# microsoft/CryptoNets

Hardware: AMD Instinct MI355X
Metric: encrypted images/sec (CryptoNets-MNIST, N=8192) (higher is better)
Workload: dtype u64

## Files before the change

cryptonets_amd/csrc/cn_api.hip:

```cpp
#include "cn_api_shared.h"

std::vector<Slab> &slabs_of(cn_ctx *ctx) { return *reinterpret_cast<std::vector<Slab> *>(ctx->slabs); }
bool in_slab(cn_ctx *ctx, const void *p) {
    for (const Slab &s : slabs_of(ctx)) if ((const char *)p >= s.base && (const char *)p < s.base + s.bytes) return true;
    return false;
}
int use(cn_ctx *c) { HIPCHK(hipSetDevice(c->device)); return 0; }

int ensure_scratch(cn_ctx *c, size_t bytes) {
    c->soff = 0;
    if (bytes <= c->scap) return 0;
    if (c->capturing || c->graphs_alive) return fail(CN_ERR_ARG, "the scratch arena would have to grow while a graph is recorded / alive: run the sequence once before cn_graph_begin");
    HIPCHK(hipStreamSynchronize(c->stream));
    if (c->scratch) HIPCHK(hipFree(c->scratch));
    c->scratch = nullptr; c->scap = 0;
    size_t want = bytes + (bytes >> 3) + (1 << 20);
    if (hipMalloc((void **)&c->scratch, want) != hipSuccess) {
        (void)hipGetLastError();
        pool_flush(c);
        HIPCHK(hipMalloc((void **)&c->scratch, want));
    }
    c->scap = want;
    return 0;
}
// ... 250 lines not shown
        if (b.kind == 2) (void)free_gemm_plan(ctx, b);
        else if (b.kind == 3) (void)free_graph(ctx, b);
        else if (!in_slab(ctx, b.d)) (void)hipFree(b.d);
    });
    pool_flush(ctx);
    for (const Slab &sl : slabs_of(ctx)) (void)hipFree(sl.base);
    delete &slabs_of(ctx);
    if (ctx->rlk.owned) (void)hipFree(ctx->rlk.d);
    for (auto &kv : ctx->gk) if (kv.second.owned) (void)hipFree(kv.second.d);
    defer_square_release(ctx);
    (void)hipFree(ctx->sk); (void)hipFree(ctx->pk); (void)hipFree(ctx->ks_part); (void)hipFree(ctx->d_index_map); (void)hipFree(ctx->stage); if (ctx->pin) (void)hipHostFree(ctx->pin);
    (void)hipFree(ctx->scratch); (void)hipFree(ctx->tw); (void)hipFree(ctx->twd); (void)hipFree(ctx->twdh); (void)hipFree(ctx->dc);
    if (ctx->ev0) (void)hipEventDestroy(ctx->ev0);
    if (ctx->ev1) (void)hipEventDestroy(ctx->ev1);
    if (ctx->ev_order) (void)hipEventDestroy(ctx->ev_order);
    if (ctx->ev_ms) (void)hipEventDestroy(ctx->ev_ms);
    if (ctx->ev_graph) (void)hipEventDestroy(ctx->ev_graph);
    if (ctx->stream2) { (void)hipStreamSynchronize(ctx->stream2); (void)hipStreamDestroy(ctx->stream2); }
    if (ctx->ev_fork) (void)hipEventDestroy(ctx->ev_fork);
    if (ctx->ev_join) (void)hipEventDestroy(ctx->ev_join);
    if (ctx->stream) (void)hipStreamDestroy(ctx->stream);
    cn_defer_delete(ctx->dq);
    delete ctx->ring; delete ctx->ready;
    delete ctx;
}
extern "C" int cn_set_option(cn_ctx *ctx, const char *name, int value) { API_BODY
    LOCK;
    if (!name) return fail(CN_ERR_ARG, "null option name");
    if (const OptionSpec *o = find_option(name)) {
        if (!o->flag && (value < o->lo || value > o->hi)) return fail(CN_ERR_ARG, "%s: %d .. %d", name, o->lo, o->hi);
        ctx->opt.*o->member = o->flag ? value != 0 : value;
        if (o->member == &CnTunables::f64 || o->member == &CnTunables::gemm_mfma || o->member == &CnTunables::gemm_pair) defer_square_drop_plans(ctx);
        return 0;
    }
    if (!strcmp(name, "defer")) {
        if (value < 0 || value > 2) return fail(CN_ERR_ARG, "defer: 0, 1 or 2");
        ctx->defer.store(value, std::memory_order_release);
        if (value != 2) {
            while (const cn_handle h = ctx->ready->pop()) CHECK(free_body(ctx, h));
            ctx->ready->misses.store(0, std::memory_order_relaxed);
        }
        return 0;
    }
    if (!strcmp(name, "ks_xi")) {
        if (ctx->level && (value != 0) != (ctx->hc.ks_xi != 0)) return fail(CN_ERR_ARG, "ks_xi of a level context is its parent's (its keys are)");
        if (ctx->capturing || ctx->graphs_alive) return fail(CN_ERR_ARG, "ks_xi cannot change while a graph is recorded or alive (its kernels were chosen for the other convention)");
        HIPCHK(hipStreamSynchronize(ctx->stream));
        ctx->hc.ks_xi = value != 0;
        HIPCHK(hipMemcpy(ctx->dc, &ctx->hc, sizeof(DevConsts), hipMemcpyHostToDevice));
        return 0;
    }
    if (!strcmp(name, "defer_square_gemm")) { ctx->defer_square_gemm = value != 0; return 0; }
    if (!strcmp(name, "digit_mfma")) { ctx->digit_mfma = value != 0; defer_square_drop_plans(ctx); return 0; }
    if (!strcmp(name, "mul_sum")) { ctx->mul_sum = value != 0; return 0; }
    if (!strcmp(name, "record_steps")) {
        ctx->rec_steps = value != 0;
        if (!value) { ctx->rec_set.clear(); ctx->rec_cols = false; }
        return 0;
    }
    return fail(CN_ERR_ARG, "unknown option %s", name);
API_END }
extern "C" int cn_get_option(cn_ctx *ctx, const char *name, int *value) { API_BODY
    LOCK_ONLY;
    if (!name || !value) return fail(CN_ERR_ARG, "null argument");
    if (const OptionSpec *o = find_option(name)) *value = ctx->opt.*o->member;
    else if (!strcmp(name, "defer")) *value = ctx->defer.load(std::memory_order_relaxed);
    else if (!strcmp(name, "ks_xi")) *value = (int)ctx->hc.ks_xi;
    else if (!strcmp(name, "record_steps")) *value = ctx->rec_steps;
    else if (!strcmp(name, "digit_mfma")) *value = ctx->digit_mfma;
    else if (!strcmp(name, "defer_square_gemm")) *value = ctx->defer_square_gemm;
    else if (!strcmp(name, "mul_sum")) *value = ctx->mul_sum;
    else if (!strcmp(name, "pin_laps")) *value = (int)ctx->pin_laps;
    else if (!strcmp(name, "ready_handles")) *value = (int)ctx->ready->size();
    else if (!strcmp(name, "folded_zero_encryptions")) *value = (int)std::min<uint64_t>(ctx->folded_zero, 0x7fffffff);
    else if (!strcmp(name, "square_gemm_fused")) *value = (int)std::min<uint64_t>(ctx->sg_fused, 0x7fffffff);
    else if (!strcmp(name, "defer_square_gemm_fused")) *value = (int)std::min<uint64_t>(ctx->dsg_fused, 0x7fffffff);
    else if (!strcmp(name, "mul_sum_fused")) *value = (int)std::min<uint64_t>(ctx->ms_fused, 0x7fffffff);
    else if (!strcmp(name, "mul_sum_groups")) *value = (int)ctx->ms_groups;
    else if (!strcmp(name, "mul_sum_min_k")) *value = (int)MUL_SUM_MIN_K;
    else if (!strcmp(name, "defer_pending_products")) *value = (int)ctx->dq->sq->out.size();
    else if (!strcmp(name, "digit_gemm_mfma")) *value = (int)std::min<uint64_t>(ctx->dg_mfma, 0x7fffffff);
    else if (!strcmp(name, "packed_bad_residues")) *value = (int)std::min<uint64_t>(ctx->packed_bad.load(), 0x7fffffff);
    else if (!strcmp(name, "mul_relin_pipelined")) *value = (int)std::min<uint64_t>(ctx->mr_pipelined, 0x7fffffff);
    else if (!strcmp(name, "behz_small_base")) *value = ctx->hc.bsk[ctx->hc.kb - 1].q < (1ull << 49);
    else if (!strcmp(name, "behz_f64")) *value = ctx->hc.behz_f64 && ctx->opt.f64;
    else if (!strcmp(name, "mod_switch_f64")) *value = ctx->ms_f64;
    else if (!strcmp(name, "aux_primes")) *value = (int)ctx->hc.kb;
    else if (!strcmp(name, "pending_calls")) *value = (int)ctx->dq->ops.size();
    else if (!strcmp(name, "pool_arrays")) { size_t c = 0; for (auto &kv : ctx->pool) c += kv.second.size(); *value = (int)std::min<size_t>(c, 0x7fffffff); }
    else if (!strcmp(name, "stream_tries")) *value = ctx->stream_tries;
    else return fail(CN_ERR_ARG, "unknown option %s", name);
    return 0;
API_END }
extern "C" int cn_sync(cn_ctx *ctx) { API_BODY LOCK; NOT_CAPTURING("cn_sync"); HIPCHK(hipStreamSynchronize(ctx->stream)); ctx->staged.clear(); return 0; API_END }
extern "C" void *cn_stream(cn_ctx *ctx) { return (void *)ctx->stream; }
extern "C" int cn_ctx_wait_for(cn_ctx *ctx_, cn_ctx *other) {
    if (!ctx_ || !other) return fail(CN_ERR_ARG, "null argument");
    if (ctx_ == other) return 0;
    hipEvent_t ev = nullptr;
    {
        cn_ctx *ctx = other;
        const int rc = ctx->mu.run([&]() -> int {
            LOCK; NOT_CAPTURING("cn_ctx_wait_for");
            if (!ctx->ev_order) HIPCHK(hipEventCreateWithFlags(&ctx->ev_order, hipEventDisableTiming));
            HIPCHK(hipEventRecord(ctx->ev_order, ctx->stream)); ev = ctx->ev_order;
            return 0;
        });
        if (rc) return rc;
    }
    cn_ctx *ctx = ctx_;
    return ctx->mu.run([&]() -> int {
        LOCK; NOT_CAPTURING("cn_ctx_wait_for");
        HIPCHK(hipStreamWaitEvent(ctx->stream, ev, 0));
        return 0;
    });
}
extern "C" size_t cn_key_words(cn_ctx *ctx, int which) { return (size_t)(which ? ctx->hc.gk_tot : ctx->hc.rl_tot) * ctx->ctw2; }

bool keys_as_f64(const cn_ctx *ctx) { return ctx->opt.f64 && cn_mod_range(ctx->hc, 0, ctx->hc.k).f64ok && rr_kernels(ctx); }
int set_key(cn_ctx *ctx, KsKey &slot, const uint64_t *words, size_t count, size_t expect, int is_dev, bool coeff_form) {
    if (!words || count != expect) return fail(CN_ERR_ARG, "key has %zu words, expected %zu", count, expect);
    HIPCHK(hipStreamSynchronize(ctx->stream));
    if (slot.owned && slot.d) HIPCHK(hipFree(slot.d));
    slot = {nullptr, false, false};
    if (is_dev) { slot.d = (uint64_t *)words; slot.owned = false; }
    else {
        HIPCHK(hipMalloc((void **)&slot.d, count * 8));
        slot.owned = true;
        HIPCHK(hipMemcpy(slot.d, words, count * 8, hipMemcpyHostToDevice));
    }
    if (coeff_form) CHECK(cn_run_ntt(ctx, slot.d, (uint32_t)(count / ctx->hc.n), 0, ctx->hc.k, 0));
    if (keys_as_f64(ctx)) {
        hipLaunchKernelGGL(k_u64_to_f64, dim3((unsigned)((count + 255) / 256)), dim3(256), 0, ctx->stream, slot.d, count);
        HIPCHK(hipGetLastError());
// ... 429 lines not shown
```

cryptonets_amd/csrc/cn_api_shared.h:

```cpp
#pragma once
#include "cn_runtime.h"
#include "cn_rotation.h"
#include <thread>
#include "cn_k_elem.hip.h"
#include <algorithm>
#include <chrono>
#include <mutex>
#include <map>
#include <unordered_map>
#include <cstdio>
#include <cstdlib>
#include <cstring>

#define fail cn_fail
struct DOp; struct DeferQueue; struct GemmPlan; struct GemmArith; struct Tab2; struct RotJob; struct BcastNext; struct Slab;

static const RrOps *const rr_ops[3] = {&cn_rr_u64, &cn_rr_f64, &cn_rr_f64l};
static const KsOps *const ks_ops[3] = {&cn_ks_u64, &cn_ks_f64, &cn_ks_f64l};
inline bool rr_kernels(const cn_ctx *c, uint32_t max_logn = 14) { return !c->opt.legacy_ntt && cn_rr_size(c->hc.logn, max_logn); }
enum { DOP_GEMM1 = 0, DOP_ADD, DOP_SUB, DOP_ADDPLAIN, DOP_SUBPLAIN, DOP_MULRELIN, DOP_ENCRYPT,
       DOP_COPY, DOP_MULPLAIN, DOP_ROT, DOP_ROTADD, DOP_COLS, DOP_COLSADD, DOP_SUMSLOTS, DOP_TYPES };
struct DOp {
    int type; int32_t level;
    uint64_t *out;
// ... 9 lines not shown
    std::vector<uint64_t> addr, wt;
    struct Haz { int32_t w = -1, r = -1, wop = -1; uint32_t readers = 0; int32_t hd = 0; };
    struct HazMap {
        struct E { const uint64_t *key = nullptr; uint32_t epoch = 0; Haz v; };
        std::vector<E> tab = std::vector<E>(1 << 12);
        uint32_t epoch = 1; size_t used = 0;
        static size_t hash(const uint64_t *p) { uint64_t x = (uint64_t)p >> 8; x *= 0x9E3779B97F4A7C15ull; return (size_t)(x >> 20); }
        Haz *find(const uint64_t *p) {
            for (size_t i = hash(p) & (tab.size() - 1);; i = (i + 1) & (tab.size() - 1)) {
                if (tab[i].epoch != epoch) return nullptr;
                if (tab[i].key == p) return &tab[i].v;
            }
        }
        Haz &operator[](const uint64_t *p) {
            if (2 * (used + 1) > tab.size()) grow();
            for (size_t i = hash(p) & (tab.size() - 1);; i = (i + 1) & (tab.size() - 1)) {
                if (tab[i].epoch != epoch) { tab[i].key = p; tab[i].epoch = epoch; tab[i].v = Haz(); used++; return tab[i].v; }
                if (tab[i].key == p) return tab[i].v;
            }
        }
        void grow() {
            std::vector<E> old; old.swap(tab);
            tab.assign(old.size() * 2, E()); used = 0;
            for (const E &e : old) if (e.epoch == epoch) (*this)[e.key] = e.v;
        }
        void clear() { used = 0; if (++epoch == 0) { for (E &e : tab) e.epoch = 0; epoch = 1; } }
    } haz;
    int32_t maxlevel = -1;
    std::vector<std::pair<uint64_t *, size_t>> frees;
    struct Fold { int32_t enc; uint64_t w; };
    std::vector<Fold> folds;
    struct DeferSquare *sq = nullptr;
};
static const size_t SLAB_MAX_ITEM = 8u << 20, SLAB_BYTES = 64u << 20;
struct Slab { char *base; size_t bytes; };
static const uint32_t DEFER_STAGED_MAX = 4;
struct CtSpan { uint64_t *d; uint32_t count; };
struct PtSpan { const uint64_t *d; uint32_t stride; const uint8_t *zero; };
struct GaloisCall {
    const uint64_t *in; uint64_t elt; uint64_t *out, *tmp; uint32_t count;
    const uint64_t *acc = nullptr, *pre = nullptr; uint64_t next_elt = 0; uint64_t *next_out = nullptr;
};
struct BcastNext { uint64_t elt; uint64_t *out, *ctn; };
struct GemmArith { bool small, two; uint32_t lazy; int bits; };
struct GemmPlan {
    uint32_t O = 0, K = 0, Kp = 0, G = 0, M = 0, MT = 0, lazy = 0, max_in = 0;
    bool small = false, two = false, one = false, has_bias = false, mfma = false;
    uint32_t P = 0, mtiles = 0, ksteps = 0;
    cn_handle bias_pt = 0; uint32_t bias_count = 0;
    uint64_t nnz = 0;
    std::vector<char> host;
    size_t off_oidx = 0, off_bidx = 0, off_w = 0;
    char *dev = nullptr;
    bool dig = false, dig_mfma = false; uint32_t dMT = 0, dKw = 0; size_t off_dw = 0;
};
struct SgPlan {
    bool ok = false, bias = false; uint32_t O = 0, K = 0;
    std::vector<uint64_t> W; std::vector<int32_t> cidx;
    GemmPlan P; std::vector<int32_t> idx, oidx;
    uint64_t used = 0;
};
struct DeferSquare {
    uint64_t *arr = nullptr; size_t cap = 0;
    std::vector<uint64_t *> out;
    std::unordered_map<const uint64_t *, uint32_t> slot;
    std::vector<std::unique_ptr<SgPlan>> plans; uint64_t tick = 0;
};
static const size_t DEFER_SQ_PLANS = 8;
struct Tab2 { const NTT_GLOBAL uint64_t *src; NTT_GLOBAL uint64_t *dst; };
struct RotJob { const uint64_t *src; uint64_t *dst; int steps; CnRotPlan plan; };

int cn_run_ntt(cn_ctx *c, uint64_t *data, uint32_t limbs, uint32_t base_off, uint32_t nmod, int inverse);
const NoiseTab &cn_noise_table();
std::vector<Slab> &slabs_of(cn_ctx *ctx);
bool in_slab(cn_ctx *ctx, const void *p);
int use(cn_ctx *c);
int ensure_scratch(cn_ctx *c, size_t bytes);
size_t al(size_t b);
char *pin_block(cn_ctx *c, size_t bytes);
int upload_bytes(cn_ctx *c, const void *host, size_t bytes, void *dev);
int place_table(cn_ctx *c, const void *host, size_t bytes, void *fallback, const void **dev);
Buffer *getbuf(cn_ctx *c, cn_handle h, int kind);
int range_ok(const Buffer *b, uint32_t first, uint32_t count, uint32_t stride = 1);
bool streams_share_a_queue(hipStream_t a, hipStream_t b);
int pick_stream(cn_ctx *c);
int ctx_init(cn_ctx *c, uint32_t n, uint32_t k, int device, std::vector<uint64_t> &tw);
void ctx_teardown(cn_ctx *ctx);
bool keys_as_f64(const cn_ctx *ctx);
int set_key(cn_ctx *ctx, KsKey &slot, const uint64_t *words, size_t count, size_t expect, int is_dev, bool coeff_form = false);
void pool_flush(cn_ctx *ctx);
int dev_alloc(cn_ctx *ctx, size_t bytes, uint64_t **out);
int dev_release(cn_ctx *ctx, uint64_t *p, size_t bytes);
int alloc_buf(cn_ctx *ctx, int kind, uint32_t count, uint32_t size, cn_handle *out);
bool submit_async(const cn_ctx *ctx);
int free_body(cn_ctx *ctx, cn_handle h);
int free_many_body(cn_ctx *ctx, const cn_handle *h, uint32_t n);
int free_graph(cn_ctx *ctx, Buffer &b);
void end_recording(cn_ctx *root);
int ensure_index_map(cn_ctx *ctx);
int addsub(cn_ctx *ctx, cn_handle a, uint32_t ai, cn_handle b, uint32_t bi, cn_handle out, uint32_t oi, uint32_t count, int op);
int addsub_body(cn_ctx *ctx, cn_handle a, uint32_t ai, cn_handle b, uint32_t bi, cn_handle out, uint32_t oi, uint32_t count, int op);
int add_plain_body(cn_ctx *ctx, cn_handle a, uint32_t ai, cn_handle pt, uint32_t pi, int subtract, cn_handle out, uint32_t oi, uint32_t count);
bool shifted_overlap(const uint64_t *a, const uint64_t *o, size_t words);
bool mul_plain_takes_bcast(cn_ctx *ctx, uint32_t count);
int mul_plain_impl(cn_ctx *ctx, CtSpan A, bool a_bcast, PtSpan P, CtSpan O, uint32_t polys, const BcastNext *nx = nullptr);
uint64_t lift_scalar(const DevConsts &hc, uint64_t w, uint32_t j);
bool gemm_weights_small(cn_ctx *ctx, const uint64_t *W, size_t count);
// ... 247 lines not shown
```

cryptonets_amd/csrc/cn_defer.hip:

```cpp
#include "cn_api_shared.h"


static const size_t DEFER_FLUSH_MIN = 64, DEFER_MAX_OPS = 32768;
DeferQueue *cn_defer_new() { DeferQueue *q = new DeferQueue(); q->sq = new DeferSquare(); return q; }
void cn_defer_delete(DeferQueue *q) { if (q) delete q->sq; delete q; }
bool cn_defer_pending(cn_ctx *ctx) { return ctx->dq && (!ctx->dq->ops.empty() || !ctx->dq->sq->out.empty()); }

int32_t defer_level(DeferQueue *q, const uint64_t *const *ins, uint32_t nin, const uint64_t *out) {
    int32_t lv = 0;
    for (uint32_t i = 0; i < nin; i++) {
        if (!ins[i]) continue;
        const DeferQueue::Haz *h = q->haz.find(ins[i]);
        if (h) lv = std::max(lv, h->w + 1);
    }
    const DeferQueue::Haz *ho = q->haz.find(out);
    if (ho) lv = std::max(lv, std::max(ho->w, ho->r) + 1);
    return lv;
}
int defer_push(cn_ctx *ctx, DOp op, const uint64_t *const *ins, uint32_t nin) {
    DeferQueue *q = ctx->dq;
    int32_t lv = defer_level(q, ins, nin, op.out);
    const bool heavy = op.type == DOP_GEMM1 || op.type == DOP_MULRELIN;
    int32_t hd = 0;
    for (uint32_t i = 0; i < nin; i++) if (ins[i]) { const DeferQueue::Haz *h = q->haz.find(ins[i]); if (h) hd = std::max(hd, h->hd); }
// ... 199 lines not shown
    if (*rc) return true;
    sq.out.resize(n);
    for (uint32_t i = 0; i < n; i++) { sq.out[i] = ops[i]->out; sq.slot[ops[i]->out] = i; }
    if (defer_trace()) fprintf(stderr, "defer %p level %d: parks %u squarings (Multiply only, %zu MB of products)\n", (void *)ctx, level, n, need >> 20);
    return true;
}
static int pending_materialise(cn_ctx *ctx, DeferSquare &sq, const std::vector<uint8_t> &need) {
    const uint32_t n = (uint32_t)sq.out.size();
    const size_t kn = (size_t)ctx->hc.k * ctx->hc.n;
    CHECK(ensure_scratch(ctx, al((size_t)n * 8) + 4096));
    uint64_t **dout; CHECK(upload_tmp(ctx, sq.out.data(), n, &dout));
    uint32_t done = 0;
    for (uint32_t s = 0; s < n;) {
        if (!need[s]) { s++; continue; }
        uint32_t e = s; while (e < n && need[e]) e++;
        CHECK(do_keyswitch(ctx, ctx->rlk, KsCall::relin(sq.arr + (size_t)s * 3 * kn, kn, e - s).to_table(dout + s)));
        done += e - s; s = e;
    }
    if (defer_trace()) fprintf(stderr, "defer %p: materialises %u of %u pending products (one key switch each)\n", (void *)ctx, done, n);
    return 0;
}
struct SgGroup { int32_t level; SgPlan *plan; std::vector<const DOp *> rows; std::vector<int32_t> slot_of; };
static SgPlan *sg_plan(cn_ctx *ctx, DeferSquare &sq, uint32_t O, uint32_t K, std::vector<uint64_t> &W, std::vector<int32_t> &cidx, uint64_t keep) {
    for (auto &p : sq.plans)
        if (p->O == O && p->K == K && !memcmp(p->W.data(), W.data(), W.size() * 8) && !memcmp(p->cidx.data(), cidx.data(), cidx.size() * 4)) { p->used = ++sq.tick; return p.get(); }
    if (sq.plans.size() >= DEFER_SQ_PLANS) {
        size_t v = sq.plans.size();
        for (size_t i = 0; i < sq.plans.size(); i++) if (sq.plans[i]->used <= keep && (v == sq.plans.size() || sq.plans[i]->used < sq.plans[v]->used)) v = i;
        if (v < sq.plans.size()) {
            if (sq.plans[v]->P.dev) { (void)hipStreamSynchronize(ctx->stream); (void)hipFree(sq.plans[v]->P.dev); }
            sq.plans.erase(sq.plans.begin() + v);
        }
    }
    std::unique_ptr<SgPlan> p(new SgPlan());
    p->O = O; p->K = K; p->W.swap(W); p->cidx.swap(cidx); p->used = ++sq.tick;
    GemmPlan &P = p->P;
    if (build_gemm_plan(ctx, p->cidx.data(), p->W.data(), O, K, nullptr, 0, nullptr, P)) return nullptr;
    p->ok = P.dig;
    if (p->ok) {
        p->idx.assign((const int32_t *)P.host.data(), (const int32_t *)P.host.data() + (size_t)P.G * P.Kp);
        p->oidx.assign((const int32_t *)(P.host.data() + P.off_oidx), (const int32_t *)(P.host.data() + P.off_oidx) + (size_t)P.G * P.M);
        if (hipMalloc((void **)&P.dev, P.host.size()) != hipSuccess || hipMemcpy(P.dev, P.host.data(), P.host.size(), hipMemcpyHostToDevice) != hipSuccess) {
            (void)hipGetLastError();
            if (P.dev) (void)hipFree(P.dev);
            P.dev = nullptr; p->ok = false;
        }
    }
    P.host.clear(); P.host.shrink_to_fit();
    sq.plans.push_back(std::move(p));
    return sq.plans.back().get();
}
static size_t sg_scratch(cn_ctx *ctx, const GemmPlan &P) {
    const size_t kn = (size_t)ctx->hc.k * ctx->hc.n;
    return al((size_t)P.O * 2 * kn * 8) + al((size_t)P.O * ctx->hc.rl_tot * ctx->hc.n * 8) + al((size_t)P.G * P.Kp * 4) + al((size_t)P.G * P.M * 4) + al((size_t)P.O * 8) + 8192;
}
static bool sg_prepare(cn_ctx *ctx, DeferQueue *q, const std::vector<uint8_t> &dead, const std::map<const uint64_t *, size_t> &freed, std::vector<SgGroup> &groups,
                       std::vector<int32_t> &sg_of, std::vector<uint8_t> &need) {
    DeferSquare &sq = *q->sq;
    const std::vector<DOp> &ops = q->ops;
    const uint32_t n = (uint32_t)sq.out.size();
    need.assign(n, 0);
    bool ok = ctx->defer_square_gemm && square_gemm_ctx_ok(ctx) && ctx->rlk.d;
    auto slot_of = [&](const uint64_t *p) -> int32_t { if (!p) return -1; auto it = sq.slot.find(p); return it == sq.slot.end() ? -1 : (int32_t)it->second; };
    std::map<std::pair<int32_t, uint32_t>, std::vector<size_t>> cand;
    for (size_t x = 0; x < ops.size(); x++) {
        if (dead[x]) continue;
        const DOp &X = ops[x];
        if (slot_of(X.out) >= 0) ok = false;
        if (X.type == DOP_GEMM1) {
            uint32_t np = 0, other = 0;
            for (uint32_t kk = 0; kk < X.K; kk++) {
                const uint64_t *a = (const uint64_t *)q->addr[X.terms + kk];
                if (!a) continue;
                const int32_t s = slot_of(a);
                if (s >= 0) { need[s] = 1; np++; } else other++;
            }
            if (!np) continue;
            if (other || X.fold_count) ok = false;
            cand[{X.level, X.K}].push_back(x);
            continue;
        }
        if (X.type == DOP_ENCRYPT) continue;
        const bool b_plain = X.type == DOP_ADDPLAIN || X.type == DOP_SUBPLAIN || X.type == DOP_MULPLAIN;
        for (const uint64_t *p : {X.a, b_plain ? nullptr : X.b}) { const int32_t s = slot_of(p); if (s >= 0) { need[s] = 1; ok = false; } }
    }
    for (uint32_t s = 0; s < n; s++) if (!in_freed(freed, sq.out[s])) { need[s] = 1; ok = false; }
    if (!ok) return false;
    const uint64_t keep = sq.tick;
    for (auto &kv : cand) {
        const uint32_t K = kv.first.second, O = (uint32_t)kv.second.size();
        SgGroup g; g.level = kv.first.first;
        for (size_t x : kv.second) g.rows.push_back(&ops[x]);
        std::stable_sort(g.rows.begin(), g.rows.end(), [&](const DOp *x, const DOp *y) {
            return std::lexicographical_compare(&q->wt[x->terms], &q->wt[x->terms] + K, &q->wt[y->terms], &q->wt[y->terms] + K); });
        std::vector<uint64_t> W((size_t)O * K); std::vector<int32_t> cidx((size_t)O * K, -1), canon(n, -1);
        for (uint32_t o = 0; o < O; o++) {
            memcpy(&W[(size_t)o * K], &q->wt[g.rows[o]->terms], (size_t)K * 8);
            for (uint32_t kk = 0; kk < K; kk++) {
                const int32_t s = slot_of((const uint64_t *)q->addr[g.rows[o]->terms + kk]);
                if (s < 0) continue;
                if (canon[s] < 0) { canon[s] = (int32_t)g.slot_of.size(); g.slot_of.push_back(s); }
                cidx[(size_t)o * K + kk] = canon[s];
            }
        }
        g.plan = sg_plan(ctx, sq, O, K, W, cidx, keep);
        if (!g.plan || !g.plan->ok || !square_gemm_fused_ok(ctx, g.plan->P) || sg_scratch(ctx, g.plan->P) > ctx->smax) return false;
        if (sg_scratch(ctx, g.plan->P) > ctx->scap && ctx->graphs_alive) return false;
        uint64_t bbase = ~0ull;
        for (const DOp *r : g.rows) { if ((r->bias != nullptr) != (g.rows[0]->bias != nullptr)) return false; if (r->bias) bbase = std::min(bbase, (uint64_t)r->bias); }
        for (const DOp *r : g.rows) if (r->bias && ((((uint64_t)r->bias - bbase) & 255) || (((uint64_t)r->bias - bbase) >> 8) >= 0x7fffffffull)) return false;
        for (size_t x : kv.second) sg_of[x] = (int32_t)groups.size();
        groups.push_back(std::move(g));
    }
    return true;
}
static int sg_run(cn_ctx *ctx, DeferQueue *q, const SgGroup &g) {
    const SgPlan &sp = *g.plan; const GemmPlan &P = sp.P;
    const uint32_t n = ctx->hc.n, k = ctx->hc.k, tot = ctx->hc.rl_tot;
    const size_t kn = (size_t)k * n;
    std::vector<int32_t> pidx(sp.idx.size()), bidx(sp.oidx.size(), 0);
    std::vector<uint64_t *> outs(P.O);
    for (size_t x = 0; x < pidx.size(); x++) pidx[x] = sp.idx[x] >= 0 ? g.slot_of[sp.idx[x]] : -1;
    const bool bias = g.rows[0]->bias != nullptr;
    uint64_t bbase = ~0ull;
    if (bias) {
        for (const DOp *r : g.rows) bbase = std::min(bbase, (uint64_t)r->bias);
        for (size_t x = 0; x < bidx.size(); x++) if (sp.oidx[x] >= 0) bidx[x] = (int32_t)(((uint64_t)g.rows[sp.oidx[x]]->bias - bbase) >> 8);
    }
    for (uint32_t o = 0; o < P.O; o++) outs[o] = g.rows[o]->out;
    CHECK(ensure_scratch(ctx, sg_scratch(ctx, P)));
    uint64_t *T = salloc<uint64_t>(ctx, (size_t)P.O * 2 * kn);
    double *S = salloc<double>(ctx, (size_t)P.O * tot * n);
    if (!T || !S) return fail(CN_ERR_HIP, "internal: scratch exhausted in the deferred square + dense form");
    int32_t *dpidx, *dbidx; uint64_t **douts;
    CHECK(upload_tmp(ctx, pidx.data(), pidx.size(), &dpidx)); CHECK(upload_tmp(ctx, bidx.data(), bidx.size(), &dbidx)); CHECK(upload_tmp(ctx, outs.data(), outs.size(), &douts));
    const uint64_t *arr = q->sq->arr;
    CHECK(launch_gemm_plan(ctx, P, P.dev, dpidx, arr, (uint32_t)(3 * kn), 2u, bias ? (const uint64_t *)bbase : nullptr, dbidx, 32, T, 0));
    DigitGemmLaunch dg{arr + 2 * kn, 3 * kn, dpidx, P.dev + P.off_dw, P.dev + P.off_oidx, S, P.G, P.M, P.K, P.Kp, P.dKw, P.dMT};
    if (P.dig_mfma) { dg.W = P.dev + P.off_w; dg.mfma = true; dg.P = P.P; dg.mtiles = P.mtiles; dg.ksteps = P.ksteps; }
    CHECK(cn_l_digit_gemm(ctx, dg));
    CHECK(do_keyswitch(ctx, ctx->rlk, KsCall::relin_digits(S, T, kn, P.O).to_table(douts)));
    ctx->dsg_fused++;
    if (defer_trace()) fprintf(stderr, "defer %p level %d: fuses %u scalar products over %zu pending products (GEMM, digit GEMM%s, %u key switches)\n", (void *)ctx, g.level, P.O,
                               g.slot_of.size(), P.dig_mfma ? " on the matrix cores" : "", P.O);
    return 0;
}

int flush_mulrelin_group(cn_ctx *ctx, const std::vector<const DOp *> &all, const std::map<const uint64_t *, size_t> *park, int32_t level) {
    const size_t kn = (size_t)ctx->hc.k * ctx->hc.n;
    for (int sq = 1; sq >= 0; sq--) {
        std::vector<const DOp *> ops;
        for (const DOp *op : all) if ((op->a == op->b) == (sq == 1)) ops.push_back(op);
        if (ops.empty()) continue;
        if (sq && park) { int rc = 0; if (park_squarings(ctx, ctx->dq, ops, *park, level, &rc)) { CHECK(rc); continue; } }
        const size_t per = mul_scratch_per_ct(ctx, sq == 1) + al(3 * kn * 8) + 3 * 8 + 64;
        const uint32_t ch = chunk_for(ctx, per, (uint32_t)ops.size());
        for (uint32_t s0 = 0; s0 < ops.size(); s0 += ch) {
            const uint32_t c = std::min<uint32_t>(ch, (uint32_t)ops.size() - s0);
            CHECK(ensure_scratch(ctx, per * c + 3 * al((size_t)c * 8) + 8192));
            std::vector<const uint64_t *> ha(c), hb(c); std::vector<uint64_t *> ho(c);
            for (uint32_t i = 0; i < c; i++) { ha[i] = ops[s0 + i]->a; hb[i] = ops[s0 + i]->b; ho[i] = ops[s0 + i]->out; }
            const uint64_t **da, **db = nullptr; uint64_t **dout;
            CHECK(upload_tmp(ctx, ha.data(), c, &da));
            if (!sq) CHECK(upload_tmp(ctx, hb.data(), c, &db));
            CHECK(upload_tmp(ctx, ho.data(), c, &dout));
            uint64_t *t3 = salloc<uint64_t>(ctx, (size_t)c * 3 * kn);
            if (!t3) return fail(CN_ERR_HIP, "internal: scratch exhausted in deferred multiply");
            auto mul = [&](uint32_t f, uint32_t n_) { return do_multiply(ctx, nullptr, 1, nullptr, 1, t3 + (size_t)f * 3 * kn, n_, da + f, (sq ? da : db) + f); };
            auto ksw = [&](uint32_t f, uint32_t n_) { return do_keyswitch(ctx, ctx->rlk, KsCall::relin(t3 + (size_t)f * 3 * kn, kn, n_).to_table(dout + f)); };
            if (ctx->opt.sq_halves >= 2 && ctx->hc.logn <= 13 && c >= SQ_HALVES_MIN && !ctx->capturing && pipeline_fused_ks(ctx, c) && aux_stream_ready(ctx)) {
                CHECK(pipelined_halves(ctx, c, mul, ksw)); continue;
            }
            CHECK(mul(0, c));
            CHECK(ksw(0, c));
        }
    }
    return 0;
}


__global__ void k_copy_tab(const Tab2 *__restrict__ tab, uint32_t pairs_per_item) {
    const Tab2 t = tab[blockIdx.y];
    const uint32_t i = blockIdx.x * blockDim.x + threadIdx.x;
    typedef unsigned long long v2u64 __attribute__((ext_vector_type(2)));
    if (i < pairs_per_item) reinterpret_cast<NTT_GLOBAL v2u64 *>(t.dst)[i] = reinterpret_cast<const NTT_GLOBAL v2u64 *>(t.src)[i];
}
int ensure_stage(cn_ctx *ctx, size_t bytes) {
    if (bytes <= ctx->stage_cap) return 0;
    if (ctx->capturing || ctx->graphs_alive) return fail(CN_ERR_ARG, "the staging arena would have to grow while a graph is recorded / alive");
    HIPCHK(hipStreamSynchronize(ctx->stream));
    if (ctx->stage) HIPCHK(hipFree(ctx->stage));
    ctx->stage = nullptr; ctx->stage_cap = 0;
    const size_t want = bytes + (bytes >> 2) + (1 << 20);
    HIPCHK(hipMalloc((void **)&ctx->stage, want));
// ... 490 lines not shown
```

cryptonets_amd/csrc/cn_eval.hip:

```cpp
#include "cn_api_shared.h"

int addsub(cn_ctx *ctx, cn_handle a, uint32_t ai, cn_handle b, uint32_t bi, cn_handle out, uint32_t oi, uint32_t count, int op) {
    GETCT(A, a, 0); GETCT(O, out, A->size);
    Buffer *B = A;
    if (op != 2) { B = getbuf(ctx, b, 0); if (!B || B->size != A->size) return fail(CN_ERR_ARG, "operand sizes do not match"); }
    if (!range_ok(A, ai, count) || !range_ok(O, oi, count) || (op != 2 && !range_ok(B, bi, count))) return fail(CN_ERR_ARG, "index out of range");
    if (!count) return 0;
    uint32_t limbs = count * A->size * ctx->hc.k;
    hipLaunchKernelGGL(k_addsub, dim3(limbs * ctx->chunks), dim3(ctx->bs), 0, ctx->stream, A->d + ai * A->item_words,
                       B->d + (op != 2 ? bi : ai) * B->item_words, O->d + oi * O->item_words, ctx->dc, ctx->chunks, op);
    HIPCHK(hipGetLastError()); launch_count(ctx);
    return 0;
}
int addsub_body(cn_ctx *ctx, cn_handle a, uint32_t ai, cn_handle b, uint32_t bi, cn_handle out, uint32_t oi, uint32_t count, int op) {
    if (deferring(ctx)) { int rc = defer_addsub(ctx, a, ai, b, bi, out, oi, count, op); if (rc <= 0) return rc; }
    CHECK(cn_defer_flush(ctx)); CHECK(addsub(ctx, a, ai, b, bi, out, oi, count, op));
    if (op) ctx->st.Subtraction += count; else ctx->st.Addition += count;
    return 0;
}
extern "C" int cn_add(cn_ctx *ctx, cn_handle a, uint32_t ai, cn_handle b, uint32_t bi, cn_handle out, uint32_t oi, uint32_t count) {
    if (submit_async(ctx) && count <= DEFER_STAGED_MAX) return ring_push(ctx, SUB_ADD, count, a, ai, b, bi, out, oi, 0, 0);
    API_BODY LOCK_ONLY; return addsub_body(ctx, a, ai, b, bi, out, oi, count, 0); API_END
}
extern "C" int cn_sub(cn_ctx *ctx, cn_handle a, uint32_t ai, cn_handle b, uint32_t bi, cn_handle out, uint32_t oi, uint32_t count) {
// ... 228 lines not shown
    const uint64_t t = ctx->hc.t.q;
    std::vector<int32_t> gidx((size_t)O * K);
    for (uint32_t o = 0; o < O; o++) {
        bool any = false;
        for (uint32_t kk = 0; kk < K; kk++) {
            int32_t id = idx ? idx[(size_t)o * K + kk] : (int32_t)kk;
            uint64_t w = W[(size_t)o * K + kk];
            if (w >= t) return fail(CN_ERR_ARG, "weight >= plain modulus");
            if (id >= 0) P.max_in = std::max<uint32_t>(P.max_in, (uint32_t)id + 1);
            if (id >= 0 && w) { any = true; P.nnz++; }
            gidx[(size_t)o * K + kk] = id;
        }
        if (!any) return fail(CN_ERR_ARG, "output %u has no non-zero term (AddMany of nothing)", o);
        if (BP && (bias_idx[o] < 0 || (uint32_t)bias_idx[o] >= BP->count)) return fail(CN_ERR_ARG, "bias index out of range");
    }
    std::vector<uint64_t> W2;
    if (ctx->opt.gemm_pair && gemm_arith(ctx, gemm_weights_small(ctx, W, (size_t)O * K)).small && pair_gather_lists(O, K, gidx, W, W2)) W = W2.data();
    std::map<std::vector<int32_t>, std::vector<uint32_t>> groups;
    for (uint32_t o = 0; o < O; o++) groups[std::vector<int32_t>(gidx.begin() + (size_t)o * K, gidx.begin() + (size_t)(o + 1) * K)].push_back(o);
    const uint32_t NONE = 0xffffffffu;
    uint32_t G = (uint32_t)groups.size(), M = 0;
    for (auto &g : groups) M = std::max<uint32_t>(M, (uint32_t)g.second.size());
    const GemmArith ar = gemm_arith(ctx, gemm_weights_small(ctx, W, (size_t)O * K));
    const bool small = ar.small, mfma = gemm_mfma_ok(ctx, ar, M, K);
    const uint32_t Kp = mfma ? ((K + 31) / 32) * 32 : ((K + 15) & ~15u) + 16;
    std::vector<int32_t> hidx((size_t)G * Kp, -1), hoidx((size_t)G * M, -1), hbidx((size_t)G * M, 0);
    std::vector<uint32_t> member((size_t)G * M, NONE);
    {
        uint32_t g = 0;
        for (auto &kv : groups) {
            memcpy(&hidx[(size_t)g * Kp], kv.first.data(), K * 4);
            for (uint32_t m = 0; m < kv.second.size(); m++) member[(size_t)g * M + m] = kv.second[m];
            g++;
        }
    }
    for (size_t x = 0; x < member.size(); x++) if (member[x] != NONE) { hoidx[x] = (int32_t)member[x]; if (BP) hbidx[x] = bias_idx[member[x]]; }
    P.O = O; P.K = K; P.Kp = Kp; P.G = G; P.M = M; P.small = small; P.has_bias = BP != nullptr; P.bias_pt = bias_pt; P.bias_count = BP ? BP->count : 0;
    P.two = ar.two; P.lazy = ar.lazy; P.mfma = mfma;
    std::vector<char> wbytes;
    auto row = [&](uint32_t g, uint32_t m) -> const uint64_t * { return member[(size_t)g * M + m] == NONE ? nullptr : W + (size_t)member[(size_t)g * M + m] * K; };
    if (mfma) {
        P.P = gemm_weight_planes(ctx, W, (size_t)O * K); P.mtiles = (M + 31) / 32; P.ksteps = (K + 31) / 32;
        pack_gemm_mfma(ctx, G, M, K, P.P, row, [&](uint32_t g, uint32_t kk) { return hidx[(size_t)g * Kp + kk] >= 0; }, wbytes);
    } else {
        auto tap = [&](uint32_t g, uint32_t kk) { return hidx[(size_t)g * Kp + kk] >= 0; };
        pack_gemm_weights(ctx, G, M, K, small, row, tap, P.MT, wbytes);
        P.one = gemm_one_limb(ctx, ar, G, M, K, row, tap);
    }
    std::vector<double> dW;
    if (small && ctx->hc.k >= 2 && ctx->hc.dbc >= 1 && ctx->hc.dbc <= 30) {
        uint64_t qmin = ~0ull; for (uint32_t j = 0; j < ctx->hc.k; j++) qmin = std::min(qmin, ctx->hc.q[j].q);
        const uint64_t dmax = (1ull << ctx->hc.dbc) - 1, lim = std::min<uint64_t>((qmin - 1) / 2, (1ull << 52) - 1) / dmax;
        bool ok = true;
        for (uint32_t g = 0; g < G && ok; g++) for (uint32_t m = 0; m < M && ok; m++) {
            const uint64_t *wr = row(g, m);
            if (!wr) continue;
            uint64_t sum = 0;
            for (uint32_t kk = 0; kk < K; kk++) if (hidx[(size_t)g * Kp + kk] >= 0) { const uint64_t w = wr[kk]; sum += w >= ctx->hc.t_half ? t - w : w; }
            ok = sum <= lim;
        }
        if (ok) { P.dig = true; P.dig_mfma = mfma && ctx->digit_mfma && ctx->hc.dbc <= 14 && !(ctx->hc.n & 255); }
        if (ok && !P.dig_mfma) {
            P.dMT = digit_gemm_tile(M); P.dKw = digit_gemm_rows(K);
            const uint32_t mtd = (M + P.dMT - 1) / P.dMT;
            dW.assign((size_t)G * mtd * P.dKw * P.dMT, 0.0);
            for (uint32_t g = 0; g < G; g++) for (uint32_t m = 0; m < M; m++) {
                const uint64_t *wr = row(g, m);
                if (!wr) continue;
                double *dst = &dW[(((size_t)g * mtd + m / P.dMT) * P.dKw) * P.dMT + m % P.dMT];
                for (uint32_t kk = 0; kk < K; kk++) { const uint64_t w = hidx[(size_t)g * Kp + kk] >= 0 ? wr[kk] : 0; dst[(size_t)kk * P.dMT] = w >= ctx->hc.t_half ? -(double)(t - w) : (double)w; }
            }
        }
    }
    P.off_oidx = al(hidx.size() * 4); P.off_bidx = P.off_oidx + al(hoidx.size() * 4); P.off_w = P.off_bidx + al(hbidx.size() * 4);
    P.off_dw = P.off_w + al(wbytes.size());
    P.host.assign(P.off_dw + al(dW.size() * 8), 0);
    memcpy(P.host.data() + P.off_dw, dW.data(), dW.size() * 8);
    memcpy(P.host.data(), hidx.data(), hidx.size() * 4);
    memcpy(P.host.data() + P.off_oidx, hoidx.data(), hoidx.size() * 4);
    memcpy(P.host.data() + P.off_bidx, hbidx.data(), hbidx.size() * 4);
    memcpy(P.host.data() + P.off_w, wbytes.data(), wbytes.size());
    return 0;
}
int launch_gemm_plan(cn_ctx *ctx, const GemmPlan &P, const char *tables, const void *idx, const uint64_t *in, uint32_t in_unit, uint32_t polys, const uint64_t *bias, const void *bidx,
                     uint32_t bias_unit, uint64_t *out, uint32_t obase) {
    GemmLaunch gl{P.small, P.two, false, P.MT, in, idx, tables + P.off_w, tables + P.off_oidx, bias, bidx, out,
                  P.G, P.M, P.K, P.lazy, P.Kp, obase, P.P, P.mtiles, P.ksteps, polys, (uint32_t)ctx->opt.gemm_order, P.one};
    gl.in_unit = in_unit; gl.bias_unit = bias_unit;
    return P.mfma ? cn_l_gemm_mfma(ctx, gl) : cn_l_gemm(ctx, gl);
}
int run_gemm_plan(cn_ctx *ctx, const GemmPlan &P, const char *tables, Buffer *I, Buffer *OB, uint32_t oi, const uint64_t *in3) {
    if (!range_ok(OB, oi, P.O)) return fail(CN_ERR_ARG, "output index out of range");
    if (!in3) {
    if (I == OB) return fail(CN_ERR_ARG, "scalar GEMM cannot run in place");
    if (P.max_in > I->count) return fail(CN_ERR_ARG, "input index out of range");
    if (I->size != OB->size || I->size < 2 || I->size > 3) return fail(CN_ERR_ARG, "scalar GEMM: input and output ciphertext sizes must match (2 or 3)");
    } else if (OB->size != 2) return fail(CN_ERR_ARG, "scalar GEMM: output ciphertext size must be 2");
    const uint64_t *bias = nullptr;
    if (P.has_bias) {
        Buffer *BP = getbuf(ctx, P.bias_pt, 1);
        if (!BP || BP->count < P.bias_count) return fail(CN_ERR_ARG, "invalid bias plaintext handle");
        bias = BP->d;
    }
    CHECK(launch_gemm_plan(ctx, P, tables, tables, in3 ? in3 : I->d, in3 ? (uint32_t)(3 * ctx->hc.k * ctx->hc.n) : 0u, in3 ? 2u : I->size, bias, tables + P.off_bidx, 0, OB->d, oi));
    ctx->st.PlainMultiplication += P.nnz; ctx->st.Addition += P.nnz - P.O;
    if (P.has_bias) ctx->st.PlainAddition += P.O;
    return 0;
}
extern "C" int cn_scalar_gemm(cn_ctx *ctx, cn_handle in, const int32_t *idx, const uint64_t *W, uint32_t O, uint32_t K, cn_handle bias_pt,
                              const int32_t *bias_idx, cn_handle out, uint32_t oi) { API_BODY
    LOCK; GETCT(I, in, 0); GETCT(OB, out, 0);
    Buffer *BP = bias_pt ? getbuf(ctx, bias_pt, 1) : nullptr;
    GemmPlan P;
    CHECK(build_gemm_plan(ctx, idx, W, O, K, BP, bias_pt, bias_idx, P));
// ... 123 lines not shown
    return (size_t)cnt * (mode == 2 ? k : tot_dig) * ctx->ctw2 * 8 > ctx->smax ? 0 : mode;
}
int do_keyswitch(cn_ctx *ctx, const KsKey &key, const KsCall &call) {
    const uint32_t n = ctx->hc.n, k = ctx->hc.k, cnt = call.cnt, tot_dig = call.galois ? ctx->hc.gk_tot : ctx->hc.rl_tot;
    const CnModRange qr = cn_mod_range(ctx->hc, 0, k);
    const int bits = qr.bits, pol = cn_policy(qr, key.f64);
    KsArgs a{call, key.d,
             key.f64 ? (bits >= 50 ? 1u : (1u << std::min(10, 50 - bits))) : 0xffffffffu,
             ks_planned_mode(ctx, cnt, call.galois)};
    if (ctx->opt.ks_xcd == 1) a.xcd_cts = cnt & ~7u;
    else if (ctx->opt.ks_xcd == 2) a.xcd_cts = 0x80000000u;
    const bool rr = rr_kernels(ctx);
    if (a.mode) CHECK(ensure_ks_part(ctx, (size_t)cnt * (a.mode == 2 ? k : tot_dig) * ctx->ctw2 * 8));
    if (a.dig && !(rr && key.f64 && ctx->hc.logn <= 13 && !a.galois && !ctx->hc.ks_xi)) return fail(CN_ERR_ARG, "internal: ready-made digits outside the FP64 register-radix key switch");
    const bool pair = ks_pair14_ok(ctx, cnt, a.galois, key);
    if ((a.perm_elt || a.items || a.next_elt) && !a.mode && !(pair && !a.items)) return fail(CN_ERR_ARG, "internal: automorphism inside the fused key switch");
    if (pair) {
        CHECK(ensure_ks_part(ctx, (size_t)cnt * ctx->ctw2 * 8));
        a.xcd_cts = ctx->opt.ks_xcd == 1 ? (cnt & ~7u) : 0u;
        ks_ops[pol]->pair14(ctx, a);
    } else if (a.mode == 0 && rr && key.f64 && ctx->hc.logn == 14 && ctx->hc.twdh && ctx->opt.ks_split14) {
        CHECK(ensure_ks_part(ctx, (size_t)cnt * ctx->ctw2 * 8));
        ks_ops[pol]->split14(ctx, a);
        hipLaunchKernelGGL(k_ks_combine14, dim3(cnt * 2 * k * (n / 512)), dim3(256), 0, ctx->stream, (const uint64_t *)ctx->ks_part, a.add0, a.add1, a.astride, a.out, ctx->dc,
                           a.extra, a.xstride, a.out_tab);
        launch_count(ctx);
    } else {
        const bool done = rr && ks_ops[pol]->launch(ctx, a);
        if (!done && key.f64) return fail(CN_ERR_ARG, "internal: FP64 key without FP64 kernel");
        if (!done) {
            uint64_t *const out = a.out;
            if (a.extra) {
                if (a.xstride != ctx->ctw2 || a.out_tab) return fail(CN_ERR_ARG, "internal: accumulator stride");
                CHECK(ensure_ks_part(ctx, (size_t)cnt * ctx->ctw2 * 8));
                a.out = (uint64_t *)ctx->ks_part;
            }
            const uint32_t nt = std::min<uint32_t>(1024, n);
            switch (n / nt) {
                case 1: launch_ks_legacy<1>(ctx, nt, a); break;
                case 2: launch_ks_legacy<2>(ctx, nt, a); break;
                case 4: launch_ks_legacy<4>(ctx, nt, a); break;
                case 8: launch_ks_legacy<8>(ctx, nt, a); break;
                case 16: launch_ks_legacy<16>(ctx, nt, a); break;
                default: return fail(CN_ERR_ARG, "unsupported poly modulus degree for key switching");
            }
            if (a.extra) {
                hipLaunchKernelGGL(k_addsub, dim3(cnt * 2 * k * ctx->chunks), dim3(ctx->bs), 0, ctx->stream, (const uint64_t *)ctx->ks_part, a.extra, out, ctx->dc,
                                   ctx->chunks, 0);
                launch_count(ctx);
            }
        }
    }
    HIPCHK(hipGetLastError()); launch_count(ctx);
    ctx->st.ntt_forward_limbs += (uint64_t)cnt * tot_dig * k; ctx->st.ntt_inverse_limbs += (uint64_t)cnt * 2 * k;
    return 0;
}
bool ks_pair14_ok(cn_ctx *ctx, uint32_t cnt, int galois, const KsKey &key) {
    return ctx->opt.ks_pair14 && ctx->opt.ks_split14 && rr_kernels(ctx) && ctx->hc.logn == 14 && ctx->hc.twdh && key.f64 && ks_planned_mode(ctx, cnt, galois) == 0;
}
uint32_t chunk_for(cn_ctx *ctx, size_t per_ct, uint32_t count) {
    size_t c = std::max<size_t>(1, ctx->smax / per_ct);
    return (uint32_t)std::min<size_t>(c, count);
}

extern "C" int cn_multiply(cn_ctx *ctx, cn_handle a, uint32_t ai, cn_handle b, uint32_t bi, cn_handle out3, uint32_t oi, uint32_t count) { API_BODY TWO_LIMBS("cn_multiply");
    LOCK; GETCT(A, a, 2); GETCT(B, b, 2); GETCT(O, out3, 3);
    if (!range_ok(A, ai, count) || !range_ok(B, bi, count) || !range_ok(O, oi, count)) return fail(CN_ERR_ARG, "index out of range");
    if (!count) return 0;
    const uint64_t *pa = A->d + ai * A->item_words, *pb = B->d + bi * B->item_words;
    size_t per = mul_scratch_per_ct(ctx, pa == pb);
    uint32_t ch = chunk_for(ctx, per, count);
    for (uint32_t s = 0; s < count; s += ch) {
        uint32_t c = std::min(ch, count - s);
        CHECK(ensure_scratch(ctx, per * c + 4096));
        CHECK(do_multiply(ctx, pa + s * A->item_words, 1, pb + s * B->item_words, 1, O->d + (oi + s) * O->item_words, c));
    }
    return 0;
API_END }
extern "C" int cn_relinearize(cn_ctx *ctx, cn_handle in3, uint32_t ii, cn_handle out, uint32_t oi, uint32_t count) { API_BODY TWO_LIMBS("cn_relinearize");
    LOCK; GETCT(I, in3, 3); GETCT(O, out, 2);
    if (!range_ok(I, ii, count) || !range_ok(O, oi, count)) return fail(CN_ERR_ARG, "index out of range");
    if (!ctx->rlk.d) return fail(CN_ERR_NOKEY, "relinearization keys not set");
    if (!count) return 0;
    const size_t kn = (size_t)ctx->hc.k * ctx->hc.n;
    const uint64_t *p = I->d + ii * I->item_words;
    CHECK(do_keyswitch(ctx, ctx->rlk, KsCall::relin(p, kn, count).to(O->d + oi * O->item_words)));
    ctx->st.Relinarization += count;
    return 0;
API_END }
static int mul_relin_overlap(cn_handle x, uint32_t xi, uint32_t xstride, cn_handle out, uint32_t oi, uint32_t count) {
    if (x != out || !count) return 0;
    const uint64_t lo = xi, hi = (uint64_t)xi + (uint64_t)(count - 1) * xstride + 1, olo = oi, ohi = (uint64_t)oi + count;
    if ((lo == olo && hi == ohi) || hi <= olo || ohi <= lo) return 0;
    return fail(CN_ERR_ARG, "mul_relin: an operand range and the result range overlap partially (use the same range or disjoint ranges)");
}
extern "C" int cn_mul_relin(cn_ctx *ctx, cn_handle a, uint32_t ai, uint32_t astride, cn_handle b, uint32_t bi, uint32_t bstride, cn_handle out,
                            uint32_t oi, uint32_t count) {
    TWO_LIMBS("cn_mul_relin");
    CHECK(mul_relin_overlap(a, ai, astride, out, oi, count)); CHECK(mul_relin_overlap(b, bi, bstride, out, oi, count));
    if (submit_async(ctx) && count <= DEFER_STAGED_MAX) return ring_push(ctx, SUB_MUL_RELIN, count, a, ai, b, bi, out, oi, astride, bstride);
    API_BODY LOCK_ONLY; return mul_relin_body(ctx, a, ai, astride, b, bi, bstride, out, oi, count); API_END
}
int mul_relin_body(cn_ctx *ctx, cn_handle a, uint32_t ai, uint32_t astride, cn_handle b, uint32_t bi, uint32_t bstride, cn_handle out, uint32_t oi, uint32_t count) {
    CHECK(mul_relin_overlap(a, ai, astride, out, oi, count)); CHECK(mul_relin_overlap(b, bi, bstride, out, oi, count));
    if (deferring(ctx)) return defer_mul_relin(ctx, a, ai, astride, b, bi, bstride, out, oi, count);
    CHECK(cn_defer_flush(ctx));
    GETCT(A, a, 2); GETCT(B, b, 2); GETCT(O, out, 2);
    if (!range_ok(A, ai, astride ? count : 1, astride ? astride : 1) || !range_ok(B, bi, bstride ? count : 1, bstride ? bstride : 1) || !range_ok(O, oi, count))
        return fail(CN_ERR_ARG, "index out of range");
    if (!ctx->rlk.d) return fail(CN_ERR_NOKEY, "relinearization keys not set");
    if (!count) return 0;
    const size_t kn = (size_t)ctx->hc.k * ctx->hc.n;
    const uint64_t *pa = A->d + ai * A->item_words, *pb = B->d + bi * B->item_words;
    const bool square = (pa == pb && astride == bstride);
    size_t per = mul_scratch_per_ct(ctx, square) + al(3 * kn * 8);
    uint32_t ch = chunk_for(ctx, per, count);
    for (uint32_t s = 0; s < count; s += ch) {
        uint32_t c = std::min(ch, count - s);
        CHECK(ensure_scratch(ctx, per * c + 8192));
        uint64_t *t3 = salloc<uint64_t>(ctx, (size_t)c * 3 * kn);
        auto mul = [&](uint32_t f, uint32_t n_) { return do_multiply(ctx, pa + (size_t)(s + f) * astride * A->item_words, astride, pb + (size_t)(s + f) * bstride * B->item_words, bstride, t3 + (size_t)f * 3 * kn, n_); };
        auto ksw = [&](uint32_t f, uint32_t n_) { return do_keyswitch(ctx, ctx->rlk, KsCall::relin(t3 + (size_t)f * 3 * kn, kn, n_).to(O->d + (oi + s + f) * O->item_words)); };
        if (ctx->opt.sq_halves && ctx->hc.logn <= 13 && c >= SQ_HALVES_MIN && !ctx->capturing && pipeline_fused_ks(ctx, c) && aux_stream_ready(ctx)) {
            CHECK(pipelined_halves(ctx, c, mul, ksw)); continue;
        }
        CHECK(mul(0, c));
        CHECK(ksw(0, c));
    }
    ctx->st.Relinarization += count;
    return 0;
}

bool square_gemm_ctx_ok(cn_ctx *ctx) {
    return ctx->opt.f64 && rr_kernels(ctx, 13) && !ctx->hc.ks_xi && ctx->rlk.f64 && cn_mod_range(ctx->hc, 0, ctx->hc.k).f64ok;
}
bool square_gemm_fused_ok(cn_ctx *ctx, const GemmPlan &P) { return P.dig && square_gemm_ctx_ok(ctx); }
extern "C" int cn_square_gemm(cn_ctx *ctx, cn_handle plan, cn_handle in, uint32_t ii, cn_handle out, uint32_t oi) { TWO_LIMBS("cn_square_gemm"); API_BODY
    LOCK; GETCT(I, in, 2); GETCT(OB, out, 2);
    Buffer *PB = getbuf(ctx, plan, 2);
    if (!PB || !PB->plan) return fail(CN_ERR_ARG, "invalid scalar GEMM plan handle");
    const GemmPlan &P = *PB->plan;
    const uint32_t cnt = P.max_in;
    if (!range_ok(I, ii, cnt)) return fail(CN_ERR_ARG, "input index out of range");
    if (!range_ok(OB, oi, P.O)) return fail(CN_ERR_ARG, "output index out of range");
    if (I == OB) return fail(CN_ERR_ARG, "cn_square_gemm cannot run in place");
    if (!ctx->rlk.d) return fail(CN_ERR_NOKEY, "relinearization keys not set");
    const uint32_t n = ctx->hc.n, k = ctx->hc.k, tot = ctx->hc.rl_tot;
    const size_t kn = (size_t)k * n;
    const size_t per = mul_scratch_per_ct(ctx, true);
    const size_t fixed = al((size_t)cnt * 3 * kn * 8) + al((size_t)P.O * tot * n * 8) + 8192;
    if (!square_gemm_fused_ok(ctx, P) || fixed + per > ctx->smax) {
        cn_handle tmp = 0;
        CHECK(alloc_buf(ctx, 0, cnt, 2, &tmp));
        int rc = mul_relin_body(ctx, in, ii, 1, in, ii, 1, tmp, 0, cnt);
        if (!rc) rc = cn_defer_flush(ctx);
        OB = getbuf(ctx, out, 0);
        if (!rc) rc = run_gemm_plan(ctx, P, P.dev, getbuf(ctx, tmp, 0), OB, oi);
        const int rf = free_body(ctx, tmp);
        return rc ? rc : rf;
    }
    const uint32_t ch = (uint32_t)std::min<size_t>(cnt, (ctx->smax - fixed) / per);
    CHECK(ensure_scratch(ctx, fixed + per * ch + 4096));
    uint64_t *t3 = salloc<uint64_t>(ctx, (size_t)cnt * 3 * kn);
    double *S = salloc<double>(ctx, (size_t)P.O * tot * n);
    if (!t3 || !S) return fail(CN_ERR_HIP, "internal: scratch exhausted in cn_square_gemm");
    const size_t mark = ctx->soff;
    const uint64_t *pa = I->d + ii * I->item_words;
    for (uint32_t s = 0; s < cnt; s += ch) {
        const uint32_t c = std::min(ch, cnt - s);
        ctx->soff = mark;
        CHECK(do_multiply(ctx, pa + (size_t)s * I->item_words, 1, pa + (size_t)s * I->item_words, 1, t3 + (size_t)s * 3 * kn, c));
    }
    CHECK(run_gemm_plan(ctx, P, P.dev, nullptr, OB, oi, t3));
    DigitGemmLaunch dg{t3 + 2 * kn, 3 * kn, P.dev, P.dev + P.off_dw, P.dev + P.off_oidx, S, P.G, P.M, P.K, P.Kp, P.dKw, P.dMT};
    if (P.dig_mfma) { dg.W = P.dev + P.off_w; dg.mfma = true; dg.P = P.P; dg.mtiles = P.mtiles; dg.ksteps = P.ksteps; }
    CHECK(cn_l_digit_gemm(ctx, dg));
    uint64_t *o = OB->d + oi * OB->item_words;
    CHECK(do_keyswitch(ctx, ctx->rlk, KsCall::relin_digits(S, o, kn, P.O).to(o)));
    ctx->st.Relinarization += cnt; ctx->sg_fused++;
    return 0;
API_END }

static bool mul_sum_fused_ok(cn_ctx *ctx, uint32_t K) {
    if (!ctx->mul_sum || K < MUL_SUM_MIN_K || !square_gemm_ctx_ok(ctx)) return false;
    const int dbc = ctx->hc.dbc;
    if (dbc < 1 || dbc > 31) return false;
    const unsigned __int128 s = (unsigned __int128)K * ((1ull << dbc) - 1);
    if (s >= ((unsigned __int128)1 << 52)) return false;
    const uint64_t qmax = cn_mod_range(ctx->hc, 0, ctx->hc.k).qmax;
    for (uint32_t j = 0; j < ctx->hc.k; j++) {
        if (s >= ctx->hc.q[j].q / 2) return false;
        if (ctx->hc.rl_dig[j] > PRODUCT_SUM_MAX_DIGITS) return false;
    }
    return (unsigned __int128)K * (qmax - 1) < ((unsigned __int128)1 << 64) && !(ctx->hc.n & 511);
}
static int add_many_terms(cn_ctx *ctx, Buffer *T, uint32_t K, Buffer *O, uint32_t oi, uint32_t count) {
    std::vector<uint32_t> idx((size_t)count * K);
    for (uint32_t i = 0; i < count; i++) for (uint32_t kk = 0; kk < K; kk++) idx[(size_t)i * K + kk] = kk * count + i;
    CHECK(ensure_scratch(ctx, al(idx.size() * 4) + 4096));
    uint32_t *didx; CHECK(upload_tmp(ctx, idx.data(), idx.size(), &didx));
    const uint32_t limbs = T->size * ctx->hc.k;
    for (uint32_t i = 0; i < count; i++) {
        hipLaunchKernelGGL(k_add_many, dim3(limbs * ctx->chunks), dim3(ctx->bs), 0, ctx->stream, T->d, didx + (size_t)i * K, K, T->item_words,
                           O->d + (oi + i) * O->item_words, ctx->dc, ctx->chunks);
        HIPCHK(hipGetLastError()); launch_count(ctx);
    }
    return 0;
}
extern "C" int cn_mul_relin_sum(cn_ctx *ctx, const cn_handle *a, const uint32_t *a_idx, const cn_handle *b, const uint32_t *b_idx, uint32_t K, uint32_t b_stride,
                                cn_handle out, uint32_t oi, uint32_t count) { TWO_LIMBS("cn_mul_relin_sum"); API_BODY
    LOCK;
    if (!a || !b) return fail(CN_ERR_ARG, "null argument");
    if (!K || !count) return fail(CN_ERR_ARG, "cn_mul_relin_sum of an empty list");
    if (b_stride > 1) return fail(CN_ERR_ARG, "cn_mul_relin_sum: b_stride is 0 (one ciphertext for every output) or 1");
    if ((uint64_t)K * count > 0x7fffffffull) return fail(CN_ERR_ARG, "cn_mul_relin_sum: too many products");
    GETCT(O, out, 2);
    if (!range_ok(O, oi, count)) return fail(CN_ERR_ARG, "output index out of range");
    auto ai = [&](uint32_t kk) { return a_idx ? a_idx[kk] : 0u; };
    auto bi = [&](uint32_t kk) { return b_idx ? b_idx[kk] : 0u; };
    for (uint32_t kk = 0; kk < K; kk++) {
        if (a[kk] == out || b[kk] == out) return fail(CN_ERR_ARG, "cn_mul_relin_sum cannot run in place (out is an operand handle)");
        Buffer *A = getbuf(ctx, a[kk], 0), *B = getbuf(ctx, b[kk], 0);
        if (!A || !B) return fail(CN_ERR_ARG, "invalid ciphertext handle in term %u", kk);
        if (A->size != 2 || B->size != 2) return fail(CN_ERR_ARG, "ciphertext size mismatch in term %u", kk);
        if (!range_ok(A, ai(kk), count) || !range_ok(B, bi(kk), b_stride ? count : 1)) return fail(CN_ERR_ARG, "index out of range in term %u", kk);
    }
    if (!ctx->rlk.d) return fail(CN_ERR_NOKEY, "relinearization keys not set");
    ctx->ms_groups = 0;
    const uint32_t n = ctx->hc.n, k = ctx->hc.k, tot = ctx->hc.rl_tot;
    const size_t kn = (size_t)k * n;
    if (K == 1) {
        int rc = mul_relin_body(ctx, a[0], ai(0), 1, b[0], bi(0), b_stride, out, oi, count);
        if (!rc) rc = cn_defer_flush(ctx);
        if (!rc) { ctx->st.AddMany += count; ctx->st.AddManyItemCount += count; }
        return rc;
    }
    const size_t per = mul_scratch_per_ct(ctx, false);
    const size_t per_out = (size_t)K * 3 * kn * 8 + (size_t)tot * n * 8 + (size_t)K * 16, slack = 4 * 256 + 8192;
    const size_t g_fit = ctx->smax > per + slack ? (ctx->smax - per - slack) / per_out : 0;
    if (!mul_sum_fused_ok(ctx, K) || !g_fit) {
        cn_handle tmp = 0;
        CHECK(alloc_buf(ctx, 0, K * count, 2, &tmp));
        int rc = 0;
        for (uint32_t kk = 0; kk < K && !rc; kk++) rc = mul_relin_body(ctx, a[kk], ai(kk), 1, b[kk], bi(kk), b_stride, tmp, kk * count, count);
        if (!rc) rc = cn_defer_flush(ctx);
        if (!rc) rc = add_many_terms(ctx, getbuf(ctx, tmp, 0), K, getbuf(ctx, out, 0), oi, count);
        if (!rc) { ctx->st.AddMany += count; ctx->st.AddManyItemCount += (uint64_t)count * K; }
        const int rf = free_body(ctx, tmp);
        return rc ? rc : rf;
    }
    const uint32_t g = (uint32_t)std::min<size_t>(count, g_fit);
    std::vector<const uint64_t *> ha((size_t)g * K), hb((size_t)g * K);
    for (uint32_t o0 = 0; o0 < count; o0 += g) {
        const uint32_t go = std::min(g, count - o0), np = go * K;
        const size_t fixed = al((size_t)np * 3 * kn * 8) + al((size_t)go * tot * n * 8) + 2 * al((size_t)np * 8) + 8192;
        const uint32_t ch = (uint32_t)std::min<size_t>(np, std::max<size_t>(1, (ctx->smax - std::min(ctx->smax, fixed)) / per));
        CHECK(ensure_scratch(ctx, fixed + per * ch + 4096));
        uint64_t *t3 = salloc<uint64_t>(ctx, (size_t)np * 3 * kn);
        double *S = salloc<double>(ctx, (size_t)go * tot * n);
        if (!t3 || !S) return fail(CN_ERR_HIP, "internal: scratch exhausted in cn_mul_relin_sum");
        for (uint32_t i = 0; i < go; i++) for (uint32_t kk = 0; kk < K; kk++) {
            const Buffer *A = getbuf(ctx, a[kk], 0), *B = getbuf(ctx, b[kk], 0);
            ha[(size_t)i * K + kk] = A->d + (size_t)(ai(kk) + o0 + i) * A->item_words;
            hb[(size_t)i * K + kk] = B->d + (size_t)(bi(kk) + (o0 + i) * b_stride) * B->item_words;
        }
        const uint64_t **da, **db;
        CHECK(upload_tmp(ctx, ha.data(), np, &da)); CHECK(upload_tmp(ctx, hb.data(), np, &db));
        const size_t mark = ctx->soff;
        for (uint32_t s = 0; s < np; s += ch) {
            const uint32_t c = std::min(ch, np - s);
            ctx->soff = mark;
            CHECK(do_multiply(ctx, nullptr, 1, nullptr, 1, t3 + (size_t)s * 3 * kn, c, da + s, db + s));
        }
        uint64_t *o = O->d + (size_t)(oi + o0) * O->item_words;
        CHECK(cn_l_product_sum(ctx, ProductSumLaunch{t3, K, o, S, go}));
        CHECK(do_keyswitch(ctx, ctx->rlk, KsCall::relin_digits(S, o, kn, go).to(o)));
        ctx->ms_groups++;
    }
    ctx->st.Relinarization += (uint64_t)K * count; ctx->st.AddMany += count; ctx->st.AddManyItemCount += (uint64_t)count * K;
    ctx->ms_fused++;
    return 0;
API_END }

const KsKey *galois_key(cn_ctx *ctx, uint64_t elt) { auto it = ctx->gk.find(elt); return it != ctx->gk.end() && it->second.d ? &it->second : nullptr; }
static int columns_key(cn_ctx *ctx) { return galois_key(ctx, 2ull * ctx->hc.n - 1) ? 0 : fail(CN_ERR_NOKEY, "Galois key not present"); }
static int add_overlap(cn_ctx *ctx, const uint64_t *in, const uint64_t *acc, const uint64_t *out, uint32_t count) {
    if (!shifted_overlap(in, out, count * ctx->ctw2) && !shifted_overlap(acc, out, count * ctx->ctw2)) return 0;
    return fail(CN_ERR_ARG, "rotate-and-add: operand / accumulator and result ranges overlap partially (use the same range or disjoint ranges)");
}
int do_galois(cn_ctx *ctx, const GaloisCall &g) {
    const KsKey *key = galois_key(ctx, g.elt);
    if (!key) return fail(CN_ERR_NOKEY, "Galois key not present");
    const size_t kn = (size_t)ctx->hc.k * ctx->hc.n;
    const uint32_t count = g.count, limbs = count * 2 * ctx->hc.k, elt = (uint32_t)g.elt;
    const bool shifted = shifted_overlap(g.in, g.out, count * ctx->ctw2);
    CHECK(add_overlap(ctx, nullptr, g.acc, g.out, count));
    KsCall ks;
    if (!shifted && ks_pair14_ok(ctx, count, 1, *key)) {
        if (!g.pre) {
            hipLaunchKernelGGL(k_galois_limbs, dim3(count * ctx->hc.k), dim3(1024), (size_t)ctx->hc.n * 8, ctx->stream, g.in + kn, 2 * kn, g.tmp, kn, ctx->dc, g.elt);
            HIPCHK(hipGetLastError()); launch_count(ctx);
        }
        ks = KsCall::galois_of(g.pre ? g.pre : g.tmp, kn, g.in, kn, count).perm(elt).next((uint32_t)g.next_elt, g.next_out);
    } else if (g.pre || g.next_elt) return fail(CN_ERR_ARG, "internal: rotation chain outside the one-launch key switch");
    else if (!shifted && ctx->opt.ks_perm_fused && ks_planned_mode(ctx, count, 1) != 0)
        ks = KsCall::galois_of(g.in + kn, 2 * kn, g.in, kn, count).perm(elt);
    else {
        if (ctx->hc.n >= 1024) hipLaunchKernelGGL(k_galois_lds, dim3(limbs), dim3(std::min<uint32_t>(1024, ctx->hc.n / 4)), (size_t)ctx->hc.n * 8, ctx->stream, g.in, g.tmp, ctx->dc, g.elt);
        else hipLaunchKernelGGL(k_galois, dim3(limbs * ctx->chunks), dim3(ctx->bs), 0, ctx->stream, g.in, g.tmp, ctx->dc, ctx->chunks, g.elt);
        HIPCHK(hipGetLastError()); launch_count(ctx);
        ks = KsCall::galois_of(g.tmp + kn, 2 * kn, g.tmp, kn, count);
    }
    CHECK(do_keyswitch(ctx, *key, ks.to(g.out).plus(g.acc, ctx->ctw2)));
    ctx->st.Rotation += count;
    if (g.acc) ctx->st.Addition += count;
    return 0;
}
static int ct_scratch(cn_ctx *ctx, uint32_t count, uint32_t arrays, uint64_t **first) {
    CHECK(ensure_scratch(ctx, al(count * ctx->ctw2 * 8) * arrays));
    *first = salloc<uint64_t>(ctx, count * ctx->ctw2);
    return 0;
}
int galois_impl(cn_ctx *ctx, CtSpan in, uint64_t elt, CtSpan acc, CtSpan out) {
    if (acc.d) CHECK(add_overlap(ctx, in.d, acc.d, out.d, out.count));
    if (!out.count) return 0;
    uint64_t *tmp; CHECK(ct_scratch(ctx, out.count, 1, &tmp));
    return do_galois(ctx, {.in = in.d, .elt = elt, .out = out.d, .tmp = tmp, .count = out.count, .acc = acc.d});
}
extern "C" int cn_apply_galois(cn_ctx *ctx, cn_handle in, uint32_t ii, uint64_t elt, cn_handle out, uint32_t oi, uint32_t count) { API_BODY TWO_LIMBS("cn_apply_galois");
// ... 302 lines not shown
```

cryptonets_amd/csrc/cn_k_gemm.hip.h:

```cpp
#pragma once
#include "cn_dev_common.hip.h"

DEV void gemm_block_coords(uint32_t bx, uint32_t by, uint32_t chunks, uint32_t limbs, uint32_t mtiles, uint32_t G, uint32_t &chunk, uint32_t &limb, uint32_t &mt, uint32_t &g,
                           uint32_t order = 0) {
    if (order == 1) {
        const uint32_t x = bx & 7, r = bx >> 3;
        if (mtiles == 1) { mt = 0; g = r; } else { mt = r % mtiles; g = r / mtiles; }
        const uint32_t sl = by * 8 + x;
        chunk = sl & (chunks - 1); limb = sl >> (__ffs((int)chunks) - 1);
        return;
    }
    const uint32_t b = bx, D = chunks * limbs * G;
    uint32_t d;
    if ((D & 7) == 0) { const uint32_t r = b >> 3; mt = r % mtiles; d = (r / mtiles) * 8 + (b & 7); }
    else { d = b % D; mt = b / D; }
    chunk = d % chunks; limb = (d / chunks) % limbs; g = d / (chunks * limbs);
}
DEV const NTT_GLOBAL uint64_t *gmem(uint64_t a) { return (const NTT_GLOBAL uint64_t *)a; }
DEV NTT_GLOBAL uint64_t *gmem_w(uint64_t a) { return (NTT_GLOBAL uint64_t *)a; }
struct GemmUnits { uint32_t in, out, bias; };
template <bool ABS> struct GemmTab { typedef int32_t T; };
template <> struct GemmTab<true> { typedef uint64_t T; };
template <int MT, bool ABS = false>
__global__ void __launch_bounds__(256) k_scalar_gemm(const uint64_t *__restrict__ in, const void *__restrict__ idx_, const uint64_t *__restrict__ Wl,
// ... 321 lines not shown
        fb[3][lane][wave] = byte_perm(cd13, ab13, 0x07060302u);
        fb[4][lane][wave] = byte_perm(hcd, hab, 0x05040100u);
        fb[5][lane][wave] = byte_perm(hcd, hab, 0x07060302u);
        load_x(xn, nidx); load_a(afn, ks + GEMM_MFMA_DEPTH);
        load_idx(nidx, ks + GEMM_MFMA_DEPTH + 1);
        __syncthreads();
        if (active) {
            v4i_t bf[ND];
#pragma unroll
            for (int i = 0; i < ND; i++) bf[i] = *reinterpret_cast<const v4i_t *>(&fb[i][lane][0]);
#pragma unroll
            for (int p = 0; p < P; p++)
#pragma unroll
                for (int i = 0; i < ND; i++) acc[i + p] = __builtin_amdgcn_mfma_i32_32x32x32_i8(af[p], bf[i], acc[i + p], 0, 0, 0);
        }
    };
    uint32_t ks = 0;
    for (; ks + NB <= ksteps; ks += NB) {
#pragma unroll
        for (int s = 0; s < NB; s++) step(xs[s], afs[s], xs[(s + GEMM_MFMA_DEPTH) % NB], afs[(s + GEMM_MFMA_DEPTH) % NB], ks + s, frag[s]);
    }
#pragma unroll
    for (int s = 0; s < NB - 1; s++)
        if (ks + s < ksteps) step(xs[s], afs[s], xs[(s + GEMM_MFMA_DEPTH) % NB], afs[(s + GEMM_MFMA_DEPTH) % NB], ks + s, frag[s]);
    if (!active) return;
    const BzF::Mod mq = {C->qd[j], C->qinvd[j]};
    const DMod qm = C->q[j];
    const double c24 = BzF::center(16777216.0, mq), c48 = BzF::center(__dmul_rn(c24, 16777216.0), mq);
#pragma unroll
    for (int r = 0; r < 16; r++) {
        const uint32_t row = (uint32_t)(r & 3) + 8u * (uint32_t)(r >> 2) + 4u * half, o = g * M + mt * 32 + row;
        if (mt * 32 + row >= M) continue;
        auto group = [&](int d0) {
            double t = (double)acc[d0][r];
            if (d0 + 1 < D) t = __fma_rn((double)acc[d0 + 1 < D ? d0 + 1 : d0][r], 256.0, t);
            if (d0 + 2 < D) t = __fma_rn((double)acc[d0 + 2 < D ? d0 + 2 : d0][r], 65536.0, t);
            return t;
        };
        double v = __dadd_rn(group(0), BzF::mulmod(group(3), c24, mq));
        if (D > 6) v = __dadd_rn(v, BzF::mulmod(group(6), c48, mq));
        uint64_t res = BzF::to_u64(v, mq);
        if constexpr (ABS) {
            if (!out_idx[o]) continue;
            if (bias_idx && bias_idx[o] && limb < k) { const uint64_t bv = gmem(bias_idx[o])[(size_t)ctile * 32 + col]; if (bv) res = addmod(res, scale_plain(C, bv, j), qm.q); }
            gmem_w(out_idx[o])[e] = res;
        } else {
            if (out_idx[o] < 0) continue;
            if (bias && limb < k) { const uint64_t bv = bias[(size_t)bias_idx[o] * bu + (size_t)ctile * 32 + col]; if (bv) res = addmod(res, scale_plain(C, bv, j), qm.q); }
            out[(size_t)(obase + (uint32_t)out_idx[o]) * ou + e] = res;
        }
    }
}

template <int MT, int DG>
__global__ void __launch_bounds__(256) k_digit_gemm(const uint64_t *__restrict__ in, size_t in_unit, const int32_t *__restrict__ idx, const double *__restrict__ Wd,
                                                    const int32_t *__restrict__ out_idx, double *__restrict__ S, const DevConsts *__restrict__ C, uint32_t G, uint32_t M,
                                                    uint32_t K, uint32_t mtiles, uint32_t Kp, uint32_t Kw, uint32_t ndg) {
    const uint32_t n = C->n, k = C->k, chunks = n >> 8;
    uint32_t chunk, lj, mt, g;
    gemm_block_coords(blockIdx.x, 0, chunks, k * ndg, mtiles, G, chunk, lj, mt, g);
    const uint32_t l = lj % k, d0 = (lj / k) * DG, nd = C->rl_dig[l];
    if (d0 >= nd) return;
    uint32_t g0 = 0;
    for (uint32_t x = 0; x < l; x++) g0 += C->rl_dig[x];
    const uint32_t i = chunk * 256 + threadIdx.x, dbc = (uint32_t)C->dbc, mask = (1u << dbc) - 1;
    const size_t e = (size_t)l * n + i;
    uint32_t sh[DG];
#pragma unroll
    for (int d = 0; d < DG; d++) sh[d] = min(dbc * (d0 + (uint32_t)d), 63u);
    double acc[DG][MT];
#pragma unroll
    for (int d = 0; d < DG; d++)
#pragma unroll
        for (int m = 0; m < MT; m++) acc[d][m] = 0.0;
    const int32_t *gi = idx + (size_t)g * Kp;
    const double *gw = Wd + ((size_t)g * mtiles + mt) * (size_t)Kw * MT;
    constexpr int PF = 4, WB = MT > 10 ? 1 : 2;
    auto fetch = [&](uint64_t (&x)[PF], uint32_t kk) {
        const int4 ids = *reinterpret_cast<const int4 *>(__builtin_assume_aligned(gi + min(kk, Kp - PF), 16));
        const int32_t id[4] = {ids.x, ids.y, ids.z, ids.w};
#pragma unroll
        for (int p = 0; p < PF; p++) x[p] = in[(size_t)max(id[p], 0) * in_unit + e];
    };
    auto terms = [&](const uint64_t (&x)[PF], uint32_t kk) {
#pragma unroll
        for (int p0 = 0; p0 < PF; p0 += WB) {
            double w[WB * MT];
            const double *wp = gw + (size_t)(kk + p0) * MT;
#pragma unroll
            for (int q = 0; q < WB * MT; q++) w[q] = wp[q];
#pragma unroll
            for (int p = p0; p < p0 + WB; p++) {
                double dg[DG];
#pragma unroll
                for (int d = 0; d < DG; d++) dg[d] = (double)((uint32_t)(x[p] >> sh[d]) & mask);
#pragma unroll
                for (int m = 0; m < MT; m++)
#pragma unroll
                    for (int d = 0; d < DG; d++) acc[d][m] = __fma_rn(dg[d], w[(p - p0) * MT + m], acc[d][m]);
            }
        }
    };
    {
        const uint32_t sets = (K + PF - 1) / PF;
        uint32_t kk = 0;
        uint64_t xa[PF], xb[PF];
        fetch(xa, 0);
        for (uint32_t it = sets >> 1; it; it--, kk += 2 * PF) {
            fetch(xb, kk + PF);
            terms(xa, kk);
            fetch(xa, kk + 2 * PF);
            terms(xb, kk + PF);
        }
        if (sets & 1) terms(xa, kk);
    }
    const uint32_t tot = C->rl_tot;
#pragma unroll
    for (int m = 0; m < MT; m++) {
        const uint32_t mm = mt * MT + (uint32_t)m;
        if (mm >= M) break;
        const int32_t o = out_idx[g * M + mm];
        if (o < 0) continue;
#pragma unroll
        for (int d = 0; d < DG; d++)
            if (d0 + (uint32_t)d < nd) S[((size_t)o * tot + g0 + d0 + (uint32_t)d) * n + i] = acc[d][m];
    }
}

template <int P, int DG>
__global__ void __launch_bounds__(256, 2) k_digit_gemm_mfma(const uint64_t *__restrict__ in, size_t in_unit, const int32_t *__restrict__ idx, const int8_t *__restrict__ Wf,
                                                            const int32_t *__restrict__ out_idx, double *__restrict__ S, const DevConsts *__restrict__ C, uint32_t G,
                                                            uint32_t M, uint32_t mtiles, uint32_t ksteps, uint32_t ndg) {
    constexpr int NP = 2 * DG, D = P + 1, NB = GEMM_MFMA_DEPTH + 1;
    __shared__ __align__(16) uint32_t frag[NB][NP][64][4];
    const uint32_t n = C->n, k = C->k, ctiles = n >> 5;
    const uint32_t lane = threadIdx.x & 63, wave = (uint32_t)__builtin_amdgcn_readfirstlane((int)(threadIdx.x >> 6)), half = lane >> 5, col = lane & 31;
    uint32_t b = blockIdx.x;
    const uint32_t x8 = b & 7; b >>= 3;
    const uint32_t dgi = b % ndg; b /= ndg;
    const uint32_t ctile = (b % (ctiles >> 3)) * 8 + x8; b /= ctiles >> 3;
    const uint32_t l = b % k; b /= k;
    const uint32_t mgroups = (mtiles + 3) >> 2, mg = b % mgroups, g = b / mgroups;
    const uint32_t d0 = dgi * DG, nd = C->rl_dig[l];
    if (d0 >= nd) return;
    const uint32_t cnt = min((uint32_t)DG, nd - d0);
    uint32_t g0 = 0;
    for (uint32_t x = 0; x < l; x++) g0 += C->rl_dig[x];
    const uint32_t mt = mg * 4 + wave;
    const bool active = mt < mtiles;
    const uint32_t dbc = (uint32_t)C->dbc, mask = (1u << dbc) - 1;
    uint32_t sh[DG];
#pragma unroll
    for (int d = 0; d < DG; d++) sh[d] = min(dbc * (d0 + (uint32_t)d), 63u);
    const size_t e = (size_t)l * n + (size_t)ctile * 32 + col;
    const uint32_t Kp = ksteps * 32;
    const int32_t *gi = idx + (size_t)g * Kp + 4 * wave;
    const int8_t *wf = Wf + ((((size_t)g * P) * mtiles + (active ? mt : 0)) * ksteps) * 1024 + (size_t)lane * 16;
    v16i_t acc[DG][D];
#pragma unroll
    for (int d = 0; d < DG; d++)
#pragma unroll
        for (int j = 0; j < D; j++)
#pragma unroll
            for (int r = 0; r < 16; r++) acc[d][j][r] = 0;
    const uint32_t klast = ksteps - 1;
    auto load_idx = [&](int32_t (&s)[8], uint32_t ks) {
        const int32_t *t = gi + (size_t)min(ks, klast) * 32;
#pragma unroll
        for (int u = 0; u < 4; u++) { s[u] = t[u]; s[4 + u] = t[16 + u]; }
    };
    auto load_x = [&](uint64_t (&x)[4], const int32_t (&s)[8]) {
#pragma unroll
        for (int u = 0; u < 4; u++) {
            size_t o0 = (size_t)max(s[u], 0) * in_unit, o1 = (size_t)max(s[4 + u], 0) * in_unit;
            asm volatile("" : "+s"(o0), "+s"(o1));
            x[u] = in[(half ? o1 : o0) + e];
        }
    };
    auto load_a = [&](v4i_t (&af)[P], uint32_t ks) {
#pragma unroll
        for (int p = 0; p < P; p++) af[p] = *reinterpret_cast<const v4i_t *>(wf + ((size_t)p * mtiles * ksteps + min(ks, klast)) * 1024);
    };
    uint64_t xs[NB][4];
    v4i_t afs[NB][P];
    int32_t nidx[8];
    load_idx(nidx, 0);
#pragma unroll
    for (int s = 0; s < GEMM_MFMA_DEPTH; s++) { load_x(xs[s], nidx); load_a(afs[s], s); load_idx(nidx, s + 1); }
    auto step = [&](uint64_t (&x)[4], v4i_t (&af)[P], uint64_t (&xn)[4], v4i_t (&afn)[P], uint32_t ks, uint32_t (*fb)[64][4]) {
#pragma unroll
        for (int d = 0; d < DG; d++) {
            uint32_t t[4];
#pragma unroll
            for (int u = 0; u < 4; u++) t[u] = ((uint32_t)(x[u] >> sh[d]) & mask) + 128u;
            const uint32_t ab = byte_perm(t[1], t[0], 0x05010400u), cd = byte_perm(t[3], t[2], 0x05010400u);
            fb[2 * d][lane][wave] = byte_perm(cd, ab, 0x05040100u) ^ 0x80808080u;
            fb[2 * d + 1][lane][wave] = byte_perm(cd, ab, 0x07060302u);
        }
        load_x(xn, nidx); load_a(afn, ks + GEMM_MFMA_DEPTH);
        load_idx(nidx, ks + GEMM_MFMA_DEPTH + 1);
        __syncthreads();
        if (active) {
#pragma unroll
            for (int d = 0; d < DG; d++) {
                if ((uint32_t)d >= cnt) continue;
                const v4i_t blo = *reinterpret_cast<const v4i_t *>(&fb[2 * d][lane][0]), bhi = *reinterpret_cast<const v4i_t *>(&fb[2 * d + 1][lane][0]);
#pragma unroll
                for (int p = 0; p < P; p++) acc[d][p] = __builtin_amdgcn_mfma_i32_32x32x32_i8(af[p], blo, acc[d][p], 0, 0, 0);
#pragma unroll
                for (int p = 0; p < P; p++) acc[d][p + 1] = __builtin_amdgcn_mfma_i32_32x32x32_i8(af[p], bhi, acc[d][p + 1], 0, 0, 0);
            }
        }
    };
    uint32_t ks = 0;
    for (; ks + NB <= ksteps; ks += NB) {
#pragma unroll
        for (int s = 0; s < NB; s++) step(xs[s], afs[s], xs[(s + GEMM_MFMA_DEPTH) % NB], afs[(s + GEMM_MFMA_DEPTH) % NB], ks + s, frag[s]);
    }
#pragma unroll
    for (int s = 0; s < NB - 1; s++)
        if (ks + s < ksteps) step(xs[s], afs[s], xs[(s + GEMM_MFMA_DEPTH) % NB], afs[(s + GEMM_MFMA_DEPTH) % NB], ks + s, frag[s]);
    if (!active) return;
    const uint32_t tot = C->rl_tot, olast = G * M - 1;
    int32_t oo[16];
#pragma unroll
    for (int r = 0; r < 16; r++) {
        const uint32_t mm = mt * 32 + (uint32_t)(r & 3) + 8u * (uint32_t)(r >> 2) + 4u * half;
        oo[r] = out_idx[min(g * M + mm, olast)];
        if (mm >= M) oo[r] = -1;
    }
#pragma unroll
    for (int d = 0; d < DG; d++) {
        if ((uint32_t)d >= cnt) continue;
#pragma unroll
        for (int r = 0; r < 16; r++) {
            if (oo[r] < 0) continue;
            double v = (double)acc[d][0][r];
#pragma unroll
            for (int j = 1; j < D; j++) v = __fma_rn((double)acc[d][j][r], (double)(1u << (8 * j)), v);
            S[((size_t)oo[r] * tot + g0 + d0 + (uint32_t)d) * n + (size_t)ctile * 32 + col] = v;
        }
    }
}

typedef uint64_t ps_u64x2 __attribute__((ext_vector_type(2)));
typedef double ps_f64x2 __attribute__((ext_vector_type(2)));
DEV uint64_t ps_reduce(uint64_t x, const DMod &m) {
    const uint64_t r = x - __umul64hi(x, m.r1) * m.q;
    return r >= m.q ? r - m.q : r;
}
template <int ND>
__global__ void __launch_bounds__(256) k_product_sum(const uint64_t *__restrict__ prod_, uint32_t K, uint64_t *__restrict__ out_, double *__restrict__ S_,
                                                     const DevConsts *__restrict__ C) {
    typedef const NTT_GLOBAL ps_u64x2 *In;
    constexpr int PF = 4;
    const uint32_t n = C->n, k = C->k, n2 = n >> 1, tiles = n >> 9;
    uint32_t b = blockIdx.x;
    const uint32_t tile = b % tiles; b /= tiles;
    const uint32_t l = b % k, o = b / k;
    const uint32_t p = tile * 256 + threadIdx.x;
    const uint32_t dbc = (uint32_t)C->dbc, mask = (1u << dbc) - 1, nd = C->rl_dig[l];
    uint32_t g0 = 0;
    for (uint32_t x = 0; x < l; x++) g0 += C->rl_dig[x];
    uint32_t sh[ND];
#pragma unroll
    for (int d = 0; d < ND; d++) sh[d] = min(dbc * (uint32_t)d, 63u);
    const size_t comp = (size_t)k * n2, unit = 3 * comp;
    const NTT_GLOBAL char *src = (const NTT_GLOBAL char *)prod_ + (size_t)o * K * unit * 16;
    const uint32_t lane_off = (l * n2 + p) * 16;
    uint64_t c0x = 0, c0y = 0, c1x = 0, c1y = 0, dx[ND], dy[ND];
#pragma unroll
    for (int d = 0; d < ND; d++) { dx[d] = 0; dy[d] = 0; }
    auto fetch = [&](ps_u64x2 (&x)[PF][3], uint32_t kk) {
#pragma unroll
        for (int t = 0; t < PF; t++) {
            const NTT_GLOBAL char *s = src + (size_t)min(kk + (uint32_t)t, K - 1) * unit * 16;
#pragma unroll
            for (int c = 0; c < 3; c++) x[t][c] = *(In)(s + (size_t)c * comp * 16 + lane_off);
        }
    };
    auto term = [&](const ps_u64x2 (&x)[3]) {
        c0x += x[0].x; c0y += x[0].y; c1x += x[1].x; c1y += x[1].y;
#pragma unroll
        for (int d = 0; d < ND; d++) { dx[d] += (uint32_t)(x[2].x >> sh[d]) & mask; dy[d] += (uint32_t)(x[2].y >> sh[d]) & mask; }
    };
    auto terms = [&](const ps_u64x2 (&x)[PF][3]) {
#pragma unroll
        for (int t = 0; t < PF; t++) term(x[t]);
    };
    auto tail = [&](const ps_u64x2 (&x)[PF][3], uint32_t nv) {
#pragma unroll
        for (int t = 0; t < PF; t++) if ((uint32_t)t < nv) term(x[t]);
    };
    {
        uint32_t kk = 0;
        ps_u64x2 xa[PF][3], xb[PF][3];
        fetch(xa, 0);
        for (uint32_t it = K / (2 * PF); it; it--, kk += 2 * PF) {
            fetch(xb, kk + PF);
            terms(xa);
            fetch(xa, kk + 2 * PF);
            terms(xb);
        }
        const uint32_t r = K - kk;
        if (r > PF) fetch(xb, kk + PF);
        tail(xa, min(r, (uint32_t)PF));
        if (r > PF) tail(xb, r - PF);
    }
    const DMod m = C->q[l];
    typedef NTT_GLOBAL ps_u64x2 *Out;
    Out dst = (Out)out_ + (size_t)o * 2 * comp + (size_t)l * n2 + p;
    ps_u64x2 v;
    v.x = ps_reduce(c0x, m); v.y = ps_reduce(c0y, m); dst[0] = v;
    v.x = ps_reduce(c1x, m); v.y = ps_reduce(c1y, m); dst[comp] = v;
    typedef NTT_GLOBAL ps_f64x2 *OutS;
    OutS sd = (OutS)S_ + ((size_t)o * C->rl_tot + g0) * n2 + p;
#pragma unroll
    for (int d = 0; d < ND; d++)
        if ((uint32_t)d < nd) { ps_f64x2 w; w.x = (double)dx[d]; w.y = (double)dy[d]; sd[(size_t)d * n2] = w; }
}
```

cryptonets_amd/csrc/cn_k_ks.hip.h:

```cpp
#pragma once
#include "cn_dev_common.hip.h"

template <class AR, int L> struct KsFwd { typedef AR P; static constexpr bool lds = false; };
template <int RN, int L> struct KsFwd<ArF64T<RN>, L> { typedef typename std::conditional<(L <= 13), ArF64LdsT<RN>, ArF64T<RN>>::type P; static constexpr bool lds = L <= 13; };
DEV void ks_premultiply(uint64_t (&raw)[16], const DevConsts *C, uint32_t l) {
    if (C->ks_xi) {
        const DMod ql = C->q[l]; const uint64_t f = C->ks_inv_qhat_q[l];
#pragma unroll
        for (int r = 0; r < 16; r++) raw[r] = mulmod(raw[r], f, ql);
    }
}
template <class AR> struct KsMac;
template <> struct KsMac<ArU64> {
    static DEV void mac(uint64_t &acc, uint64_t x, uint64_t key, const DMod &qm, const ArCtx<ArU64> &A) { acc = addmod(acc, mulmod(canon4(x, qm.q), key, qm), qm.q); }
    static DEV void settle(uint64_t (&)[16], const ArCtx<ArU64> &) {}
    static DEV uint64_t sum(uint64_t acc, uint64_t x, const DMod &qm) { return addmod(acc, x, qm.q); }
};
template <int RN> struct KsMac<ArF64T<RN>> {
    typedef ArF64T<RN> ArF64;
    static DEV void mac(double &acc, double x, double key, const DMod &, const ArCtx<ArF64> &A) { acc = __dadd_rn(acc, ArF64::mulmod(x, key, A.m)); }
    static DEV void settle(double (&a)[16], const ArCtx<ArF64> &A) { ArF64::renorm(a, A.m); }
    static DEV double sum(double acc, double x, const DMod &) { return __dadd_rn(acc, x); }
};
#ifndef KS_SGPR_A
#define KS_SGPR_A 1
#endif
template <class FW0, bool ON> struct KsPassA { typedef FW0 P; };
template <class FW0> struct KsPassA<FW0, true> { typedef ArPassA<FW0> P; };
#ifndef KS_PRE_SYNC
#define KS_PRE_SYNC 1
#endif
#ifndef KS_SRC_AHEAD
#define KS_SRC_AHEAD 0
#endif
#ifndef KS_MAC_FENCE
#define KS_MAC_FENCE 0
#endif
template <class AR> struct KsDigits {};
template <class AR> struct KsSrc { typedef AR P; static constexpr bool dig = false; };
template <class AR> struct KsSrc<KsDigits<AR>> { typedef AR P; static constexpr bool dig = true; };
template <int L, class AR_, int MINW = 1, bool TWL = false, bool XI = false>
__global__ void __launch_bounds__(NttPlan<L>::NT, MINW) k_keyswitch_rr(const uint64_t *__restrict__ target, size_t tgt_stride, const uint64_t *__restrict__ add0,
                                                                 const uint64_t *__restrict__ add1, size_t add_stride, const void *__restrict__ key_,
                                                                 uint64_t *out, const DevConsts *__restrict__ C, int galois, uint32_t accmax,
                                                                 const uint64_t *extra, size_t ex_stride, uint64_t *const *__restrict__ out_tab,
                                                                 uint32_t xcd_cts) {
    typedef typename KsSrc<AR_>::P AR;
    constexpr bool DIG = KsSrc<AR_>::dig;
    typedef typename AR::T T;
    static_assert(!DIG || (std::is_same<T, double>::value && !XI), "ready-made digits: FP64 policies, plain decomposition");
    extern __shared__ __align__(16) unsigned char smem[];
    T *s = reinterpret_cast<T *>(smem);
    constexpr uint32_t n = 1u << L;
    constexpr int SA = NttPlan<L>::SA;
    const uint32_t k = C->k, tid = threadIdx.x;
    uint32_t ct = blockIdx.x / k, j = blockIdx.x % k;
    if (xcd_cts & 0x80000000u) { const uint32_t cnt = gridDim.x / k; j = blockIdx.x / cnt; ct = blockIdx.x % cnt; }
    else if (blockIdx.x < xcd_cts * k) { const uint32_t x = blockIdx.x & 7, sl = blockIdx.x >> 3; ct = 8 * (sl / k) + x; j = sl % k; }
    const DMod qm = C->q[j];
    const uint64_t q = qm.q;
    const ArCtx<AR> A(C, j);
    const int dbc = galois ? C->gdbc : C->dbc;
    const uint64_t mask = (1ull << dbc) - 1;
    const size_t kn = (size_t)k * n;
    T acc0[16], acc1[16];
#pragma unroll
    for (int r = 0; r < 16; r++) { acc0[r] = 0; acc1[r] = 0; }
    typedef typename std::conditional<TWL, typename KsFwd<AR, L>::P, AR>::type FW0;
    typedef typename KsPassA<FW0, KS_SGPR_A && std::is_same<T, double>::value>::P FW;
    typename FW::Tw fwt;
    if constexpr (TWL) {
        static_assert(KsFwd<AR, L>::lds, "LDS twiddles need an FP64 policy and N <= 8192");
        double *tws = reinterpret_cast<double *>(smem) + ntt_lds_words(n);
        stage_table(tws, A.fw.w, n, tid, NttPlan<L>::NT);
        fwt.w = (const __attribute__((address_space(3))) double *)tws;
        __syncthreads();
    } else static_cast<typename FW0::Tw &>(fwt) = A.fw;
    if constexpr (HasPassA<FW>::value) ntt_load_pass_a<SA>(fwt, A.fw.w);
    const T *kp = reinterpret_cast<const T *>(key_);
    uint32_t terms = 0;
    uint64_t raw[16];
    constexpr bool AHEAD = KS_SRC_AHEAD && MINW == 1 && L <= 13;
    uint64_t nraw[AHEAD ? 16 : 1];
    auto request = [&](uint64_t (&w)[16], uint32_t l) {
        uint32_t t0 = tid;
        asm volatile("" : "+v"(t0));
        const uint64_t *src = target + (size_t)ct * tgt_stride + (size_t)l * n;
#pragma unroll
        for (int r = 0; r < 16; r++) w[r] = src[pass_index<L, SA, 0>(t0, r)];
    };
    if constexpr (AHEAD) request(nraw, 0);
    const double *dsrc = reinterpret_cast<const double *>(target) + (size_t)ct * tgt_stride;
    for (uint32_t l = 0; l < k; l++) {
        const uint32_t nd = galois ? C->gk_dig[l] : C->rl_dig[l];
        if constexpr (DIG) {
        } else if constexpr (AHEAD) {
#pragma unroll
            for (int r = 0; r < 16; r++) raw[r] = nraw[r];
            request(nraw, min(l + 1, k - 1));
        } else request(raw, l);
        if constexpr (XI) {
            const DMod ql = C->q[l]; const uint64_t xf = C->ks_inv_qhat_q[l];
#pragma unroll
            for (int r = 0; r < 16; r++) raw[r] = mulmod(raw[r], xf, ql);
        }
        for (uint32_t d = 0; d < nd; d++, kp += 2 * kn) {
            const int sh = dbc * (int)d;
            uint32_t tl = tid;
            asm volatile("" : "+v"(tl));
            T v[16];
            if constexpr (DIG) {
#pragma unroll
                for (int r = 0; r < 16; r++) v[r] = (T)dsrc[pass_index<L, SA, 0>(tl, r)];
                dsrc += n;
            } else {
#pragma unroll
            for (int r = 0; r < 16; r++) {
                uint64_t t = (raw[r] >> sh) & mask;
                if constexpr (std::is_same<T, uint64_t>::value) { if (mask >= q) t = t >= q ? bred128(t, 0, qm) : t; }
                v[r] = A.load(t);
            }
            if constexpr (std::is_same<T, double>::value) { if (mask >= q) AR::renorm(v, A.m); }
            }
            ntt_forward_regs<FW, L, KS_PRE_SYNC != 0>(v, s, fwt, A.m, tl);
            const T *k0 = kp + (size_t)j * n, *k1 = kp + kn + (size_t)j * n;
#pragma unroll
            for (int r = 0; r < 16; r += 2) {
                if (KS_MAC_FENCE || std::is_same<T, uint64_t>::value) __builtin_amdgcn_sched_barrier(0);
                const uint32_t pos = tail_index<L>(tl, r);
                struct alignas(16) P2 { T a, b; };
                const P2 a = *reinterpret_cast<const P2 *>(k0 + pos), b = *reinterpret_cast<const P2 *>(k1 + pos);
                KsMac<AR>::mac(acc0[r], v[r], a.a, qm, A); KsMac<AR>::mac(acc0[r + 1], v[r + 1], a.b, qm, A);
                KsMac<AR>::mac(acc1[r], v[r], b.a, qm, A); KsMac<AR>::mac(acc1[r + 1], v[r + 1], b.b, qm, A);
            }
            if (++terms == accmax) { terms = 0; KsMac<AR>::settle(acc0, A); KsMac<AR>::settle(acc1, A); }
            if (!KS_PRE_SYNC) __syncthreads();
        }
    }
    if (KS_PRE_SYNC && !ntt_tail_local<L>()) __syncthreads();
#pragma unroll 1
    for (int p = 0; p < 2; p++) {
        T v[16];
#pragma unroll
        for (int r = 0; r < 16; r++) v[r] = p ? acc1[r] : acc0[r];
        uint32_t tl = tid;
// ... 279 lines not shown
            }
        }
    }
}
template <class T> NTT_DEV void ks_load2(const NTT_GLOBAL T *p, T &a, T &b) {
    typedef T V2 __attribute__((ext_vector_type(2)));
    const V2 v = *reinterpret_cast<const NTT_GLOBAL V2 *>(p);
    a = v.x; b = v.y;
}
template <int L> NTT_DEV void ks_gather_automorphism(uint64_t (&raw)[16], const NTT_GLOBAL uint64_t *limb, uint32_t elt, uint64_t q, void *image, uint32_t tid) {
    constexpr uint32_t n = 1u << L, NT = NttPlan<L>::NT;
    uint64_t *s = reinterpret_cast<uint64_t *>(image);
#pragma unroll
    for (int r = 0; r < 16; r++) {
        const uint32_t i = tid + NT * (uint32_t)r, pos = (i * elt) & (2 * n - 1);
        const uint64_t v = limb[i];
        s[lds_pos(pos & (n - 1))] = (pos >> L) ? (v ? q - v : 0) : v;
    }
    __syncthreads();
#pragma unroll
    for (int r = 0; r < 16; r++) raw[r] = s[lds_pos(pass_index<L, NttPlan<L>::SA, 0>(tid, r))];
    __syncthreads();
}
template <int L, class AR_>
__global__ void __launch_bounds__(NttPlan<L>::NT) k_ks_digit_mac(const uint64_t *__restrict__ target, size_t tgt_stride, const void *__restrict__ key_,
                                                                  void *__restrict__ part_, const DevConsts *__restrict__ C, int galois, uint32_t tot, uint32_t perm_elt,
                                                                  const KsItem *__restrict__ items) {
    typedef typename KsSrc<AR_>::P AR;
    constexpr bool DIG = KsSrc<AR_>::dig;
    typedef typename AR::T T;
    extern __shared__ __align__(16) unsigned char smem[];
    T *s = reinterpret_cast<T *>(smem);
    constexpr uint32_t n = 1u << L;
    constexpr int SA = NttPlan<L>::SA;
    const uint32_t k = C->k, tid = threadIdx.x;
    const uint32_t j = blockIdx.x % k, g = (blockIdx.x / k) % tot, ct = blockIdx.x / (k * tot);
    uint32_t l = 0, d = g;
    for (;; l++) { const uint32_t nd = galois ? C->gk_dig[l] : C->rl_dig[l]; if (d < nd) break; d -= nd; }
    const DMod qm = C->q[j];
    const uint64_t q = qm.q;
    const ArCtx<AR> A(C, j);
    const int dbc = galois ? C->gdbc : C->dbc, sh = dbc * (int)d;
    const uint64_t mask = (1ull << dbc) - 1;
    const size_t kn = (size_t)k * n;
    const NTT_GLOBAL uint64_t *src = (const NTT_GLOBAL uint64_t *)target + (size_t)ct * tgt_stride + (size_t)l * n;
    const NTT_GLOBAL T *keyp = (const NTT_GLOBAL T *)key_;
    if (items) {
        const KsItem it = items[ct];
        src = (const NTT_GLOBAL uint64_t *)it.in + kn + (size_t)l * n; keyp = (const NTT_GLOBAL T *)it.key; perm_elt = it.elt;
    }
    T v[16];
    if constexpr (DIG) {
        static_assert(std::is_same<T, double>::value, "ready-made digits: FP64 policies");
        const double *dsrc = reinterpret_cast<const double *>(target) + (size_t)ct * tgt_stride + (size_t)g * n;
#pragma unroll
        for (int r = 0; r < 16; r++) v[r] = (T)dsrc[pass_index<L, SA, 0>(tid, r)];
    } else {
    uint64_t raw[16];
    if (perm_elt) ks_gather_automorphism<L>(raw, src, perm_elt, C->q[l].q, s, tid);
    else {
#pragma unroll
        for (int r = 0; r < 16; r++) raw[r] = src[pass_index<L, SA, 0>(tid, r)];
    }
    ks_premultiply(raw, C, l);
#pragma unroll
    for (int r = 0; r < 16; r++) {
        uint64_t t = (raw[r] >> sh) & mask;
        if constexpr (std::is_same<T, uint64_t>::value) { if (mask >= q) t = t >= q ? bred128(t, 0, qm) : t; }
        v[r] = A.load(t);
    }
    if constexpr (std::is_same<T, double>::value) { if (mask >= q) AR::renorm(v, A.m); }
    }
    ntt_forward_regs<AR, L>(v, s, A.fw, A.m, tid);
    const NTT_GLOBAL T *k0 = keyp + (size_t)g * 2 * kn + (size_t)j * n, *k1 = k0 + kn;
    T *o0 = reinterpret_cast<T *>(part_) + (((size_t)ct * tot + g) * 2) * kn + (size_t)j * n, *o1 = o0 + kn;
    struct alignas(16) P2 { T a, b; };
#pragma unroll
    for (int r = 0; r < 16; r += 2) {
        const uint32_t pos = tail_index<L>(tid, r);
        P2 a, b;
        ks_load2<T>(k0 + pos, a.a, a.b); ks_load2<T>(k1 + pos, b.a, b.b);
        P2 x = {0, 0}, y = {0, 0};
        KsMac<AR>::mac(x.a, v[r], a.a, qm, A); KsMac<AR>::mac(x.b, v[r + 1], a.b, qm, A);
        KsMac<AR>::mac(y.a, v[r], b.a, qm, A); KsMac<AR>::mac(y.b, v[r + 1], b.b, qm, A);
        *reinterpret_cast<P2 *>(o0 + pos) = x; *reinterpret_cast<P2 *>(o1 + pos) = y;
    }
}
template <int L, class AR_>
__global__ void __launch_bounds__(NttPlan<L>::NT) k_ks_limb_mac(const uint64_t *__restrict__ target, size_t tgt_stride, const void *__restrict__ key_,
                                                                 void *__restrict__ part_, const DevConsts *__restrict__ C, int galois, uint32_t accmax, uint32_t perm_elt,
                                                                 const KsItem *__restrict__ items) {
    typedef typename KsSrc<AR_>::P AR;
    constexpr bool DIG = KsSrc<AR_>::dig;
    typedef typename AR::T T;
    extern __shared__ __align__(16) unsigned char smem[];
    T *s = reinterpret_cast<T *>(smem);
    constexpr uint32_t n = 1u << L;
    constexpr int SA = NttPlan<L>::SA;
    const uint32_t k = C->k, tid = threadIdx.x;
    const uint32_t j = blockIdx.x % k, l = (blockIdx.x / k) % k, ct = blockIdx.x / (k * k);
    const DMod qm = C->q[j];
    const uint64_t q = qm.q;
    const ArCtx<AR> A(C, j);
    const int dbc = galois ? C->gdbc : C->dbc;
    const uint64_t mask = (1ull << dbc) - 1;
    const size_t kn = (size_t)k * n;
    uint32_t g0 = 0;
    for (uint32_t i = 0; i < l; i++) g0 += galois ? C->gk_dig[i] : C->rl_dig[i];
    const uint32_t nd = galois ? C->gk_dig[l] : C->rl_dig[l];
    const NTT_GLOBAL uint64_t *src = (const NTT_GLOBAL uint64_t *)target + (size_t)ct * tgt_stride + (size_t)l * n;
    const NTT_GLOBAL T *keyp = (const NTT_GLOBAL T *)key_;
    if (items) {
        const KsItem it = items[ct];
        src = (const NTT_GLOBAL uint64_t *)it.in + kn + (size_t)l * n; keyp = (const NTT_GLOBAL T *)it.key; perm_elt = it.elt;
    }
    uint64_t raw[16];
    if constexpr (DIG) static_assert(std::is_same<T, double>::value, "ready-made digits: FP64 policies");
    else {
    if (perm_elt) ks_gather_automorphism<L>(raw, src, perm_elt, C->q[l].q, s, tid);
    else {
        uint32_t t0 = tid;
        asm volatile("" : "+v"(t0));
#pragma unroll
        for (int r = 0; r < 16; r++) raw[r] = src[pass_index<L, SA, 0>(t0, r)];
    }
    ks_premultiply(raw, C, l);
    }
    const double *dsrc = reinterpret_cast<const double *>(target) + (size_t)ct * tgt_stride + (size_t)g0 * n;
    T acc0[16], acc1[16];
#pragma unroll
    for (int r = 0; r < 16; r++) { acc0[r] = 0; acc1[r] = 0; }
    const NTT_GLOBAL T *kp = keyp + (size_t)g0 * 2 * kn;
    uint32_t terms = 0;
    for (uint32_t d = 0; d < nd; d++, kp += 2 * kn) {
        const int sh = dbc * (int)d;
        uint32_t tl = tid;
        asm volatile("" : "+v"(tl));
        T v[16];
        if constexpr (DIG) {
#pragma unroll
            for (int r = 0; r < 16; r++) v[r] = (T)dsrc[pass_index<L, SA, 0>(tl, r)];
            dsrc += n;
        } else {
#pragma unroll
        for (int r = 0; r < 16; r++) {
            uint64_t t = (raw[r] >> sh) & mask;
            if constexpr (std::is_same<T, uint64_t>::value) { if (mask >= q) t = t >= q ? bred128(t, 0, qm) : t; }
            v[r] = A.load(t);
        }
        if constexpr (std::is_same<T, double>::value) { if (mask >= q) AR::renorm(v, A.m); }
        }
        ntt_forward_regs<AR, L, KS_PRE_SYNC != 0>(v, s, A.fw, A.m, tl);
        const NTT_GLOBAL T *k0 = kp + (size_t)j * n, *k1 = kp + kn + (size_t)j * n;
#pragma unroll
        for (int r = 0; r < 16; r += 2) {
            const uint32_t pos = tail_index<L>(tl, r);
            struct alignas(16) P2 { T a, b; };
            P2 a, b;
            ks_load2<T>(k0 + pos, a.a, a.b); ks_load2<T>(k1 + pos, b.a, b.b);
            KsMac<AR>::mac(acc0[r], v[r], a.a, qm, A); KsMac<AR>::mac(acc0[r + 1], v[r + 1], a.b, qm, A);
            KsMac<AR>::mac(acc1[r], v[r], b.a, qm, A); KsMac<AR>::mac(acc1[r + 1], v[r + 1], b.b, qm, A);
        }
        if (++terms == accmax) { terms = 0; KsMac<AR>::settle(acc0, A); KsMac<AR>::settle(acc1, A); }
        if (!KS_PRE_SYNC) __syncthreads();
    }
    KsMac<AR>::settle(acc0, A); KsMac<AR>::settle(acc1, A);
    T *o0 = reinterpret_cast<T *>(part_) + (((size_t)ct * k + l) * 2) * kn + (size_t)j * n, *o1 = o0 + kn;
    struct alignas(16) P2 { T a, b; };
#pragma unroll
    for (int r = 0; r < 16; r += 2) {
        const uint32_t pos = tail_index<L>(tid, r);
        *reinterpret_cast<P2 *>(o0 + pos) = P2{acc0[r], acc0[r + 1]};
        *reinterpret_cast<P2 *>(o1 + pos) = P2{acc1[r], acc1[r + 1]};
    }
}
template <int L, class AR>
__global__ void __launch_bounds__(NttPlan<L>::NT) k_ks_sum_intt(const void *__restrict__ part_, const uint64_t *__restrict__ add0, const uint64_t *__restrict__ add1,
                                                                 size_t add_stride, uint64_t *out, const DevConsts *__restrict__ C, uint32_t tot,
                                                                 uint32_t accmax, const uint64_t *extra, size_t ex_stride, uint64_t *const *__restrict__ out_tab, uint32_t perm_elt,
                                                                 const KsItem *__restrict__ items) {
    typedef typename AR::T T;
// ... 46 lines not shown
```

cryptonets_amd/csrc/cn_l_gemm.hip:

```cpp
#include "cn_runtime.h"
#include <algorithm>
#include "cn_k_gemm.hip.h"

struct GemmGrid { dim3 grid; uint32_t order; };
static GemmGrid gemm_grid(cn_ctx *c, const GemmLaunch &g, uint32_t mtiles) {
    const uint32_t slices = c->chunks * g.polys * c->hc.k;
    if (g.order == 1 && (slices & 7) == 0 && (c->chunks & (c->chunks - 1)) == 0 && (uint64_t)8 * mtiles * g.G < (1ull << 31) && slices / 8 < 65536)
        return {dim3(8 * mtiles * g.G, slices / 8), 1u};
    return {dim3((uint32_t)((size_t)slices * mtiles * g.G)), 0u};
}
template <int MT, bool ABS> static void launch_int(cn_ctx *c, const GemmLaunch &g) {
    const uint32_t mtiles = (g.M + MT - 1) / MT;
    const GemmGrid gg = gemm_grid(c, g, mtiles);
    hipLaunchKernelGGL((k_scalar_gemm<MT, ABS>), gg.grid, dim3(c->bs), 0, c->stream, g.in, g.idx, (const uint64_t *)g.W, g.oidx, g.bias, g.bidx, g.out, c->dc,
                       c->chunks, g.G, g.M, g.K, mtiles, g.lazy, g.Kp, g.obase, g.polys, gg.order, GemmUnits{g.in_unit, g.out_unit, g.bias_unit});
}
template <int MT, bool ABS> static void launch_f64(cn_ctx *c, const GemmLaunch &g) {
    const uint32_t mtiles = (g.M + MT - 1) / MT;
    const GemmGrid gg = gemm_grid(c, g, mtiles);
    if (g.one) hipLaunchKernelGGL((k_scalar_gemm_f64<MT, 1, 0, ABS>), gg.grid, dim3(c->bs), 0, c->stream, g.in, g.idx, (const double *)g.W, g.oidx, g.bias,
                                  g.bidx, g.out, c->dc, c->chunks, g.G, g.M, g.K, mtiles, g.lazy, g.Kp, g.obase, g.polys, gg.order, gemm_f64_rows(g.K), GemmUnits{g.in_unit, g.out_unit, g.bias_unit});
    else if (g.two) hipLaunchKernelGGL((k_scalar_gemm_f64<MT, 2, 22, ABS>), gg.grid, dim3(c->bs), 0, c->stream, g.in, g.idx, (const double *)g.W, g.oidx, g.bias,
                                  g.bidx, g.out, c->dc, c->chunks, g.G, g.M, g.K, mtiles, g.lazy, g.Kp, g.obase, g.polys, gg.order, gemm_f64_rows(g.K), GemmUnits{g.in_unit, g.out_unit, g.bias_unit});
    else hipLaunchKernelGGL((k_scalar_gemm_f64<MT, 3, 17, ABS>), gg.grid, dim3(c->bs), 0, c->stream, g.in, g.idx, (const double *)g.W, g.oidx, g.bias,
                            g.bidx, g.out, c->dc, c->chunks, g.G, g.M, g.K, mtiles, g.lazy, g.Kp, g.obase, g.polys, gg.order, gemm_f64_rows(g.K), GemmUnits{g.in_unit, g.out_unit, g.bias_unit});
}
template <bool ABS> static int launch(cn_ctx *c, const GemmLaunch &g) {
    if (g.small) {
        switch (g.MT) {
            case 20: launch_f64<20, ABS>(c, g); break;
            case 10: launch_f64<10, ABS>(c, g); break;
            case 5: launch_f64<5, ABS>(c, g); break;
            case 1: launch_f64<1, ABS>(c, g); break;
            default: return cn_fail(CN_ERR_ARG, "internal: scalar GEMM tile %u", g.MT);
        }
    } else {
        switch (g.MT) {
            case 10: launch_int<10, ABS>(c, g); break;
            case 5: launch_int<5, ABS>(c, g); break;
            case 1: launch_int<1, ABS>(c, g); break;
            default: return cn_fail(CN_ERR_ARG, "internal: scalar GEMM tile %u", g.MT);
        }
    }
    HIPCHK(hipGetLastError());
    cn_launch_count(c);
    return 0;
}
int cn_l_gemm(cn_ctx *c, const GemmLaunch &g) { return g.abs ? launch<true>(c, g) : launch<false>(c, g); }

template <int P, bool ABS> static void launch_mfma(cn_ctx *c, const GemmLaunch &g) {
    const uint32_t mgroups = (g.mtiles + 3) / 4;
    const size_t blocks = (size_t)g.G * mgroups * g.polys * c->hc.k * (c->hc.n / 32);
    hipLaunchKernelGGL((k_scalar_gemm_mfma<P, ABS>), dim3((uint32_t)blocks), dim3(256), 0, c->stream, g.in, g.idx, (const int8_t *)g.W, g.oidx, g.bias, g.bidx, g.out,
                       c->dc, g.G, g.M, g.mtiles, g.ksteps, g.obase, g.polys, GemmUnits{g.in_unit, g.out_unit, g.bias_unit});
}
template <bool ABS> static int launch_mfma_p(cn_ctx *c, const GemmLaunch &g) {
    switch (g.P) {
        case 1: launch_mfma<1, ABS>(c, g); break;
        case 2: launch_mfma<2, ABS>(c, g); break;
        case 3: launch_mfma<3, ABS>(c, g); break;
        default: return cn_fail(CN_ERR_ARG, "internal: %u weight digit planes", g.P);
    }
    HIPCHK(hipGetLastError());
    cn_launch_count(c);
    return 0;
}
int cn_l_gemm_mfma(cn_ctx *c, const GemmLaunch &g) { return g.abs ? launch_mfma_p<true>(c, g) : launch_mfma_p<false>(c, g); }

template <int MT> static void launch_digit(cn_ctx *c, const DigitGemmLaunch &g, uint32_t ndg, uint32_t mtiles) {
    const size_t blocks = (size_t)(c->hc.n >> 8) * c->hc.k * ndg * mtiles * g.G;
    hipLaunchKernelGGL((k_digit_gemm<MT, 5>), dim3((uint32_t)blocks), dim3(256), 0, c->stream, g.in, g.in_unit, (const int32_t *)g.idx, (const double *)g.W,
                       (const int32_t *)g.oidx, g.S, c->dc, g.G, g.M, g.K, mtiles, g.Kp, g.Kw, ndg);
}
template <int P, int DG> static void launch_digit_mfma(cn_ctx *c, const DigitGemmLaunch &g, uint32_t ndg, size_t blocks) {
    hipLaunchKernelGGL((k_digit_gemm_mfma<P, DG>), dim3((uint32_t)blocks), dim3(256), 0, c->stream, g.in, g.in_unit, (const int32_t *)g.idx, (const int8_t *)g.W,
                       (const int32_t *)g.oidx, g.S, c->dc, g.G, g.M, g.mtiles, g.ksteps, ndg);
}
static int digit_gemm_mfma(cn_ctx *c, const DigitGemmLaunch &g, uint32_t ndmax) {
    const uint32_t DG = digit_gemm_mfma_group(g.P), ndg = (ndmax + DG - 1) / DG, mgroups = (g.mtiles + 3) / 4;
    const uint64_t blocks = (uint64_t)g.G * mgroups * c->hc.k * (c->hc.n / 32) * ndg;
    if ((c->hc.n & 255) || !g.ksteps || blocks >= (1ull << 31)) return cn_fail(CN_ERR_ARG, "internal: digit GEMM grid");
    switch (g.P) {
        case 1: launch_digit_mfma<1, 3>(c, g, ndg, blocks); break;
        case 2: launch_digit_mfma<2, 3>(c, g, ndg, blocks); break;
        case 3: launch_digit_mfma<3, 2>(c, g, ndg, blocks); break;
        default: return cn_fail(CN_ERR_ARG, "internal: %u weight digit planes", g.P);
    }
    HIPCHK(hipGetLastError());
    cn_launch_count(c);
    c->dg_mfma++;
    return 0;
}
int cn_l_digit_gemm(cn_ctx *c, const DigitGemmLaunch &g) {
    uint32_t ndmax = 0; for (uint32_t l = 0; l < c->hc.k; l++) ndmax = std::max(ndmax, c->hc.rl_dig[l]);
    if (g.mfma) return digit_gemm_mfma(c, g, ndmax);
    const uint32_t ndg = (ndmax + 4) / 5, mtiles = (g.M + g.MT - 1) / g.MT;
    if ((c->hc.n & 255) || (uint64_t)(c->hc.n >> 8) * c->hc.k * ndg * mtiles * g.G >= (1ull << 31)) return cn_fail(CN_ERR_ARG, "internal: digit GEMM grid");
    switch (g.MT) {
        case 10: launch_digit<10>(c, g, ndg, mtiles); break;
        case 2: launch_digit<2>(c, g, ndg, mtiles); break;
        default: return cn_fail(CN_ERR_ARG, "internal: digit GEMM tile %u", g.MT);
    }
    HIPCHK(hipGetLastError());
    cn_launch_count(c);
    return 0;
}

template <int ND> static void launch_product_sum(cn_ctx *c, const ProductSumLaunch &g, uint32_t blocks) {
    hipLaunchKernelGGL((k_product_sum<ND>), dim3(blocks), dim3(256), 0, c->stream, g.prod, g.K, g.out, g.S, c->dc);
}
int cn_l_product_sum(cn_ctx *c, const ProductSumLaunch &g) {
    uint32_t ndmax = 0; for (uint32_t l = 0; l < c->hc.k; l++) ndmax = std::max(ndmax, c->hc.rl_dig[l]);
    const uint64_t blocks = (uint64_t)(c->hc.n >> 9) * c->hc.k * g.outputs;
    if ((c->hc.n & 511) || !g.K || !g.outputs || ndmax > PRODUCT_SUM_MAX_DIGITS || c->hc.dbc > 31 || blocks >= (1ull << 31)) return cn_fail(CN_ERR_ARG, "internal: product sum grid");
    if (ndmax <= 2) launch_product_sum<2>(c, g, (uint32_t)blocks);
    else if (ndmax <= 4) launch_product_sum<4>(c, g, (uint32_t)blocks);
    else if (ndmax <= 5) launch_product_sum<5>(c, g, (uint32_t)blocks);
    else launch_product_sum<8>(c, g, (uint32_t)blocks);
    HIPCHK(hipGetLastError());
    cn_launch_count(c);
    return 0;
}
```

cryptonets_amd/csrc/cn_l_ks.inc.h:

```cpp
#include "cn_runtime.h"
#include "cn_k_ks.hip.h"

typedef KS_POLICY AR;
static constexpr bool kF64 = std::is_same<typename AR::T, double>::value;

static constexpr size_t PAIR14_LDS = (size_t)ntt_lds_words(8192) * 8 + 65536;
template <class K> static int big_lds(K kern, size_t bytes) {
    HIPCHK(hipFuncSetAttribute((const void *)kern, hipFuncAttributeMaxDynamicSharedMemorySize, (int)bytes));
    return 0;
}
template <int L> static size_t ks_twl_lds() { return ((size_t)ntt_lds_words(1u << L) + (1u << L)) * 8; }
template <int L> static int set_attrs_l(size_t bytes) {
    CHECK(big_lds(k_keyswitch_rr<L, AR>, bytes)); CHECK(big_lds(k_keyswitch_rr<L, AR, 1, false, true>, bytes));
    if constexpr (KsFwd<AR, L>::lds) { CHECK(big_lds(k_keyswitch_rr<L, AR, 1, true>, ks_twl_lds<L>())); CHECK(big_lds(k_keyswitch_rr<L, AR, 1, true, true>, ks_twl_lds<L>())); }
    CHECK(big_lds(k_ks_digit_mac<L, AR>, bytes)); CHECK(big_lds(k_ks_limb_mac<L, AR>, bytes)); CHECK(big_lds(k_ks_sum_intt<L, AR>, bytes));
    if constexpr (kF64) {
        CHECK(big_lds(k_keyswitch_rr<L, KsDigits<AR>, 1, false, false>, bytes));
        if constexpr (KsFwd<AR, L>::lds) CHECK(big_lds(k_keyswitch_rr<L, KsDigits<AR>, 1, true, false>, ks_twl_lds<L>()));
        CHECK(big_lds(k_ks_digit_mac<L, KsDigits<AR>>, bytes)); CHECK(big_lds(k_ks_limb_mac<L, KsDigits<AR>>, bytes));
    }
    return 0;
}
static int set_attrs(uint32_t logn, size_t bytes) {
    if constexpr (kF64) { if (logn == 12) { CHECK(big_lds(k_keyswitch_rr<12, AR, 1, true>, ks_twl_lds<12>())); CHECK(big_lds(k_keyswitch_rr<12, AR, 1, true, true>, ks_twl_lds<12>()));
                                           CHECK(big_lds(k_keyswitch_rr<12, KsDigits<AR>, 1, true, false>, ks_twl_lds<12>())); } }
    if (logn == 13) CHECK(set_attrs_l<13>(bytes));
    if (logn == 14) {
        CHECK(set_attrs_l<14>(bytes));
        if constexpr (kF64) {
            CHECK(big_lds(k_keyswitch_split14<AR>, (size_t)ntt_lds_words(8192) * 8)); CHECK(big_lds(k_keyswitch_split14<AR, true>, (size_t)ntt_lds_words(8192) * 8));
            CHECK(big_lds(k_keyswitch_pair14<AR, false, false>, PAIR14_LDS)); CHECK(big_lds(k_keyswitch_pair14<AR, true, false>, PAIR14_LDS));
            CHECK(big_lds(k_keyswitch_pair14<AR, false, true>, PAIR14_LDS)); CHECK(big_lds(k_keyswitch_pair14<AR, true, true>, PAIR14_LDS));
        }
    }
    return 0;
}
static const uint32_t KS_TWL_MIN_DIGITS = 12;
template <int L, bool XI, bool DIG = false> static void launch_fused_x(cn_ctx *c, const KsArgs &a) {
    const uint32_t tot = a.galois ? c->hc.gk_tot : c->hc.rl_tot;
    typedef typename std::conditional<DIG, KsDigits<AR>, AR>::type ARS;
    const uint64_t *tgt = DIG ? (const uint64_t *)a.dig : a.target;
    const size_t tstride = DIG ? (size_t)tot * c->hc.n : a.tstride;
    if constexpr (KsFwd<AR, L>::lds) {
        if (tot >= KS_TWL_MIN_DIGITS) {
            hipLaunchKernelGGL((k_keyswitch_rr<L, ARS, 1, true, XI>), dim3(a.cnt * c->hc.k), dim3(NttPlan<L>::NT), ks_twl_lds<L>(), c->stream, tgt, tstride, a.add0, a.add1,
                               a.astride, (const void *)a.key, a.out, c->dc, a.galois, a.accmax, a.extra, a.xstride, a.out_tab, a.xcd_cts);
            return;
        }
    }
    hipLaunchKernelGGL((k_keyswitch_rr<L, ARS, 1, false, XI>), dim3(a.cnt * c->hc.k), dim3(NttPlan<L>::NT), (size_t)ntt_lds_words(1u << L) * 8, c->stream, tgt, tstride,
                       a.add0, a.add1, a.astride, (const void *)a.key, a.out, c->dc, a.galois, a.accmax, a.extra, a.xstride, a.out_tab, a.xcd_cts);
}
template <int L> static void launch_fused(cn_ctx *c, const KsArgs &a) {
    if constexpr (kF64) { if (a.dig) { launch_fused_x<L, false, true>(c, a); return; } }
    if (c->hc.ks_xi) launch_fused_x<L, true>(c, a);
    else launch_fused_x<L, false>(c, a);
}
template <int L> static void launch_two_phase(cn_ctx *c, const KsArgs &a) {
    const uint32_t tot = a.galois ? c->hc.gk_tot : c->hc.rl_tot, k = c->hc.k;
    const size_t lds = (size_t)ntt_lds_words(1u << L) * 8;
    bool dig = false;
    if constexpr (kF64) dig = a.dig != nullptr;
    if (dig) {
        if constexpr (kF64) {
            if (a.mode == 2) hipLaunchKernelGGL((k_ks_limb_mac<L, KsDigits<AR>>), dim3(a.cnt * k * k), dim3(NttPlan<L>::NT), lds, c->stream, (const uint64_t *)a.dig, (size_t)tot * c->hc.n,
                                                (const void *)a.key, c->ks_part, c->dc, a.galois, a.accmax, 0u, (const KsItem *)nullptr);
            else hipLaunchKernelGGL((k_ks_digit_mac<L, KsDigits<AR>>), dim3(a.cnt * tot * k), dim3(NttPlan<L>::NT), lds, c->stream, (const uint64_t *)a.dig, (size_t)tot * c->hc.n,
                                    (const void *)a.key, c->ks_part, c->dc, a.galois, tot, 0u, (const KsItem *)nullptr);
        }
        hipLaunchKernelGGL((k_ks_sum_intt<L, AR>), dim3(a.cnt * k * 2), dim3(NttPlan<L>::NT), lds, c->stream, (const void *)c->ks_part, a.add0, a.add1, a.astride,
                           a.out, c->dc, a.mode == 2 ? k : tot, a.mode == 2 ? 0xffffffffu : a.accmax, a.extra, a.xstride, a.out_tab, a.perm_elt, a.items);
    } else if (a.mode == 2) {
        hipLaunchKernelGGL((k_ks_limb_mac<L, AR>), dim3(a.cnt * k * k), dim3(NttPlan<L>::NT), lds, c->stream, a.target, a.tstride, (const void *)a.key, c->ks_part,
                           c->dc, a.galois, a.accmax, a.perm_elt, a.items);
        hipLaunchKernelGGL((k_ks_sum_intt<L, AR>), dim3(a.cnt * k * 2), dim3(NttPlan<L>::NT), lds, c->stream, (const void *)c->ks_part, a.add0, a.add1, a.astride,
                           a.out, c->dc, k, 0xffffffffu, a.extra, a.xstride, a.out_tab, a.perm_elt, a.items);
    } else {
        hipLaunchKernelGGL((k_ks_digit_mac<L, AR>), dim3(a.cnt * tot * k), dim3(NttPlan<L>::NT), lds, c->stream, a.target, a.tstride, (const void *)a.key, c->ks_part,
                           c->dc, a.galois, tot, a.perm_elt, a.items);
        hipLaunchKernelGGL((k_ks_sum_intt<L, AR>), dim3(a.cnt * k * 2), dim3(NttPlan<L>::NT), lds, c->stream, (const void *)c->ks_part, a.add0, a.add1, a.astride,
                           a.out, c->dc, tot, a.accmax, a.extra, a.xstride, a.out_tab, a.perm_elt, a.items);
    }
    cn_launch_count(c);
}
template <int L> static void launch_rr(cn_ctx *c, const KsArgs &a) {
    if (a.mode) { launch_two_phase<L>(c, a); return; }
    launch_fused<L>(c, a);
}
static bool launch(cn_ctx *c, const KsArgs &a) {
    switch (c->hc.logn) {
        case 10: launch_rr<10>(c, a); return true;
        case 11: launch_rr<11>(c, a); return true;
        case 12: launch_rr<12>(c, a); return true;
        case 13: launch_rr<13>(c, a); return true;
        case 14: launch_rr<14>(c, a); return true;
        default: return false;
    }
}
static bool split14(cn_ctx *c, const KsArgs &a) {
    if constexpr (kF64) {
        if (c->hc.ks_xi)
            hipLaunchKernelGGL((k_keyswitch_split14<AR, true>), dim3(a.cnt * c->hc.k * 2), dim3(NttPlan<13>::NT), (size_t)ntt_lds_words(8192) * 8, c->stream, a.target, a.tstride,
                               (const void *)a.key, (uint64_t *)c->ks_part, c->dc, a.galois, a.accmax);
        else
            hipLaunchKernelGGL((k_keyswitch_split14<AR>), dim3(a.cnt * c->hc.k * 2), dim3(NttPlan<13>::NT), (size_t)ntt_lds_words(8192) * 8, c->stream, a.target, a.tstride,
                               (const void *)a.key, (uint64_t *)c->ks_part, c->dc, a.galois, a.accmax);
        return true;
    }
    return false;
}
template <bool XI, bool WHOLE> static void launch_pair14(cn_ctx *c, const KsArgs &a) {
    if constexpr (kF64)
        hipLaunchKernelGGL((k_keyswitch_pair14<AR, XI, WHOLE>), dim3(a.cnt * c->hc.k), dim3(NttPlan<13>::NT), PAIR14_LDS, c->stream, a.target, a.tstride, a.add0, a.add1, a.astride,
                           (const void *)a.key, a.out, (double *)c->ks_part, c->dc, a.galois, a.accmax, a.extra, a.xstride, a.out_tab, a.perm_elt, a.next_elt, a.next_out, a.xcd_cts);
}
static bool pair14(cn_ctx *c, const KsArgs &a0) {
    if constexpr (kF64) {
        KsArgs a = a0;
        const CnModRange qr = cn_mod_range(c->hc, 0, c->hc.k);
        if (!qr.light && qr.bits <= 49) a.accmax = std::max(a.accmax, 1u << (52 - qr.bits));
        const int dbc = a.galois ? c->hc.gdbc : c->hc.dbc;
// ... 11 lines not shown
```

cryptonets_amd/csrc/cn_level.hip:

```cpp
#include "cn_api_shared.h"

static int slice_polys(cn_ctx *child, uint64_t *dst, const uint64_t *src, size_t rows, uint32_t k_src, uint32_t k_dst) {
    const size_t n = child->hc.n;
    HIPCHK(hipMemcpy2DAsync(dst, k_dst * n * 8, src, k_src * n * 8, k_dst * n * 8, rows, hipMemcpyDeviceToDevice, child->stream));
    return 0;
}
static int slice_ks_key(cn_ctx *child, const cn_ctx *parent, const KsKey &from, KsKey &to, int which) {
    const size_t words = cn_key_words(child, which);
    HIPCHK(hipMalloc((void **)&to.d, words * 8));
    to.owned = true; to.f64 = from.f64;
    CHECK(slice_polys(child, to.d, from.d, words / ((size_t)child->hc.k * child->hc.n), parent->hc.k, child->hc.k));
    const bool want = keys_as_f64(child);
    if (want != to.f64) {
        if (want) hipLaunchKernelGGL(k_u64_to_f64, dim3((unsigned)((words + 255) / 256)), dim3(256), 0, child->stream, to.d, words);
        else hipLaunchKernelGGL(k_f64_to_u64, dim3((unsigned)((words + 255) / 256)), dim3(256), 0, child->stream, to.d, words);
        HIPCHK(hipGetLastError());
        to.f64 = want;
    }
    return 0;
}
static int adopt_from_parent(cn_ctx *c, cn_ctx *parent) {
    const uint32_t k = c->hc.k;
    c->opt = parent->opt; c->defer_square_gemm = parent->defer_square_gemm; c->mul_sum = parent->mul_sum;
    memcpy(c->rng_key, parent->rng_key, sizeof c->rng_key);
    c->hc.ks_xi = parent->hc.ks_xi;
    for (uint32_t l = 0; l < k; l++) c->hc.ks_inv_qhat_q[l] = parent->hc.ks_inv_qhat_q[l];
    HIPCHK(hipMemcpy(c->dc, &c->hc, sizeof(DevConsts), hipMemcpyHostToDevice));
    HIPCHK(hipStreamSynchronize(parent->stream));
    const size_t kn = (size_t)k * c->hc.n;
    if (parent->rlk.d) CHECK(slice_ks_key(c, parent, parent->rlk, c->rlk, 0));
    for (auto &kv : parent->gk) if (kv.second.d) CHECK(slice_ks_key(c, parent, kv.second, c->gk[kv.first], 1));
    if (parent->pk) { HIPCHK(hipMalloc((void **)&c->pk, 2 * kn * 8)); CHECK(slice_polys(c, c->pk, parent->pk, 2, parent->hc.k, k)); }
    if (parent->sk) { HIPCHK(hipMalloc((void **)&c->sk, kn * 8)); HIPCHK(hipMemcpyAsync(c->sk, parent->sk, kn * 8, hipMemcpyDeviceToDevice, c->stream)); }
    HIPCHK(hipStreamSynchronize(c->stream));
    c->level = true;
    return 0;
}
extern "C" int cn_ctx_create_level(cn_ctx *parent, uint32_t limbs, cn_ctx **out) {
    if (!parent || !out) return fail(CN_ERR_ARG, "null argument");
    if (limbs == 0 || limbs >= parent->hc.k) return fail(CN_ERR_ARG, "a level keeps 1 .. %u of the %u coefficient moduli (got %u)", parent->hc.k - 1, parent->hc.k, limbs);
    uint64_t q[CN_MAXK];
    for (uint32_t j = 0; j < limbs; j++) q[j] = parent->hc.q[j].q;
    cn_ctx *c = nullptr;
    CHECK(cn_ctx_create(parent->hc.n, q, limbs, parent->hc.t.q, parent->hc.dbc, parent->hc.gdbc, parent->device, &c));
    const int rc = [&]() -> int {
        cn_ctx *ctx = parent;
        return ctx->mu.run([&]() -> int { LOCK; NOT_CAPTURING("cn_ctx_create_level"); return adopt_from_parent(c, parent); });
    }();
    if (rc) {
        char msg[256]; snprintf(msg, sizeof msg, "%s", cn_last_error());
        (void)cn_ctx_destroy(c);
        return fail(rc, "%s", msg);
    }
    *out = c;
    return 0;
}

int flush_all(cn_ctx *ctx) { CHECK(use(ctx)); CHECK(ring_sync(ctx, true)); return cn_defer_flush(ctx); }
static int chain_check(const cn_ctx *src, const cn_ctx *dst, const char *what) {
    const DevConsts &a = src->hc, &b = dst->hc;
    if (src->device != dst->device) return fail(CN_ERR_ARG, "%s: the target context is on another device", what);
    if (a.n != b.n || a.t.q != b.t.q) return fail(CN_ERR_ARG, "%s: the target context has another N or t", what);
    if (b.k >= a.k) return fail(CN_ERR_ARG, "%s: the target keeps %u of the source's %u coefficient moduli (must be fewer)", what, b.k, a.k);
    for (uint32_t j = 0; j < b.k; j++) if (a.q[j].q != b.q[j].q) return fail(CN_ERR_ARG, "%s: the target's coefficient modulus is not a prefix of the source's", what);
    if (a.ks_xi != b.ks_xi) return fail(CN_ERR_ARG, "%s: the contexts use different key-switch conventions (ks_xi)", what);
    if (a.ks_xi) for (uint32_t j = 0; j < b.k; j++) if (a.ks_inv_qhat_q[j] != b.ks_inv_qhat_q[j])
        return fail(CN_ERR_ARG, "%s: under ks_xi = 1 the target must be a level of the source's chain (cn_ctx_create_level)", what);
    return 0;
}
static int mod_switch_locked(cn_ctx *src, cn_handle in, uint32_t ii, uint32_t count, cn_ctx *dst, cn_handle out, uint32_t oi) {
    if ((src->capturing || dst->capturing) && !(src->cap_root && src->cap_root == dst->cap_root)) {
        cn_ctx *ctx = src->capturing ? src : dst; NOT_CAPTURING("cn_mod_switch (other than between the contexts of one cn_graph_begin_levels)");
    }
    CHECK(chain_check(src, dst, "cn_mod_switch"));
    const DevConsts &a = src->hc, &b = dst->hc;
    {   cn_ctx *ctx = src; CHECK(flush_all(ctx)); }
// ... 67 lines not shown
```

cryptonets_amd/csrc/cn_policy.h:

```cpp
#pragma once
#include "cn_internal.h"

enum { POL_U64 = 0, POL_F64 = 1, POL_F64L = 2 };

struct CnModRange {
    bool f64ok;
    bool light;
    int bits;
    uint64_t qmax;
};
inline CnModRange cn_mod_range(const DevConsts &hc, uint32_t base_off, uint32_t nmod) {
    CnModRange r{true, true, 0, 0};
    for (uint32_t m = base_off; m < base_off + nmod; m++) {
        const uint64_t q = m < hc.k ? hc.q[m].q : (m < hc.k + hc.kb ? hc.bsk[m - hc.k].q : hc.t.q);
        r.f64ok = r.f64ok && hc.f64ok[m];
        if (q > r.qmax) r.qmax = q;
    }
    r.light = !(r.qmax >> 44);
    r.bits = r.qmax ? 64 - __builtin_clzll(r.qmax) : 0;
    return r;
}
inline int cn_policy(const CnModRange &r, bool use_f64) { return !(use_f64 && r.f64ok) ? POL_U64 : (r.light ? POL_F64L : POL_F64); }
inline bool cn_rr_size(uint32_t logn, uint32_t max_logn = 14) { return logn >= 10 && logn <= max_logn; }
```

cryptonets_amd/csrc/cn_runtime.h:

```cpp
#pragma once
#include "../../include/cnhip.h"
#include "cn_policy.h"
#include "cn_submit.h"
#include <hip/hip_runtime.h>
#include <atomic>
#include <cstring>
#include <map>
#include <memory>
#include <mutex>
#include <set>
#include <string>
#include <type_traits>
#include <unordered_map>
#include <vector>

int cn_fail(int code, const char *fmt, ...);
#define HIPCHK(x) do { hipError_t e_ = (x); if (e_ != hipSuccess) return cn_fail(CN_ERR_HIP, "%s failed: %s", #x, hipGetErrorString(e_)); } while (0)
#define CHECK(x) do { int rc_ = (x); if (rc_) return rc_; } while (0)

struct GemmPlan;
struct cn_ctx;
struct CapturedGraph {
    hipGraph_t graph = nullptr; hipGraphExec_t exec = nullptr;
    std::vector<std::unique_ptr<char[]>> staged;
// ... 107 lines not shown
struct DeferQueue;
struct cn_ctx {
    int device = 0;
    hipStream_t stream = nullptr;
    CnTunables opt;
    DevConsts hc;
    DevConsts *dc = nullptr;
    uint64_t *tw = nullptr;
    CnMutex mu;
    HandleTable bufs;
    KsKey rlk{nullptr, false, false};
    double *twd = nullptr, *twdh = nullptr;
    std::map<uint64_t, KsKey> gk;
    uint64_t *sk = nullptr, *pk = nullptr;
    uint64_t rng_item = 0;
    uint32_t rng_key[8] = {0, 0, 0, 0, 0, 0, 0, 0};
    char *scratch = nullptr; size_t scap = 0, soff = 0, smax;
    std::vector<std::unique_ptr<char[]>> staged;
    cn_stats st{};
    hipEvent_t ev0 = nullptr, ev1 = nullptr;
    hipEvent_t ev_order = nullptr;
    uint32_t bs, chunks;
    std::vector<uint32_t> index_map;
    uint32_t *d_index_map = nullptr;
    size_t ctw2;
    std::unordered_map<size_t, std::vector<uint64_t *>> pool;
    size_t pool_bytes = 0, pool_max;
    void *slabs = nullptr;
    void *ks_part = nullptr; size_t ks_part_cap = 0;
    char *pin = nullptr, *pin_dev = nullptr; size_t pin_off = 0; uint32_t pin_laps = 0;
    char *stage = nullptr; size_t stage_cap = 0;
    int stream_tries = 0;
    std::atomic<int> probe_pins{0};
    std::atomic<bool> capturing{false};
    std::vector<std::unique_ptr<char[]>> cap_staged;
    std::vector<std::pair<uint64_t *, size_t>> cap_allocs;
    int graphs_alive = 0;
    cn_ctx *cap_root = nullptr;
    std::vector<cn_ctx *> cap_members;
    hipStream_t own_stream = nullptr;
    int member_graphs = 0;
    hipEvent_t ev_graph = nullptr;
    int cus = 0;
    uint64_t folded_zero = 0;
    uint64_t mr_pipelined = 0;
    uint64_t sg_fused = 0;
    uint64_t dsg_fused = 0;
    uint64_t dg_mfma = 0;
    std::atomic<uint64_t> packed_bad{0};
    uint64_t ms_fused = 0;
    uint32_t ms_groups = 0;
    bool mul_sum = true;
    bool digit_mfma = true;
    bool defer_square_gemm = false;
    uint64_t uid = 0;
    hipStream_t stream2 = nullptr; hipEvent_t ev_fork = nullptr, ev_join = nullptr; bool stream2_failed = false;
    std::atomic<int> defer{0};
    DeferQueue *dq = nullptr;
    SubmitRing *ring = nullptr;
    ReadyRing *ready = nullptr;
    int async_rc = 0; std::string async_msg;
    bool level = false;
    bool rec_steps = false, rec_cols = false;
    std::set<int> rec_set;
    hipEvent_t ev_ms = nullptr;
    bool ms_f64 = false;
};

struct KsItem { const uint64_t *in; const void *key; uint32_t elt, pad; };
struct KsCall {
    const uint64_t *target = nullptr; size_t tstride = 0;
    const uint64_t *add0 = nullptr, *add1 = nullptr; size_t astride = 0;
    uint64_t *out = nullptr; uint32_t cnt = 0; int galois = 0;
    const uint64_t *extra = nullptr; size_t xstride = 0;
    uint64_t *const *out_tab = nullptr;
    const KsItem *items = nullptr;
    uint32_t perm_elt = 0;
    uint32_t next_elt = 0; uint64_t *next_out = nullptr;
    const double *dig = nullptr;
    static KsCall relin(const uint64_t *prod, size_t kn, uint32_t cnt) {
        return {.target = prod + 2 * kn, .tstride = 3 * kn, .add0 = prod, .add1 = prod + kn, .astride = 3 * kn, .cnt = cnt};
    }
    static KsCall relin_digits(const double *S, const uint64_t *base, size_t kn, uint32_t cnt) { return {.add0 = base, .add1 = base + kn, .astride = 2 * kn, .cnt = cnt, .dig = S}; }
    static KsCall galois_of(const uint64_t *c1, size_t c1_stride, const uint64_t *c0, size_t kn, uint32_t cnt) {
        return {.target = c1, .tstride = c1_stride, .add0 = c0, .astride = 2 * kn, .cnt = cnt, .galois = 1};
    }
    static KsCall galois_items(const KsItem *items, uint32_t cnt) { return {.cnt = cnt, .galois = 1, .items = items}; }
    KsCall &to(uint64_t *dense) { out = dense; return *this; }
    KsCall &to_table(uint64_t *const *tab) { out_tab = tab; return *this; }
    KsCall &plus(const uint64_t *acc, size_t stride) { extra = acc; xstride = stride; return *this; }
    KsCall &perm(uint32_t elt) { perm_elt = elt; return *this; }
    KsCall &next(uint32_t elt, uint64_t *nout) { next_elt = elt; next_out = nout; return *this; }
};
struct KsArgs : KsCall {
    const uint64_t *key;
    uint32_t accmax;
    int mode;
    uint32_t xcd_cts = 0;
};
struct FoldOut { uint64_t *out; uint32_t first, count; };
struct FoldTerm { double w; uint32_t enc, pad; };
struct RrOps {
    int (*set_attrs)(uint32_t logn, size_t lds);
    bool (*ntt)(cn_ctx *c, uint64_t *data, uint32_t limbs, uint32_t base_off, uint32_t nmod, int inverse);
    bool (*intt_tensor)(cn_ctx *c, const uint64_t *A, const uint64_t *B, uint64_t *D, uint32_t cnt, uint32_t base_off, uint32_t Lm, bool lazy);
    bool (*square_fused)(cn_ctx *c, const uint64_t *A, size_t astride, const uint64_t *const *atab, uint64_t *D, uint32_t cnt, uint32_t base_off, uint32_t Lm);
    bool (*mul_plain_fused)(cn_ctx *c, const uint64_t *pt, uint32_t pitch, uint32_t npt, uint64_t *lift, const uint64_t *src, size_t sstride, uint32_t pstride,
                            uint64_t *out, uint32_t count, uint32_t polys);
    bool (*enc_tail)(cn_ctx *c, const uint64_t *u, const uint64_t *pt, uint32_t pts, uint64_t *out, uint32_t cnt, const int8_t *noise, const void *tab);
    bool (*enc_fused)(cn_ctx *c, const int8_t *us, const uint64_t *pt, uint32_t pts, uint64_t *out, uint32_t cnt, const int8_t *noise, const void *tab);
    bool (*mul_plain_bcast)(cn_ctx *c, const uint64_t *pt, uint32_t pitch, const uint64_t *ctn, uint64_t *out, uint32_t count, uint32_t polys, uint32_t next_elt,
                            uint64_t *next_out);
    bool (*enc_fold)(cn_ctx *c, const int8_t *us, const int8_t *noise, const void *fout, const void *terms, uint32_t outputs);
};
struct KsOps {
    int (*set_attrs)(uint32_t logn, size_t lds);
    bool (*launch)(cn_ctx *c, const KsArgs &a);
    bool (*split14)(cn_ctx *c, const KsArgs &a);
    bool (*pair14)(cn_ctx *c, const KsArgs &a);
};
extern const RrOps cn_rr_u64, cn_rr_f64, cn_rr_f64l;
extern const KsOps cn_ks_u64, cn_ks_f64, cn_ks_f64l;

int cn_l_behz_extend(cn_ctx *c, const uint64_t *src, uint32_t stride, const uint64_t *const *src_tab, uint64_t *aq, uint64_t *ab, uint32_t cnt);
int cn_l_behz_floor(cn_ctx *c, const uint64_t *dq, const uint64_t *db, uint64_t *out, uint32_t cnt, bool lazy);
inline bool cn_behz_lazy(const cn_ctx *c) { return c->hc.behz_f64 && c->opt.f64; }

struct GemmLaunch {
    bool small, two, abs; uint32_t MT;
    const uint64_t *in; const void *idx; const void *W; const void *oidx; const uint64_t *bias; const void *bidx; uint64_t *out;
    uint32_t G, M, K, lazy, Kp, obase;
    uint32_t P = 0, mtiles = 0, ksteps = 0;
    uint32_t polys = 2;
    uint32_t order = 0;
    bool one = false;
    uint32_t in_unit = 0, out_unit = 0, bias_unit = 0;
};
inline uint32_t gemm_f64_rows(uint32_t K) { return ((K + 15) & ~15u) + 16; }
int cn_l_gemm(cn_ctx *c, const GemmLaunch &g);
int cn_l_gemm_mfma(cn_ctx *c, const GemmLaunch &g);
struct DigitGemmLaunch {
    const uint64_t *in; size_t in_unit; const void *idx; const void *W; const void *oidx; double *S;
    uint32_t G, M, K, Kp, Kw, MT;
    bool mfma = false; uint32_t P = 0, mtiles = 0, ksteps = 0;
};
inline uint32_t digit_gemm_mfma_group(uint32_t P) { return P <= 2 ? 3u : 2u; }
inline uint32_t digit_gemm_tile(uint32_t M) { return M > 2 ? 10u : 2u; }
inline uint32_t digit_gemm_rows(uint32_t K) { return ((K + 7) & ~7u) + 8; }
int cn_l_digit_gemm(cn_ctx *c, const DigitGemmLaunch &g);
struct ProductSumLaunch { const uint64_t *prod; uint32_t K; uint64_t *out; double *S; uint32_t outputs; };
static const uint32_t PRODUCT_SUM_MAX_DIGITS = 8;
int cn_l_product_sum(cn_ctx *c, const ProductSumLaunch &g);
struct MulPlainSumLaunch { const uint64_t *pt, *ctn; const uint32_t *grp_off, *slot; uint64_t *out; uint32_t groups, accmax; };
int cn_l_mul_plain_sum(cn_ctx *c, int policy, const MulPlainSumLaunch &a);
bool cn_l_mul_plain_sum_kernel(int policy, uint32_t logn);
int cn_l_diag_set_attrs(uint32_t logn, size_t lds);
int cn_l_mod_switch(cn_ctx *c, const uint64_t *src, uint64_t *dst, const DevConsts *src_consts, uint32_t ks, uint32_t kd, uint32_t items, uint32_t logn,
                    bool f64, bool *ran_f64);
int cn_l_noise_norm(cn_ctx *c, const uint64_t *c0, size_t ct_stride, const uint64_t *acc, uint64_t *out, uint32_t count);
int cn_l_crt_join(cn_ctx *c, const uint64_t *plain, const uint32_t *index_map, const void *tab, uint32_t P, uint32_t W, double *values, uint64_t *words, uint32_t count, uint32_t nslots);
int cn_l_join_argmax(cn_ctx *c, const uint64_t *words, uint32_t W, int32_t *argmax, uint32_t count, uint32_t nslots);
int cn_l_crt_split(cn_ctx *c, const void *values, int64_t stride_ct, int64_t stride_slot, uint32_t count, uint32_t nvalues, uint32_t flags, double scale,
                   const uint64_t *t, uint64_t *const *dst, uint32_t P, const uint32_t *index_map, uint32_t *nz, uint32_t nz_stride, uint32_t *bad);
struct SeededArgs {
    uint64_t *out; size_t ct_stride; uint32_t cnt; bool expand_only;
    const uint8_t *a_seed32; uint64_t a_nonce, a_item0;
    const int8_t *noise; const uint64_t *pt; uint32_t pt_stride_words;
};
int cn_l_seeded(cn_ctx *c, const SeededArgs &a);
size_t cn_packed_row_words(const cn_ctx *c);
int cn_l_unpack_rows(cn_ctx *c, const uint64_t *packed, uint64_t *arr, size_t item_words, uint32_t cnt, uint32_t polys, uint32_t *flag, hipStream_t stream = nullptr);
int cn_l_pack_rows(cn_ctx *c, const uint64_t *arr, size_t item_words, uint64_t *packed, uint32_t cnt, uint32_t polys, hipStream_t stream = nullptr);
struct KskGenArgs {
    const void *outs, *fac; const uint16_t *perm; const int8_t *noise;
    uint64_t seed, item0; uint32_t elts, tot; bool f64out;
};
int cn_l_ksk_gen(cn_ctx *c, const KskGenArgs &a);

inline void cn_launch_count(cn_ctx *c, int n = 1) { c->st.kernel_launches += n; }
```

Measured before the change: 1.205 million.

## Store relinearization digit sums as int32 when bounded sums fit

Adds an int32 storage path for the intermediate digit matrix S that the digit GEMM, product-sum and MFMA digit GEMM kernels write and the key-switch kernels read. A bound check on the summed absolute weights times the maximum digit decides when the values fit in 32 bits. Otherwise the existing double path is kept. The aim is to halve the scratch footprint and the memory traffic of S between the digit producer and the key switch, at the cost of more template instantiations and a new conversion path inside the key-switch kernels.

```diff
diff --git a/cryptonets_amd/csrc/cn_api.hip b/cryptonets_amd/csrc/cn_api.hip
--- a/cryptonets_amd/csrc/cn_api.hip
+++ b/cryptonets_amd/csrc/cn_api.hip
@@ -326,6 +326,7 @@
     }
     if (!strcmp(name, "defer_square_gemm")) { ctx->defer_square_gemm = value != 0; return 0; }
     if (!strcmp(name, "digit_mfma")) { ctx->digit_mfma = value != 0; defer_square_drop_plans(ctx); return 0; }
+    if (!strcmp(name, "digit_i32")) { ctx->digit_i32 = value != 0; defer_square_drop_plans(ctx); return 0; }
     if (!strcmp(name, "mul_sum")) { ctx->mul_sum = value != 0; return 0; }
     if (!strcmp(name, "record_steps")) {
         ctx->rec_steps = value != 0;
@@ -342,6 +343,7 @@
     else if (!strcmp(name, "ks_xi")) *value = (int)ctx->hc.ks_xi;
     else if (!strcmp(name, "record_steps")) *value = ctx->rec_steps;
     else if (!strcmp(name, "digit_mfma")) *value = ctx->digit_mfma;
+    else if (!strcmp(name, "digit_i32")) *value = ctx->digit_i32;
     else if (!strcmp(name, "defer_square_gemm")) *value = ctx->defer_square_gemm;
     else if (!strcmp(name, "mul_sum")) *value = ctx->mul_sum;
     else if (!strcmp(name, "pin_laps")) *value = (int)ctx->pin_laps;
@@ -354,6 +356,7 @@
     else if (!strcmp(name, "mul_sum_min_k")) *value = (int)MUL_SUM_MIN_K;
     else if (!strcmp(name, "defer_pending_products")) *value = (int)ctx->dq->sq->out.size();
     else if (!strcmp(name, "digit_gemm_mfma")) *value = (int)std::min<uint64_t>(ctx->dg_mfma, 0x7fffffff);
+    else if (!strcmp(name, "ks_digits_i32")) *value = (int)std::min<uint64_t>(ctx->ks_dig_i32, 0x7fffffff);
     else if (!strcmp(name, "packed_bad_residues")) *value = (int)std::min<uint64_t>(ctx->packed_bad.load(), 0x7fffffff);
     else if (!strcmp(name, "mul_relin_pipelined")) *value = (int)std::min<uint64_t>(ctx->mr_pipelined, 0x7fffffff);
     else if (!strcmp(name, "behz_small_base")) *value = ctx->hc.bsk[ctx->hc.kb - 1].q < (1ull << 49);
diff --git a/cryptonets_amd/csrc/cn_api_shared.h b/cryptonets_amd/csrc/cn_api_shared.h
--- a/cryptonets_amd/csrc/cn_api_shared.h
+++ b/cryptonets_amd/csrc/cn_api_shared.h
@@ -85,7 +85,7 @@
     std::vector<char> host;
     size_t off_oidx = 0, off_bidx = 0, off_w = 0;
     char *dev = nullptr;
-    bool dig = false, dig_mfma = false; uint32_t dMT = 0, dKw = 0; size_t off_dw = 0;
+    bool dig = false, dig_mfma = false, dig_i32 = false; uint32_t dMT = 0, dKw = 0; size_t off_dw = 0;
 };
 struct SgPlan {
     bool ok = false, bias = false; uint32_t O = 0, K = 0;
diff --git a/cryptonets_amd/csrc/cn_defer.hip b/cryptonets_amd/csrc/cn_defer.hip
--- a/cryptonets_amd/csrc/cn_defer.hip
+++ b/cryptonets_amd/csrc/cn_defer.hip
@@ -275,7 +275,7 @@
 }
 static size_t sg_scratch(cn_ctx *ctx, const GemmPlan &P) {
     const size_t kn = (size_t)ctx->hc.k * ctx->hc.n;
-    return al((size_t)P.O * 2 * kn * 8) + al((size_t)P.O * ctx->hc.rl_tot * ctx->hc.n * 8) + al((size_t)P.G * P.Kp * 4) + al((size_t)P.G * P.M * 4) + al((size_t)P.O * 8) + 8192;
+    return al((size_t)P.O * 2 * kn * 8) + al((size_t)P.O * ctx->hc.rl_tot * ctx->hc.n * (P.dig_i32 ? 4 : 8)) + al((size_t)P.G * P.Kp * 4) + al((size_t)P.G * P.M * 4) + al((size_t)P.O * 8) + 8192;
 }
 static bool sg_prepare(cn_ctx *ctx, DeferQueue *q, const std::vector<uint8_t> &dead, const std::map<const uint64_t *, size_t> &freed, std::vector<SgGroup> &groups,
                        std::vector<int32_t> &sg_of, std::vector<uint8_t> &need) {
@@ -353,7 +353,7 @@
     for (uint32_t o = 0; o < P.O; o++) outs[o] = g.rows[o]->out;
     CHECK(ensure_scratch(ctx, sg_scratch(ctx, P)));
     uint64_t *T = salloc<uint64_t>(ctx, (size_t)P.O * 2 * kn);
-    double *S = salloc<double>(ctx, (size_t)P.O * tot * n);
+    void *S = salloc<char>(ctx, (size_t)P.O * tot * n * (P.dig_i32 ? 4 : 8));
     if (!T || !S) return fail(CN_ERR_HIP, "internal: scratch exhausted in the deferred square + dense form");
     int32_t *dpidx, *dbidx; uint64_t **douts;
     CHECK(upload_tmp(ctx, pidx.data(), pidx.size(), &dpidx)); CHECK(upload_tmp(ctx, bidx.data(), bidx.size(), &dbidx)); CHECK(upload_tmp(ctx, outs.data(), outs.size(), &douts));
@@ -361,8 +361,9 @@
     CHECK(launch_gemm_plan(ctx, P, P.dev, dpidx, arr, (uint32_t)(3 * kn), 2u, bias ? (const uint64_t *)bbase : nullptr, dbidx, 32, T, 0));
     DigitGemmLaunch dg{arr + 2 * kn, 3 * kn, dpidx, P.dev + P.off_dw, P.dev + P.off_oidx, S, P.G, P.M, P.K, P.Kp, P.dKw, P.dMT};
     if (P.dig_mfma) { dg.W = P.dev + P.off_w; dg.mfma = true; dg.P = P.P; dg.mtiles = P.mtiles; dg.ksteps = P.ksteps; }
+    dg.i32 = P.dig_i32;
     CHECK(cn_l_digit_gemm(ctx, dg));
-    CHECK(do_keyswitch(ctx, ctx->rlk, KsCall::relin_digits(S, T, kn, P.O).to_table(douts)));
+    CHECK(do_keyswitch(ctx, ctx->rlk, KsCall::relin_digits(S, P.dig_i32, T, kn, P.O).to_table(douts)));
     ctx->dsg_fused++;
     if (defer_trace()) fprintf(stderr, "defer %p level %d: fuses %u scalar products over %zu pending products (GEMM, digit GEMM%s, %u key switches)\n", (void *)ctx, g.level, P.O,
                                g.slot_of.size(), P.dig_mfma ? " on the matrix cores" : "", P.O);
diff --git a/cryptonets_amd/csrc/cn_eval.hip b/cryptonets_amd/csrc/cn_eval.hip
--- a/cryptonets_amd/csrc/cn_eval.hip
+++ b/cryptonets_amd/csrc/cn_eval.hip
@@ -304,14 +304,16 @@
         uint64_t qmin = ~0ull; for (uint32_t j = 0; j < ctx->hc.k; j++) qmin = std::min(qmin, ctx->hc.q[j].q);
         const uint64_t dmax = (1ull << ctx->hc.dbc) - 1, lim = std::min<uint64_t>((qmin - 1) / 2, (1ull << 52) - 1) / dmax;
         bool ok = true;
+        uint64_t sum_max = 0;
         for (uint32_t g = 0; g < G && ok; g++) for (uint32_t m = 0; m < M && ok; m++) {
             const uint64_t *wr = row(g, m);
             if (!wr) continue;
             uint64_t sum = 0;
             for (uint32_t kk = 0; kk < K; kk++) if (hidx[(size_t)g * Kp + kk] >= 0) { const uint64_t w = wr[kk]; sum += w >= ctx->hc.t_half ? t - w : w; }
             ok = sum <= lim;
-        }
-        if (ok) { P.dig = true; P.dig_mfma = mfma && ctx->digit_mfma && ctx->hc.dbc <= 14 && !(ctx->hc.n & 255); }
+            sum_max = std::max(sum_max, sum);
+        }
+        if (ok) { P.dig = true; P.dig_mfma = mfma && ctx->digit_mfma && ctx->hc.dbc <= 14 && !(ctx->hc.n & 255); P.dig_i32 = ctx->digit_i32 && cn_digit_sum_fits_i32(sum_max, ctx->hc.dbc); }
         if (ok && !P.dig_mfma) {
             P.dMT = digit_gemm_tile(M); P.dKw = digit_gemm_rows(K);
             const uint32_t mtd = (M + P.dMT - 1) / P.dMT;
@@ -541,6 +543,7 @@
         }
     }
     HIPCHK(hipGetLastError()); launch_count(ctx);
+    if (a.dig && a.dig_i32) ctx->ks_dig_i32++;
     ctx->st.ntt_forward_limbs += (uint64_t)cnt * tot_dig * k; ctx->st.ntt_inverse_limbs += (uint64_t)cnt * 2 * k;
     return 0;
 }
@@ -637,7 +640,8 @@
     const uint32_t n = ctx->hc.n, k = ctx->hc.k, tot = ctx->hc.rl_tot;
     const size_t kn = (size_t)k * n;
     const size_t per = mul_scratch_per_ct(ctx, true);
-    const size_t fixed = al((size_t)cnt * 3 * kn * 8) + al((size_t)P.O * tot * n * 8) + 8192;
+    const size_t sw = P.dig_i32 ? 4 : 8;
+    const size_t fixed = al((size_t)cnt * 3 * kn * 8) + al((size_t)P.O * tot * n * sw) + 8192;
     if (!square_gemm_fused_ok(ctx, P) || fixed + per > ctx->smax) {
         cn_handle tmp = 0;
         CHECK(alloc_buf(ctx, 0, cnt, 2, &tmp));
@@ -651,7 +655,7 @@
     const uint32_t ch = (uint32_t)std::min<size_t>(cnt, (ctx->smax - fixed) / per);
     CHECK(ensure_scratch(ctx, fixed + per * ch + 4096));
     uint64_t *t3 = salloc<uint64_t>(ctx, (size_t)cnt * 3 * kn);
-    double *S = salloc<double>(ctx, (size_t)P.O * tot * n);
+    void *S = salloc<char>(ctx, (size_t)P.O * tot * n * sw);
     if (!t3 || !S) return fail(CN_ERR_HIP, "internal: scratch exhausted in cn_square_gemm");
     const size_t mark = ctx->soff;
     const uint64_t *pa = I->d + ii * I->item_words;
@@ -663,9 +667,10 @@
     CHECK(run_gemm_plan(ctx, P, P.dev, nullptr, OB, oi, t3));
     DigitGemmLaunch dg{t3 + 2 * kn, 3 * kn, P.dev, P.dev + P.off_dw, P.dev + P.off_oidx, S, P.G, P.M, P.K, P.Kp, P.dKw, P.dMT};
     if (P.dig_mfma) { dg.W = P.dev + P.off_w; dg.mfma = true; dg.P = P.P; dg.mtiles = P.mtiles; dg.ksteps = P.ksteps; }
+    dg.i32 = P.dig_i32;
     CHECK(cn_l_digit_gemm(ctx, dg));
     uint64_t *o = OB->d + oi * OB->item_words;
-    CHECK(do_keyswitch(ctx, ctx->rlk, KsCall::relin_digits(S, o, kn, P.O).to(o)));
+    CHECK(do_keyswitch(ctx, ctx->rlk, KsCall::relin_digits(S, P.dig_i32, o, kn, P.O).to(o)));
     ctx->st.Relinarization += cnt; ctx->sg_fused++;
     return 0;
 API_END }
@@ -725,7 +730,9 @@
         return rc;
     }
     const size_t per = mul_scratch_per_ct(ctx, false);
-    const size_t per_out = (size_t)K * 3 * kn * 8 + (size_t)tot * n * 8 + (size_t)K * 16, slack = 4 * 256 + 8192;
+    const bool s32 = ctx->digit_i32 && cn_digit_sum_fits_i32(K, ctx->hc.dbc);
+    const size_t sw = s32 ? 4 : 8;
+    const size_t per_out = (size_t)K * 3 * kn * 8 + (size_t)tot * n * sw + (size_t)K * 16, slack = 4 * 256 + 8192;
     const size_t g_fit = ctx->smax > per + slack ? (ctx->smax - per - slack) / per_out : 0;
     if (!mul_sum_fused_ok(ctx, K) || !g_fit) {
         cn_handle tmp = 0;
@@ -742,11 +749,11 @@
     std::vector<const uint64_t *> ha((size_t)g * K), hb((size_t)g * K);
     for (uint32_t o0 = 0; o0 < count; o0 += g) {
         const uint32_t go = std::min(g, count - o0), np = go * K;
-        const size_t fixed = al((size_t)np * 3 * kn * 8) + al((size_t)go * tot * n * 8) + 2 * al((size_t)np * 8) + 8192;
+        const size_t fixed = al((size_t)np * 3 * kn * 8) + al((size_t)go * tot * n * sw) + 2 * al((size_t)np * 8) + 8192;
         const uint32_t ch = (uint32_t)std::min<size_t>(np, std::max<size_t>(1, (ctx->smax - std::min(ctx->smax, fixed)) / per));
         CHECK(ensure_scratch(ctx, fixed + per * ch + 4096));
         uint64_t *t3 = salloc<uint64_t>(ctx, (size_t)np * 3 * kn);
-        double *S = salloc<double>(ctx, (size_t)go * tot * n);
+        void *S = salloc<char>(ctx, (size_t)go * tot * n * sw);
         if (!t3 || !S) return fail(CN_ERR_HIP, "internal: scratch exhausted in cn_mul_relin_sum");
         for (uint32_t i = 0; i < go; i++) for (uint32_t kk = 0; kk < K; kk++) {
             const Buffer *A = getbuf(ctx, a[kk], 0), *B = getbuf(ctx, b[kk], 0);
@@ -762,8 +769,8 @@
             CHECK(do_multiply(ctx, nullptr, 1, nullptr, 1, t3 + (size_t)s * 3 * kn, c, da + s, db + s));
         }
         uint64_t *o = O->d + (size_t)(oi + o0) * O->item_words;
-        CHECK(cn_l_product_sum(ctx, ProductSumLaunch{t3, K, o, S, go}));
-        CHECK(do_keyswitch(ctx, ctx->rlk, KsCall::relin_digits(S, o, kn, go).to(o)));
+        CHECK(cn_l_product_sum(ctx, ProductSumLaunch{t3, K, o, S, go, s32}));
+        CHECK(do_keyswitch(ctx, ctx->rlk, KsCall::relin_digits(S, s32, o, kn, go).to(o)));
         ctx->ms_groups++;
     }
     ctx->st.Relinarization += (uint64_t)K * count; ctx->st.AddMany += count; ctx->st.AddManyItemCount += (uint64_t)count * K;
diff --git a/cryptonets_amd/csrc/cn_k_gemm.hip.h b/cryptonets_amd/csrc/cn_k_gemm.hip.h
--- a/cryptonets_amd/csrc/cn_k_gemm.hip.h
+++ b/cryptonets_amd/csrc/cn_k_gemm.hip.h
@@ -397,9 +397,11 @@
     }
 }
 
-template <int MT, int DG>
+template <class... E> struct DigitWord { typedef double type; };
+template <> struct DigitWord<int32_t> { typedef int32_t type; };
+template <int MT, int DG, class... E>
 __global__ void __launch_bounds__(256) k_digit_gemm(const uint64_t *__restrict__ in, size_t in_unit, const int32_t *__restrict__ idx, const double *__restrict__ Wd,
-                                                    const int32_t *__restrict__ out_idx, double *__restrict__ S, const DevConsts *__restrict__ C, uint32_t G, uint32_t M,
+                                                    const int32_t *__restrict__ out_idx, typename DigitWord<E...>::type *__restrict__ S, const DevConsts *__restrict__ C, uint32_t G, uint32_t M,
                                                     uint32_t K, uint32_t mtiles, uint32_t Kp, uint32_t Kw, uint32_t ndg) {
     const uint32_t n = C->n, k = C->k, chunks = n >> 8;
     uint32_t chunk, lj, mt, g;
@@ -468,13 +470,13 @@
         if (o < 0) continue;
 #pragma unroll
         for (int d = 0; d < DG; d++)
-            if (d0 + (uint32_t)d < nd) S[((size_t)o * tot + g0 + d0 + (uint32_t)d) * n + i] = acc[d][m];
+            if (d0 + (uint32_t)d < nd) S[((size_t)o * tot + g0 + d0 + (uint32_t)d) * n + i] = (typename DigitWord<E...>::type)acc[d][m];
     }
 }
 
-template <int P, int DG>
+template <int P, int DG, class... E>
 __global__ void __launch_bounds__(256, 2) k_digit_gemm_mfma(const uint64_t *__restrict__ in, size_t in_unit, const int32_t *__restrict__ idx, const int8_t *__restrict__ Wf,
-                                                            const int32_t *__restrict__ out_idx, double *__restrict__ S, const DevConsts *__restrict__ C, uint32_t G,
+                                                            const int32_t *__restrict__ out_idx, typename DigitWord<E...>::type *__restrict__ S, const DevConsts *__restrict__ C, uint32_t G,
                                                             uint32_t M, uint32_t mtiles, uint32_t ksteps, uint32_t ndg) {
     constexpr int NP = 2 * DG, D = P + 1, NB = GEMM_MFMA_DEPTH + 1;
     __shared__ __align__(16) uint32_t frag[NB][NP][64][4];
@@ -580,10 +582,18 @@
 #pragma unroll
         for (int r = 0; r < 16; r++) {
             if (oo[r] < 0) continue;
-            double v = (double)acc[d][0][r];
-#pragma unroll
-            for (int j = 1; j < D; j++) v = __fma_rn((double)acc[d][j][r], (double)(1u << (8 * j)), v);
-            S[((size_t)oo[r] * tot + g0 + d0 + (uint32_t)d) * n + (size_t)ctile * 32 + col] = v;
+            typename DigitWord<E...>::type *dst = S + ((size_t)oo[r] * tot + g0 + d0 + (uint32_t)d) * n + (size_t)ctile * 32 + col;
+            if constexpr (std::is_same<typename DigitWord<E...>::type, int32_t>::value) {
+                uint32_t v = (uint32_t)acc[d][D - 1][r];
+#pragma unroll
+                for (int j = D - 2; j >= 0; j--) v = (v << 8) + (uint32_t)acc[d][j][r];
+                *dst = (int32_t)v;
+            } else {
+                double v = (double)acc[d][0][r];
+#pragma unroll
+                for (int j = 1; j < D; j++) v = __fma_rn((double)acc[d][j][r], (double)(1u << (8 * j)), v);
+                *dst = v;
+            }
         }
     }
 }
@@ -594,8 +604,9 @@
     const uint64_t r = x - __umul64hi(x, m.r1) * m.q;
     return r >= m.q ? r - m.q : r;
 }
-template <int ND>
-__global__ void __launch_bounds__(256) k_product_sum(const uint64_t *__restrict__ prod_, uint32_t K, uint64_t *__restrict__ out_, double *__restrict__ S_,
+typedef int32_t ps_i32x2 __attribute__((ext_vector_type(2)));
+template <int ND, class... E>
+__global__ void __launch_bounds__(256) k_product_sum(const uint64_t *__restrict__ prod_, uint32_t K, uint64_t *__restrict__ out_, typename DigitWord<E...>::type *__restrict__ S_,
                                                      const DevConsts *__restrict__ C) {
     typedef const NTT_GLOBAL ps_u64x2 *In;
     constexpr int PF = 4;
@@ -658,9 +669,11 @@
     ps_u64x2 v;
     v.x = ps_reduce(c0x, m); v.y = ps_reduce(c0y, m); dst[0] = v;
     v.x = ps_reduce(c1x, m); v.y = ps_reduce(c1y, m); dst[comp] = v;
-    typedef NTT_GLOBAL ps_f64x2 *OutS;
+    typedef typename DigitWord<E...>::type SE;
+    typedef typename std::conditional<std::is_same<SE, int32_t>::value, ps_i32x2, ps_f64x2>::type SV;
+    typedef NTT_GLOBAL SV *OutS;
     OutS sd = (OutS)S_ + ((size_t)o * C->rl_tot + g0) * n2 + p;
 #pragma unroll
     for (int d = 0; d < ND; d++)
-        if ((uint32_t)d < nd) { ps_f64x2 w; w.x = (double)dx[d]; w.y = (double)dy[d]; sd[(size_t)d * n2] = w; }
-}
+        if ((uint32_t)d < nd) { SV w; w.x = (SE)dx[d]; w.y = (SE)dy[d]; sd[(size_t)d * n2] = w; }
+}
diff --git a/cryptonets_amd/csrc/cn_k_ks.hip.h b/cryptonets_amd/csrc/cn_k_ks.hip.h
--- a/cryptonets_amd/csrc/cn_k_ks.hip.h
+++ b/cryptonets_amd/csrc/cn_k_ks.hip.h
@@ -36,9 +36,10 @@
 #ifndef KS_MAC_FENCE
 #define KS_MAC_FENCE 0
 #endif
-template <class AR> struct KsDigits {};
-template <class AR> struct KsSrc { typedef AR P; static constexpr bool dig = false; };
-template <class AR> struct KsSrc<KsDigits<AR>> { typedef AR P; static constexpr bool dig = true; };
+template <class AR, class... E> struct KsDigits {};
+template <class AR> struct KsSrc { typedef AR P; typedef double E; static constexpr bool dig = false; };
+template <class AR> struct KsSrc<KsDigits<AR>> { typedef AR P; typedef double E; static constexpr bool dig = true; };
+template <class AR> struct KsSrc<KsDigits<AR, int32_t>> { typedef AR P; typedef int32_t E; static constexpr bool dig = true; };
 template <int L, class AR_, int MINW = 1, bool TWL = false, bool XI = false>
 __global__ void __launch_bounds__(NttPlan<L>::NT, MINW) k_keyswitch_rr(const uint64_t *__restrict__ target, size_t tgt_stride, const uint64_t *__restrict__ add0,
                                                                  const uint64_t *__restrict__ add1, size_t add_stride, const void *__restrict__ key_,
@@ -90,7 +91,8 @@
         for (int r = 0; r < 16; r++) w[r] = src[pass_index<L, SA, 0>(t0, r)];
     };
     if constexpr (AHEAD) request(nraw, 0);
-    const double *dsrc = reinterpret_cast<const double *>(target) + (size_t)ct * tgt_stride;
+    typedef typename KsSrc<AR_>::E E;
+    const E *dsrc = reinterpret_cast<const E *>(target) + (size_t)ct * tgt_stride;
     for (uint32_t l = 0; l < k; l++) {
         const uint32_t nd = galois ? C->gk_dig[l] : C->rl_dig[l];
         if constexpr (DIG) {
@@ -476,7 +478,8 @@
     T v[16];
     if constexpr (DIG) {
         static_assert(std::is_same<T, double>::value, "ready-made digits: FP64 policies");
-        const double *dsrc = reinterpret_cast<const double *>(target) + (size_t)ct * tgt_stride + (size_t)g * n;
+        typedef typename KsSrc<AR_>::E E;
+        const E *dsrc = reinterpret_cast<const E *>(target) + (size_t)ct * tgt_stride + (size_t)g * n;
 #pragma unroll
         for (int r = 0; r < 16; r++) v[r] = (T)dsrc[pass_index<L, SA, 0>(tid, r)];
     } else {
@@ -550,7 +553,8 @@
     }
     ks_premultiply(raw, C, l);
     }
-    const double *dsrc = reinterpret_cast<const double *>(target) + (size_t)ct * tgt_stride + (size_t)g0 * n;
+    typedef typename KsSrc<AR_>::E E;
+    const E *dsrc = reinterpret_cast<const E *>(target) + (size_t)ct * tgt_stride + (size_t)g0 * n;
     T acc0[16], acc1[16];
 #pragma unroll
     for (int r = 0; r < 16; r++) { acc0[r] = 0; acc1[r] = 0; }
diff --git a/cryptonets_amd/csrc/cn_l_gemm.hip b/cryptonets_amd/csrc/cn_l_gemm.hip
--- a/cryptonets_amd/csrc/cn_l_gemm.hip
+++ b/cryptonets_amd/csrc/cn_l_gemm.hip
@@ -69,12 +69,16 @@
 
 template <int MT> static void launch_digit(cn_ctx *c, const DigitGemmLaunch &g, uint32_t ndg, uint32_t mtiles) {
     const size_t blocks = (size_t)(c->hc.n >> 8) * c->hc.k * ndg * mtiles * g.G;
-    hipLaunchKernelGGL((k_digit_gemm<MT, 5>), dim3((uint32_t)blocks), dim3(256), 0, c->stream, g.in, g.in_unit, (const int32_t *)g.idx, (const double *)g.W,
-                       (const int32_t *)g.oidx, g.S, c->dc, g.G, g.M, g.K, mtiles, g.Kp, g.Kw, ndg);
+    if (g.i32) hipLaunchKernelGGL((k_digit_gemm<MT, 5, int32_t>), dim3((uint32_t)blocks), dim3(256), 0, c->stream, g.in, g.in_unit, (const int32_t *)g.idx, (const double *)g.W,
+                                  (const int32_t *)g.oidx, (int32_t *)g.S, c->dc, g.G, g.M, g.K, mtiles, g.Kp, g.Kw, ndg);
+    else hipLaunchKernelGGL((k_digit_gemm<MT, 5>), dim3((uint32_t)blocks), dim3(256), 0, c->stream, g.in, g.in_unit, (const int32_t *)g.idx, (const double *)g.W,
+                            (const int32_t *)g.oidx, (double *)g.S, c->dc, g.G, g.M, g.K, mtiles, g.Kp, g.Kw, ndg);
 }
 template <int P, int DG> static void launch_digit_mfma(cn_ctx *c, const DigitGemmLaunch &g, uint32_t ndg, size_t blocks) {
-    hipLaunchKernelGGL((k_digit_gemm_mfma<P, DG>), dim3((uint32_t)blocks), dim3(256), 0, c->stream, g.in, g.in_unit, (const int32_t *)g.idx, (const int8_t *)g.W,
-                       (const int32_t *)g.oidx, g.S, c->dc, g.G, g.M, g.mtiles, g.ksteps, ndg);
+    if (g.i32) hipLaunchKernelGGL((k_digit_gemm_mfma<P, DG, int32_t>), dim3((uint32_t)blocks), dim3(256), 0, c->stream, g.in, g.in_unit, (const int32_t *)g.idx, (const int8_t *)g.W,
+                                  (const int32_t *)g.oidx, (int32_t *)g.S, c->dc, g.G, g.M, g.mtiles, g.ksteps, ndg);
+    else hipLaunchKernelGGL((k_digit_gemm_mfma<P, DG>), dim3((uint32_t)blocks), dim3(256), 0, c->stream, g.in, g.in_unit, (const int32_t *)g.idx, (const int8_t *)g.W,
+                            (const int32_t *)g.oidx, (double *)g.S, c->dc, g.G, g.M, g.mtiles, g.ksteps, ndg);
 }
 static int digit_gemm_mfma(cn_ctx *c, const DigitGemmLaunch &g, uint32_t ndmax) {
     const uint32_t DG = digit_gemm_mfma_group(g.P), ndg = (ndmax + DG - 1) / DG, mgroups = (g.mtiles + 3) / 4;
@@ -107,7 +111,8 @@
 }
 
 template <int ND> static void launch_product_sum(cn_ctx *c, const ProductSumLaunch &g, uint32_t blocks) {
-    hipLaunchKernelGGL((k_product_sum<ND>), dim3(blocks), dim3(256), 0, c->stream, g.prod, g.K, g.out, g.S, c->dc);
+    if (g.i32) hipLaunchKernelGGL((k_product_sum<ND, int32_t>), dim3(blocks), dim3(256), 0, c->stream, g.prod, g.K, g.out, (int32_t *)g.S, c->dc);
+    else hipLaunchKernelGGL((k_product_sum<ND>), dim3(blocks), dim3(256), 0, c->stream, g.prod, g.K, g.out, (double *)g.S, c->dc);
 }
 int cn_l_product_sum(cn_ctx *c, const ProductSumLaunch &g) {
     uint32_t ndmax = 0; for (uint32_t l = 0; l < c->hc.k; l++) ndmax = std::max(ndmax, c->hc.rl_dig[l]);
diff --git a/cryptonets_amd/csrc/cn_l_ks.inc.h b/cryptonets_amd/csrc/cn_l_ks.inc.h
--- a/cryptonets_amd/csrc/cn_l_ks.inc.h
+++ b/cryptonets_amd/csrc/cn_l_ks.inc.h
@@ -10,20 +10,24 @@
     return 0;
 }
 template <int L> static size_t ks_twl_lds() { return ((size_t)ntt_lds_words(1u << L) + (1u << L)) * 8; }
+template <int L> static constexpr bool kDig32 = kF64 && L <= 13;
+template <int L, class DS> static int set_attrs_dig(size_t bytes) {
+    CHECK(big_lds(k_keyswitch_rr<L, DS, 1, false, false>, bytes));
+    if constexpr (KsFwd<AR, L>::lds) CHECK(big_lds(k_keyswitch_rr<L, DS, 1, true, false>, ks_twl_lds<L>()));
+    CHECK(big_lds(k_ks_digit_mac<L, DS>, bytes)); CHECK(big_lds(k_ks_limb_mac<L, DS>, bytes));
+    return 0;
+}
 template <int L> static int set_attrs_l(size_t bytes) {
     CHECK(big_lds(k_keyswitch_rr<L, AR>, bytes)); CHECK(big_lds(k_keyswitch_rr<L, AR, 1, false, true>, bytes));
     if constexpr (KsFwd<AR, L>::lds) { CHECK(big_lds(k_keyswitch_rr<L, AR, 1, true>, ks_twl_lds<L>())); CHECK(big_lds(k_keyswitch_rr<L, AR, 1, true, true>, ks_twl_lds<L>())); }
     CHECK(big_lds(k_ks_digit_mac<L, AR>, bytes)); CHECK(big_lds(k_ks_limb_mac<L, AR>, bytes)); CHECK(big_lds(k_ks_sum_intt<L, AR>, bytes));
-    if constexpr (kF64) {
-        CHECK(big_lds(k_keyswitch_rr<L, KsDigits<AR>, 1, false, false>, bytes));
-        if constexpr (KsFwd<AR, L>::lds) CHECK(big_lds(k_keyswitch_rr<L, KsDigits<AR>, 1, true, false>, ks_twl_lds<L>()));
-        CHECK(big_lds(k_ks_digit_mac<L, KsDigits<AR>>, bytes)); CHECK(big_lds(k_ks_limb_mac<L, KsDigits<AR>>, bytes));
-    }
+    if constexpr (kF64) { CHECK((set_attrs_dig<L, KsDigits<AR>>(bytes))); if constexpr (kDig32<L>) CHECK((set_attrs_dig<L, KsDigits<AR, int32_t>>(bytes))); }
     return 0;
 }
 static int set_attrs(uint32_t logn, size_t bytes) {
     if constexpr (kF64) { if (logn == 12) { CHECK(big_lds(k_keyswitch_rr<12, AR, 1, true>, ks_twl_lds<12>())); CHECK(big_lds(k_keyswitch_rr<12, AR, 1, true, true>, ks_twl_lds<12>()));
-                                           CHECK(big_lds(k_keyswitch_rr<12, KsDigits<AR>, 1, true, false>, ks_twl_lds<12>())); } }
+                                           CHECK(big_lds(k_keyswitch_rr<12, KsDigits<AR>, 1, true, false>, ks_twl_lds<12>()));
+                                           CHECK(big_lds(k_keyswitch_rr<12, KsDigits<AR, int32_t>, 1, true, false>, ks_twl_lds<12>())); } }
     if (logn == 13) CHECK(set_attrs_l<13>(bytes));
     if (logn == 14) {
         CHECK(set_attrs_l<14>(bytes));
@@ -36,9 +40,9 @@
     return 0;
 }
 static const uint32_t KS_TWL_MIN_DIGITS = 12;
-template <int L, bool XI, bool DIG = false> static void launch_fused_x(cn_ctx *c, const KsArgs &a) {
+template <int L, bool XI, class ARS = AR> static void launch_fused_x(cn_ctx *c, const KsArgs &a) {
     const uint32_t tot = a.galois ? c->hc.gk_tot : c->hc.rl_tot;
-    typedef typename std::conditional<DIG, KsDigits<AR>, AR>::type ARS;
+    constexpr bool DIG = KsSrc<ARS>::dig;
     const uint64_t *tgt = DIG ? (const uint64_t *)a.dig : a.target;
     const size_t tstride = DIG ? (size_t)tot * c->hc.n : a.tstride;
     if constexpr (KsFwd<AR, L>::lds) {
@@ -52,9 +56,21 @@
                        a.add0, a.add1, a.astride, (const void *)a.key, a.out, c->dc, a.galois, a.accmax, a.extra, a.xstride, a.out_tab, a.xcd_cts);
 }
 template <int L> static void launch_fused(cn_ctx *c, const KsArgs &a) {
-    if constexpr (kF64) { if (a.dig) { launch_fused_x<L, false, true>(c, a); return; } }
+    if constexpr (kF64) {
+        if (a.dig) {
+            if constexpr (kDig32<L>) { if (a.dig_i32) { launch_fused_x<L, false, KsDigits<AR, int32_t>>(c, a); return; } }
+            launch_fused_x<L, false, KsDigits<AR>>(c, a); return;
+        }
+    }
     if (c->hc.ks_xi) launch_fused_x<L, true>(c, a);
     else launch_fused_x<L, false>(c, a);
+}
+template <int L, class DS> static void launch_dig_mac(cn_ctx *c, const KsArgs &a, uint32_t tot, size_t lds) {
+    const uint32_t k = c->hc.k;
+    if (a.mode == 2) hipLaunchKernelGGL((k_ks_limb_mac<L, DS>), dim3(a.cnt * k * k), dim3(NttPlan<L>::NT), lds, c->stream, (const uint64_t *)a.dig, (size_t)tot * c->hc.n,
+                                        (const void *)a.key, c->ks_part, c->dc, a.galois, a.accmax, 0u, (const KsItem *)nullptr);
+    else hipLaunchKernelGGL((k_ks_digit_mac<L, DS>), dim3(a.cnt * tot * k), dim3(NttPlan<L>::NT), lds, c->stream, (const uint64_t *)a.dig, (size_t)tot * c->hc.n,
+                            (const void *)a.key, c->ks_part, c->dc, a.galois, tot, 0u, (const KsItem *)nullptr);
 }
 template <int L> static void launch_two_phase(cn_ctx *c, const KsArgs &a) {
     const uint32_t tot = a.galois ? c->hc.gk_tot : c->hc.rl_tot, k = c->hc.k;
@@ -63,10 +79,10 @@
     if constexpr (kF64) dig = a.dig != nullptr;
     if (dig) {
         if constexpr (kF64) {
-            if (a.mode == 2) hipLaunchKernelGGL((k_ks_limb_mac<L, KsDigits<AR>>), dim3(a.cnt * k * k), dim3(NttPlan<L>::NT), lds, c->stream, (const uint64_t *)a.dig, (size_t)tot * c->hc.n,
-                                                (const void *)a.key, c->ks_part, c->dc, a.galois, a.accmax, 0u, (const KsItem *)nullptr);
-            else hipLaunchKernelGGL((k_ks_digit_mac<L, KsDigits<AR>>), dim3(a.cnt * tot * k), dim3(NttPlan<L>::NT), lds, c->stream, (const uint64_t *)a.dig, (size_t)tot * c->hc.n,
-                                    (const void *)a.key, c->ks_part, c->dc, a.galois, tot, 0u, (const KsItem *)nullptr);
+            bool i32 = false;
+            if constexpr (kDig32<L>) i32 = a.dig_i32;
+            if constexpr (kDig32<L>) { if (i32) launch_dig_mac<L, KsDigits<AR, int32_t>>(c, a, tot, lds); }
+            if (!i32) launch_dig_mac<L, KsDigits<AR>>(c, a, tot, lds);
         }
         hipLaunchKernelGGL((k_ks_sum_intt<L, AR>), dim3(a.cnt * k * 2), dim3(NttPlan<L>::NT), lds, c->stream, (const void *)c->ks_part, a.add0, a.add1, a.astride,
                            a.out, c->dc, a.mode == 2 ? k : tot, a.mode == 2 ? 0xffffffffu : a.accmax, a.extra, a.xstride, a.out_tab, a.perm_elt, a.items);
diff --git a/cryptonets_amd/csrc/cn_level.hip b/cryptonets_amd/csrc/cn_level.hip
--- a/cryptonets_amd/csrc/cn_level.hip
+++ b/cryptonets_amd/csrc/cn_level.hip
@@ -21,7 +21,7 @@
 }
 static int adopt_from_parent(cn_ctx *c, cn_ctx *parent) {
     const uint32_t k = c->hc.k;
-    c->opt = parent->opt; c->defer_square_gemm = parent->defer_square_gemm; c->mul_sum = parent->mul_sum;
+    c->opt = parent->opt; c->defer_square_gemm = parent->defer_square_gemm; c->mul_sum = parent->mul_sum; c->digit_i32 = parent->digit_i32;
     memcpy(c->rng_key, parent->rng_key, sizeof c->rng_key);
     c->hc.ks_xi = parent->hc.ks_xi;
     for (uint32_t l = 0; l < k; l++) c->hc.ks_inv_qhat_q[l] = parent->hc.ks_inv_qhat_q[l];
diff --git a/cryptonets_amd/csrc/cn_policy.h b/cryptonets_amd/csrc/cn_policy.h
--- a/cryptonets_amd/csrc/cn_policy.h
+++ b/cryptonets_amd/csrc/cn_policy.h
@@ -21,4 +21,8 @@
     return r;
 }
 inline int cn_policy(const CnModRange &r, bool use_f64) { return !(use_f64 && r.f64ok) ? POL_U64 : (r.light ? POL_F64L : POL_F64); }
+inline bool cn_digit_sum_fits_i32(uint64_t sum_abs_w, int dbc) {
+    if (dbc < 1 || dbc > 31) return false;
+    return (unsigned __int128)sum_abs_w * ((1ull << dbc) - 1) <= 0x7fffffffull;
+}
 inline bool cn_rr_size(uint32_t logn, uint32_t max_logn = 14) { return logn >= 10 && logn <= max_logn; }
diff --git a/cryptonets_amd/csrc/cn_runtime.h b/cryptonets_amd/csrc/cn_runtime.h
--- a/cryptonets_amd/csrc/cn_runtime.h
+++ b/cryptonets_amd/csrc/cn_runtime.h
@@ -183,6 +183,8 @@
     uint32_t ms_groups = 0;
     bool mul_sum = true;
     bool digit_mfma = true;
+    bool digit_i32 = true;
+    uint64_t ks_dig_i32 = 0;
     bool defer_square_gemm = false;
     uint64_t uid = 0;
     hipStream_t stream2 = nullptr; hipEvent_t ev_fork = nullptr, ev_join = nullptr; bool stream2_failed = false;
@@ -208,11 +210,14 @@
     const KsItem *items = nullptr;
     uint32_t perm_elt = 0;
     uint32_t next_elt = 0; uint64_t *next_out = nullptr;
-    const double *dig = nullptr;
+    const void *dig = nullptr;
+    bool dig_i32 = false;
     static KsCall relin(const uint64_t *prod, size_t kn, uint32_t cnt) {
         return {.target = prod + 2 * kn, .tstride = 3 * kn, .add0 = prod, .add1 = prod + kn, .astride = 3 * kn, .cnt = cnt};
     }
-    static KsCall relin_digits(const double *S, const uint64_t *base, size_t kn, uint32_t cnt) { return {.add0 = base, .add1 = base + kn, .astride = 2 * kn, .cnt = cnt, .dig = S}; }
+    static KsCall relin_digits(const void *S, bool i32, const uint64_t *base, size_t kn, uint32_t cnt) {
+        return {.add0 = base, .add1 = base + kn, .astride = 2 * kn, .cnt = cnt, .dig = S, .dig_i32 = i32};
+    }
     static KsCall galois_of(const uint64_t *c1, size_t c1_stride, const uint64_t *c0, size_t kn, uint32_t cnt) {
         return {.target = c1, .tstride = c1_stride, .add0 = c0, .astride = 2 * kn, .cnt = cnt, .galois = 1};
     }
@@ -271,15 +276,16 @@
 int cn_l_gemm(cn_ctx *c, const GemmLaunch &g);
 int cn_l_gemm_mfma(cn_ctx *c, const GemmLaunch &g);
 struct DigitGemmLaunch {
-    const uint64_t *in; size_t in_unit; const void *idx; const void *W; const void *oidx; double *S;
+    const uint64_t *in; size_t in_unit; const void *idx; const void *W; const void *oidx; void *S;
     uint32_t G, M, K, Kp, Kw, MT;
     bool mfma = false; uint32_t P = 0, mtiles = 0, ksteps = 0;
+    bool i32 = false;
 };
 inline uint32_t digit_gemm_mfma_group(uint32_t P) { return P <= 2 ? 3u : 2u; }
 inline uint32_t digit_gemm_tile(uint32_t M) { return M > 2 ? 10u : 2u; }
 inline uint32_t digit_gemm_rows(uint32_t K) { return ((K + 7) & ~7u) + 8; }
 int cn_l_digit_gemm(cn_ctx *c, const DigitGemmLaunch &g);
-struct ProductSumLaunch { const uint64_t *prod; uint32_t K; uint64_t *out; double *S; uint32_t outputs; };
+struct ProductSumLaunch { const uint64_t *prod; uint32_t K; uint64_t *out; void *S; uint32_t outputs; bool i32 = false; };
 static const uint32_t PRODUCT_SUM_MAX_DIGITS = 8;
 int cn_l_product_sum(cn_ctx *c, const ProductSumLaunch &g);
 struct MulPlainSumLaunch { const uint64_t *pt, *ctn; const uint32_t *grp_off, *slot; uint64_t *out; uint32_t groups, accmax; };
```

After: 1.229 million, median of 6. 1.02x the previous value.
